# Wumpf/yasph2d

Hardware: AMD Instinct MI355X
Metric: particle-steps/sec (whole node), 2D DFSPH dam-break (higher is better)
Workload: dtype f32

## Files before the change

### include/sphx.h

```cpp
#ifndef SPHX_H
#define SPHX_H

#include <stddef.h>
#include <stdint.h>

#ifdef __cplusplus
extern "C" {
#endif

#define SPHX_ABI_VERSION 5

enum {
    SPHX_OK = 0,
    SPHX_ERR_INVALID_ARGUMENT = 1,
    SPHX_ERR_NO_DEVICE = 2,
    SPHX_ERR_HIP = 3,
    SPHX_ERR_NOT_READY = 4,
    SPHX_ERR_NONFINITE = 5,
    SPHX_ERR_NEIGHBOR_PANIC = 6,
    SPHX_ERR_CAPACITY = 7,
    SPHX_ERR_OUT_OF_DOMAIN = 8
};

enum {
// ... 93 lines not shown
    uint32_t* owner;
} sphx_render_out;
enum { SPHX_RENDER_NONE = 0xFFFFFFFFu, SPHX_RENDER_BOUNDARY = 0xFFFFFFFEu };
enum { SPHX_RENDER_DEVICE_POINTERS = 1u };
int sphx_render_fit(uint32_t width, uint32_t height, float x, float y, float w, float h, sphx_render_view* out);
int sphx_render(sphx_ctx* ctx, const sphx_render_view* view, uint32_t flags, const sphx_render_out* out);

typedef struct sphx_rect { float x0, y0, x1, y1; } sphx_rect;
#define SPHX_REMOVE_MAX_RECTS 8
enum { SPHX_REMOVE_OUTSIDE = 1u };
int sphx_append(sphx_ctx* ctx, const float* pos_xy, const float* vel_xy , uint32_t m, uint32_t* out_first_id );
int sphx_remove(sphx_ctx* ctx, const sphx_rect* rects, uint32_t n_rects, uint32_t flags, uint32_t* out_removed );

#define SPHX_STATE_SECTIONS 9
enum {
    SPHX_STATE_SEC_POSITIONS = 0, SPHX_STATE_SEC_VELOCITIES = 1, SPHX_STATE_SEC_PARTICLE_ID = 2, SPHX_STATE_SEC_DENSITY = 3, SPHX_STATE_SEC_ALPHA = 4,
    SPHX_STATE_SEC_KAPPA = 5, SPHX_STATE_SEC_STIFFNESS = 6, SPHX_STATE_SEC_ACCEL = 7, SPHX_STATE_SEC_BOUNDARY = 8
};
enum { SPHX_STATE_DEVICE_BUFFER = 1u };
int sphx_state_size(sphx_ctx* ctx, uint64_t* out_bytes);
int sphx_state_save(sphx_ctx* ctx, void* buf, uint64_t capacity, uint32_t flags, uint64_t* out_bytes );
int sphx_state_load(sphx_ctx* ctx, const void* buf, uint64_t bytes, uint32_t flags);
int sphx_state_digest(sphx_ctx* ctx, uint64_t* out );
int sphx_state_save_file(sphx_ctx* ctx, const char* path);
int sphx_state_load_file(sphx_ctx* ctx, const char* path);

#define SPHX_TRACK_MAX_IDS 16384
#define SPHX_TRACK_ABSENT  0xFFFFFFFFu
enum { SPHX_TRACK_DEVICE_POINTERS = 1u };
typedef struct sphx_track_out {
    uint32_t* slot;
    float* pos;
    float* vel;
    float* density;
} sphx_track_out;
typedef struct sphx_track_status { uint32_t m, recording, max_frames, every, frames, dropped, reserved[2]; } sphx_track_status;
int sphx_track_set(sphx_ctx* ctx, const uint32_t* ids , uint32_t m);
int sphx_track_fetch(sphx_ctx* ctx, uint32_t flags, const sphx_track_out* out);
int sphx_track_record(sphx_ctx* ctx, uint32_t max_frames, uint32_t every);
int sphx_track_get_status(const sphx_ctx* ctx, sphx_track_status* out);
int sphx_track_read(sphx_ctx* ctx, uint32_t first_frame, uint32_t n_frames, uint32_t flags, float* out );
int sphx_download_by_id(sphx_ctx* ctx, uint32_t first_id, uint32_t count, uint32_t flags, const sphx_track_out* out, uint32_t* out_present );

typedef struct sphx_fields_out {
    float* vel_grad;
    float* divergence;
    float* vorticity;
    float* color_grad;
} sphx_fields_out;
enum { SPHX_FIELDS_DEVICE_POINTERS = 1u };
int sphx_particle_fields(sphx_ctx* ctx, uint32_t flags, const sphx_fields_out* out);

#define SPHX_STATS_MAX_RECTS 8
enum { SPHX_STATS_DEVICE_POINTERS = 1u };
typedef struct sphx_stats_rec {
    uint64_t count;
    uint64_t nonfinite;
    uint64_t density_count;
    uint32_t density_valid;
    uint32_t reserved;
    double sum_pos[2];
    double sum_vel[2];
    double sum_speed_sq;
    double sum_angular;
    double sum_density;
    double sum_density_sq;
    double max_speed_sq;
    float min_pos[2], max_pos[2];
    float min_density, max_density;
} sphx_stats_rec;
typedef struct sphx_stats_frame { uint64_t step; float dt; uint32_t n; } sphx_stats_frame;
typedef struct sphx_stats_status { uint32_t n_rects, recording, max_frames, every, frames, dropped, reserved[2]; } sphx_stats_status;
int sphx_fluid_stats(sphx_ctx* ctx, const sphx_rect* rects , uint32_t n_rects, uint32_t flags, sphx_stats_rec* out );
int sphx_stats_record(sphx_ctx* ctx, const sphx_rect* rects , uint32_t n_rects, uint32_t max_frames, uint32_t every);
int sphx_stats_get_status(const sphx_ctx* ctx, sphx_stats_status* out);
int sphx_stats_read(sphx_ctx* ctx, uint32_t first_frame, uint32_t n_frames, sphx_stats_rec* out ,
                    sphx_stats_frame* info );

int sphx_debug_correction_counts(sphx_ctx* ctx, uint64_t out[3]);
int sphx_debug_quiet_counts(sphx_ctx* ctx, uint64_t out[2]);
int sphx_debug_takeover_counts(sphx_ctx* ctx, uint64_t out[3]);

int sphx_debug_rigid_counts(sphx_ctx* ctx, uint64_t out[3]);
int sphx_debug_download_accel(sphx_ctx* ctx, float* out_xy);

int sphx_clear_cached(sphx_ctx* ctx);
int sphx_step_begin(sphx_ctx* ctx, float dt_prev, float* out_vmax);
int sphx_step_finish(sphx_ctx* ctx, float dt, sphx_step_stats* out_stats);

typedef struct sphx_timer_law {
    uint32_t adaptive;
    float cfl_factor;
    float particle_diameter;
    uint32_t reserved;
    uint64_t timestep_min_ns;
    uint64_t timestep_max_ns;
    uint64_t simulation_step_ns;
} sphx_timer_law;
int sphx_step_begin_law(sphx_ctx* ctx, float dt_prev, const sphx_timer_law* law, float* out_vmax);

int sphx_wcsph_step_begin(sphx_ctx* ctx, float dt, float* out_vmax);
int sphx_wcsph_step_finish(sphx_ctx* ctx, float dt, sphx_step_stats* out_stats);

int sphx_update_neighborhood(sphx_ctx* ctx);
int sphx_update_densities(sphx_ctx* ctx, int kernel_kind);
int sphx_compute_alpha(sphx_ctx* ctx);

int sphx_download_solver_state(sphx_ctx* ctx, float* alpha, float* kappa, float* stiffness);
int sphx_download_neighbors(sphx_ctx* ctx, uint16_t* counts, uint32_t* lists, uint64_t* out_total_entries);
int sphx_download_cells(sphx_ctx* ctx, int which, uint32_t* first_particle, uint32_t* cidx, uint32_t* out_count);
uint32_t sphx_last_flags(const sphx_ctx* ctx);
int sphx_grid_info(const sphx_ctx* ctx, int which, uint32_t* out4);
int sphx_get_constants(const sphx_ctx* ctx, float* out6);
int sphx_get_viscosity(const sphx_ctx* ctx, uint32_t* model, float* fluid_viscosity, float* normalizer_laplacian);


int sphx_reserve(sphx_ctx* ctx, uint32_t capacity);
int sphx_tile_configure(sphx_ctx* ctx, int axis, uint32_t cell_lo, uint32_t cell_hi, uint32_t halo_cells, int has_left, int has_right);
#define SPHX_MAX_TILE_PEERS 8
typedef struct sphx_tile_rect { uint32_t x0, x1, y0, y1; } sphx_tile_rect;
int sphx_tile_configure_rect(sphx_ctx* ctx, const sphx_tile_rect* own, uint32_t halo_cells, const sphx_tile_rect* peers, uint32_t n_peers);
int sphx_tile_pack_n(sphx_ctx* ctx, void* const* d_send, uint32_t n_send, uint32_t cap_records);
int sphx_tile_apply_n(sphx_ctx* ctx, const void* const* d_recv, uint32_t n_recv, uint32_t cap_records);
int sphx_tile_advect_pack_n(sphx_ctx* ctx, float dt, void* const* d_send, uint32_t n_send, uint32_t cap_records);
int sphx_tile_upload(sphx_ctx* ctx, const float* pos_xy, const float* vel_xy, const uint32_t* ids, uint32_t n);
#define SPHX_HALO_RECORD_BYTES 32
int sphx_tile_pack(sphx_ctx* ctx, void* d_send_left, void* d_send_right, uint32_t cap_records);
int sphx_tile_apply(sphx_ctx* ctx, const void* d_from_left, const void* d_from_right, uint32_t cap_records);
int sphx_tile_count_kept(sphx_ctx* ctx);
int sphx_sub_regrid(sphx_ctx* ctx, uint32_t* out_n_local);
int sphx_sub_regrid_div(sphx_ctx* ctx, uint32_t* out_n_local);
int sphx_sub_regrid_warm(sphx_ctx* ctx, uint32_t* out_n_local);
int sphx_sub_run_ahead(sphx_ctx* ctx, float dt_prev_of_next_step);
int sphx_tile_carry_warmstart(sphx_ctx* ctx, int kappa, int stiffness);
int sphx_tile_defer_advect(sphx_ctx* ctx, int on);
int sphx_tile_band_packs(const sphx_ctx* ctx, uint32_t* out);
int sphx_tile_send_counts(sphx_ctx* ctx, void* const* d_send, uint32_t n_send, uint32_t cap_records, uint32_t* out_counts);
int sphx_sub_nonpressure(sphx_ctx* ctx, float dt_prev, float* out_vmax_sq);
int sphx_sub_predict(sphx_ctx* ctx, float dt);
int sphx_sub_warmstart(sphx_ctx* ctx, int divergence, float dt);
int sphx_sub_iteration(sphx_ctx* ctx, int divergence, float dt, int first, double* out_err_sum, uint64_t* out_n_owned);
int sphx_sub_advect(sphx_ctx* ctx, float dt);
int sphx_sub_predict_iteration(sphx_ctx* ctx, float dt, double* out_err_sum, uint64_t* out_n_owned);


typedef struct sphx_multi sphx_multi;
enum { SPHX_LAYOUT_AUTO = 0, SPHX_LAYOUT_STRIPS = 1, SPHX_LAYOUT_GRID = 2 };
typedef struct sphx_multi_options {
    uint32_t halo_cells;
    uint32_t fixed_halo;
    uint32_t rebalance_every;
    uint32_t layout;
    uint32_t cap_records;
    uint32_t overlap_exchange;
    uint32_t reserved[2];
} sphx_multi_options;
typedef struct sphx_comm_ops {
    void* user;
    int rank, world;
    int (*exchange)(void* user, const int* peers, int n_peers, void* const* d_send, void* const* d_recv, size_t bytes, void* hip_stream);
    int (*allreduce)(void* user, const double* in, int n, int op, double* out);
    void (*abort)(void* user);
} sphx_comm_ops;
typedef struct sphx_multi_info_t {
    uint32_t world, local_tiles, halo_now, halo_max, peers, n_local, cap_records, grid_layout;
    int32_t axis;
// ... 247 lines not shown
```

### yasph2d_amd/__init__.py

```python
import ctypes as C

import numpy as np

from . import _lib
from ._lib import (FLAG_DENSITY_ITER_CAP, FLAG_DIVERGENCE_ITER_CAP, FLAG_DENSE_CELL, FLAG_NEIGHBOR_CAP, FLAG_STRAY_PARTICLES, FLAG_WARMUP, KERNEL_POLY6,
                   KERNEL_SPIKY, KERNEL_WENDLAND_C2, VISCOSITY_PHYSICAL, VISCOSITY_XSPH, SphxError, SphxKernelTime, SphxParams, SphxStepStats)

__all__ = ["SphxContext", "FluidParticleWorld", "TimeManager", "DFSPHSolver", "DFSPHMultiSolver", "default_params", "duration_from_secs_f32",
           "duration_as_secs_f32", "SphxError", "WCSPHSolver", "VISCOSITY_XSPH", "VISCOSITY_PHYSICAL", "SAMPLE_FIELDS", "gauge_elevation",
           "sample_merge", "render_fit", "render_merge", "track_merge", "track_merge_frames", "write_png", "SCENE_RECT", "TRACK_FIELDS", "MULTI_TRACK_FIELDS", "FIELD_NAMES", "STATS_DTYPE", "STATS_FRAME_DTYPE"]


def _p(a):
    return a.ctypes.data_as(C.c_void_p) if a is not None else None


LISTS_32BIT = 0xFFFFFFFF


_VISCOSITY_MODELS = {"xsph": VISCOSITY_XSPH, "physical": VISCOSITY_PHYSICAL}


def default_params(smoothing_factor=2.0, particle_density=10000.0, fluid_density=100.0, device=0, fixed_iterations=(0, 0), viscosity="xsph",
                   fluid_viscosity=None):
# ... 538 lines not shown

    def track_record(self, max_frames, every=1):
        self._chk(self.L.sphx_track_record(self.h, max_frames, every))

    def track_frames(self, first=0, count=None):
        st = self.track_status()
        if count is None:
            count = max(st["frames"] - first, 0)
        out = np.zeros((count, st["m"], 4), np.float32)
        self._chk(self.L.sphx_track_read(self.h, first, count, 0, _p(out) if out.size else None))
        return out

    def ids_issued(self):
        first = C.c_uint32()
        rc = self.L.sphx_append(self.h, None, None, 0, C.byref(first))
        if rc == _lib.ERR_NOT_READY:
            return 0
        self._chk(rc)
        return first.value

    def download_by_id(self, first=0, count=None, fields=TRACK_FIELDS):
        if count is None:
            count = max(self.ids_issued() - first, 0)
        outs = _track_outputs(fields, count)
        present = C.c_uint32()
        self._chk(self.L.sphx_download_by_id(self.h, first, count, 0, C.byref(_track_struct(outs)), C.byref(present)))
        outs["present"] = present.value
        return outs

    def download_boundary(self):
        xy = np.zeros((self.nb, 2), np.float32)
        ids = np.zeros(self.nb, np.uint32)
        self._chk(self.L.sphx_download_boundary(self.h, _p(xy), _p(ids)))
        return xy, ids

    def download_solver_state(self):
        n = self.n
        a, k, s = (np.zeros(n, np.float32) for _ in range(3))
        self._chk(self.L.sphx_download_solver_state(self.h, _p(a), _p(k), _p(s)))
        return dict(alpha=a, kappa=k, stiffness=s)

    def download_neighbors(self):
        n = self.n
        counts = np.zeros((n, 2), np.uint16)
        total = C.c_uint64()
        self._chk(self.L.sphx_download_neighbors(self.h, _p(counts), None, C.byref(total)))
        lists = np.zeros(total.value, np.uint32)
        self._chk(self.L.sphx_download_neighbors(self.h, None, _p(lists), C.byref(total)))
        start = np.zeros(n + 1, np.uint64)
        np.cumsum(counts[:, 1].astype(np.uint64), out=start[1:])
        return counts, start, lists

    def download_cells(self, static=False):
        m = C.c_uint32()
        self._chk(self.L.sphx_download_cells(self.h, int(static), None, None, C.byref(m)))
        first = np.zeros(m.value, np.uint32)
        cidx = np.zeros(m.value, np.uint32)
        self._chk(self.L.sphx_download_cells(self.h, int(static), _p(first), _p(cidx), C.byref(m)))
        return first, cidx

    def last_flags(self):
        return self.L.sphx_last_flags(self.h)

    def correction_counts(self):
        out = (C.c_uint64 * 3)()
        self._chk(self.L.sphx_debug_correction_counts(self.h, out))
        return int(out[0]), int(out[1]), int(out[2])

    def quiet_counts(self):
        out = (C.c_uint64 * 2)()
        self._chk(self.L.sphx_debug_quiet_counts(self.h, out))
        return int(out[0]), int(out[1])

    def takeover_counts(self):
        out = (C.c_uint64 * 3)()
        self._chk(self.L.sphx_debug_takeover_counts(self.h, out))
        return int(out[0]), int(out[1]), int(out[2])

    def rigid_counts(self):
        out = (C.c_uint64 * 3)()
        self._chk(self.L.sphx_debug_rigid_counts(self.h, out))
        return int(out[0]), int(out[1]), int(out[2])

    def download_accel(self):
        out = np.zeros((self.n, 2), np.float32)
        self._chk(self.L.sphx_debug_download_accel(self.h, out.ctypes.data_as(C.c_void_p)))
        return out

    def grid_info(self, which=0):
        out = (C.c_uint32 * 4)()
        self._chk(self.L.sphx_grid_info(self.h, which, out))
        return dict(blocks=out[0], entries=out[1], nbx=out[2], nby=out[3])

    def constants(self):
        out = np.zeros(6, np.float32)
        self._chk(self.L.sphx_get_constants(self.h, _p(out)))
        return out

    def viscosity(self):
        m, mu, nlap = C.c_uint32(), C.c_float(), C.c_float()
        self._chk(self.L.sphx_get_viscosity(self.h, C.byref(m), C.byref(mu), C.byref(nlap)))
        return {VISCOSITY_XSPH: "xsph", VISCOSITY_PHYSICAL: "physical"}[m.value], np.float32(mu.value), np.float32(nlap.value)

    def sample(self, points, kernel=KERNEL_WENDLAND_C2, fields=SAMPLE_FIELDS):
        flags = _sample_fields(fields)
        if _is_torch(points):
            import torch

            if points.device.type != "cuda" or points.dtype != torch.float32 or points.dim() != 2 or points.shape[1] != 2:
                raise ValueError("points must be a float32 [m, 2] tensor on the context's device")
            if self.params is not None and points.device.index not in (None, self.params.device):
                raise ValueError("points are on %s, the context on device %d" % (points.device, self.params.device))
            pts = points.contiguous()
            m = pts.shape[0]
            outs = _torch_outputs(flags, (m,), pts.device)
            torch.cuda.current_stream(pts.device).synchronize()
            self._chk(self.L.sphx_sample_points(self.h, C.c_void_p(pts.data_ptr()), m, kernel, _lib.SAMPLE_DEVICE_POINTERS,
                                                C.byref(_out_struct(outs, lambda t: t.data_ptr()))))
            self.synchronize()
            return outs
        pts = np.ascontiguousarray(points, np.float32)
        if pts.ndim != 2 or pts.shape[1] != 2:
            raise ValueError("points must be a float32 [m, 2] array, not shape %s" % (pts.shape,))
        m = len(pts)
        outs = _numpy_outputs(flags, (m,))
        self._chk(self.L.sphx_sample_points(self.h, _p(pts), m, kernel, 0, C.byref(_out_struct(outs, lambda a: a.ctypes.data))))
        return outs

    def sample_grid(self, origin, spacing, shape, kernel=KERNEL_WENDLAND_C2, fields=SAMPLE_FIELDS):
        flags = _sample_fields(fields)
        dx, dy = (spacing, spacing) if np.ndim(spacing) == 0 else spacing
        ny, nx = (int(v) for v in shape)
        if nx < 0 or ny < 0:
            raise ValueError("shape must be (ny, nx) with non-negative sizes")
        outs = _numpy_outputs(flags, (ny, nx))
        self._chk(self.L.sphx_sample_grid(self.h, origin[0], origin[1], dx, dy, nx, ny, kernel, 0,
                                          C.byref(_out_struct(outs, lambda a: a.ctypes.data))))
        return outs

    def render(self, view=None, *, out=None, owner=False, rgba=True, **view_fields):
        if view is None:
            width, height = view_fields.pop("width", 1920), view_fields.pop("height", 1080)
            view = render_fit(width, height, view_fields.pop("world_rect", SCENE_RECT))
        else:
            view = _copy_view(view)
        _set_view_fields(view, view_fields)
        owner_tensor = owner if _is_torch(owner) else None
        owner = owner_tensor is not None or bool(owner)
        if not rgba and not owner:
            raise ValueError("nothing to render: rgba and owner are both off")
        h, w = view.height, view.width
        o = _lib.SphxRenderOut()
        if out is not None or owner_tensor is not None:
            import torch

            dev = out.device if out is not None else owner_tensor.device
            if out is not None and (not _is_torch(out) or out.device.type != "cuda" or out.dtype != torch.uint8 or tuple(out.shape) != (h, w, 4)
                                    or not out.is_contiguous()):
                raise ValueError("out must be a contiguous uint8 (%d, %d, 4) tensor on the context's device" % (h, w))
            if not rgba and out is not None:
                raise ValueError("out given with rgba=False")
            own = None
            if owner:
                own = owner_tensor if owner_tensor is not None else torch.empty((h, w), dtype=torch.int32, device=dev)
                if own.dtype != torch.int32 or tuple(own.shape) != (h, w) or not own.is_contiguous() or own.device != dev:
                    raise ValueError("owner must be a contiguous int32 (%d, %d) tensor on the device of out" % (h, w))
# ... 399 lines not shown
```

### yasph2d_amd/_lib.py

```python
import ctypes as C
import os
import subprocess

_HERE = os.path.dirname(os.path.abspath(__file__))
LIB_PATH = os.environ.get("SPHX_LIB") or os.path.join(_HERE, "libsphx.so")
CSRC = os.path.join(_HERE, "csrc")

OK, ERR_INVALID_ARGUMENT, ERR_NO_DEVICE, ERR_HIP, ERR_NOT_READY, ERR_NONFINITE, ERR_NEIGHBOR_PANIC, ERR_CAPACITY, ERR_OUT_OF_DOMAIN = range(9)
FLAG_NEIGHBOR_CAP, FLAG_DENSITY_ITER_CAP, FLAG_DIVERGENCE_ITER_CAP, FLAG_WARMUP, FLAG_STRAY_PARTICLES, FLAG_DENSE_CELL = 1, 2, 4, 8, 16, 32
KERNEL_WENDLAND_C2, KERNEL_POLY6, KERNEL_SPIKY = 0, 1, 2
VISCOSITY_XSPH, VISCOSITY_PHYSICAL = 0, 1


class SphxParams(C.Structure):
    _fields_ = [
        ("smoothing_length", C.c_float),
        ("particle_mass", C.c_float),
        ("fluid_density", C.c_float),
        ("particle_radius", C.c_float),
        ("gravity", C.c_float * 2),
        ("grid_min", C.c_float * 2),
        ("xsph_epsilon", C.c_float),
        ("max_avg_density_error", C.c_float),
        ("max_density_iterations", C.c_uint32),
# ... 183 lines not shown
                ("exchanges", C.c_uint64), ("rebalances", C.c_uint64), ("build_particles", C.c_uint64), ("neighbor_entries", C.c_uint64),
                ("remote_entries", C.c_uint64), ("owned_local", C.c_uint64), ("transport", C.c_char * 96),
                ("halo_bytes_packed", C.c_uint64), ("halo_bytes_sent", C.c_uint64), ("ownership_seconds", C.c_double)]


LAYOUT_AUTO, LAYOUT_STRIPS, LAYOUT_GRID = 0, 1, 2

_vp, _u16p = C.c_void_p, C.c_void_p
_f, _u32, _u64, _i = C.c_float, C.c_uint32, C.c_uint64, C.c_int
class SphxTileStateOut(C.Structure):
    _fields_ = [(k, C.c_void_p) for k in ("pos", "vel", "id", "density", "alpha", "kappa", "stiffness")]


SIGNATURES = {
    "sphx_abi_version": (_u32, []),
    "sphx_default_params": (_i, [_f, _f, _f, C.POINTER(SphxParams)]),
    "sphx_create": (_i, [C.POINTER(SphxParams), C.POINTER(_vp)]),
    "sphx_destroy": (None, [_vp]),
    "sphx_last_error": (C.c_char_p, [_vp]),
    "sphx_set_boundary": (_i, [_vp, _vp, _u32]),
    "sphx_upload": (_i, [_vp, _vp, _vp, _u32]),
    "sphx_append": (_i, [_vp, _vp, _vp, _u32, C.POINTER(_u32)]),
    "sphx_remove": (_i, [_vp, C.POINTER(SphxRect), _u32, _u32, C.POINTER(_u32)]),
    "sphx_state_size": (_i, [_vp, C.POINTER(_u64)]),
    "sphx_state_save": (_i, [_vp, _vp, _u64, _u32, C.POINTER(_u64)]),
    "sphx_state_load": (_i, [_vp, _vp, _u64, _u32]),
    "sphx_state_digest": (_i, [_vp, C.POINTER(_u64)]),
    "sphx_state_save_file": (_i, [_vp, C.c_char_p]),
    "sphx_state_load_file": (_i, [_vp, C.c_char_p]),
    "sphx_track_set": (_i, [_vp, _vp, _u32]),
    "sphx_track_fetch": (_i, [_vp, _u32, C.POINTER(SphxTrackOut)]),
    "sphx_track_record": (_i, [_vp, _u32, _u32]),
    "sphx_track_get_status": (_i, [_vp, C.POINTER(SphxTrackStatus)]),
    "sphx_track_read": (_i, [_vp, _u32, _u32, _u32, _vp]),
    "sphx_particle_fields": (_i, [_vp, _u32, C.POINTER(SphxFieldsOut)]),
    "sphx_multi_track_set": (_i, [_vp, _vp, _u32]),
    "sphx_multi_track_fetch": (_i, [_vp, _u32, C.POINTER(SphxMultiTrackOut)]),
    "sphx_multi_track_record": (_i, [_vp, _u32, _u32]),
    "sphx_multi_track_get_status": (_i, [_vp, C.POINTER(SphxTrackStatus)]),
    "sphx_multi_track_read": (_i, [_vp, _u32, _u32, _u32, _vp, _vp]),
    "sphx_multi_download_by_id": (_i, [_vp, _u32, _u32, _u32, C.POINTER(SphxMultiTrackOut), C.POINTER(_u32)]),
    "sphx_track_merge": (_i, [_u32, C.POINTER(SphxMultiTrackOut), _u32, C.POINTER(SphxMultiTrackOut), C.POINTER(_u32)]),
    "sphx_track_merge_frames": (_i, [_u64, C.POINTER(_vp), C.POINTER(_vp), _u32, _vp, _vp]),
    "sphx_tile_track_install": (_i, [_vp, _vp, _vp, _u32, _u32]),
    "sphx_tile_track_fetch_enqueue": (_i, [_vp]),
    "sphx_tile_track_fetch": (_i, [_vp, _vp, _vp, _vp]),
    "sphx_tile_track_window_enqueue": (_i, [_vp, _u32, _u32, _u32]),
    "sphx_tile_track_window_fetch": (_i, [_vp, _vp, C.POINTER(_u32)]),
    "sphx_tile_track_record": (_i, [_vp, _u32, _u32]),
    "sphx_tile_track_frame": (_i, [_vp]),
    "sphx_tile_track_read": (_i, [_vp, _u32, _u32, _vp, _vp]),
    "sphx_fluid_stats": (_i, [_vp, C.POINTER(SphxRect), _u32, _u32, _vp]),
    "sphx_stats_record": (_i, [_vp, C.POINTER(SphxRect), _u32, _u32, _u32]),
    "sphx_stats_get_status": (_i, [_vp, C.POINTER(SphxStatsStatus)]),
    "sphx_stats_read": (_i, [_vp, _u32, _u32, _vp, _vp]),
    "sphx_tile_fluid_stats": (_i, [_vp, C.POINTER(SphxRect), _u32, _u32, _vp]),
    "sphx_tile_stats_record": (_i, [_vp, C.POINTER(SphxRect), _u32, _u32, _u32]),
    "sphx_tile_stats_frame": (_i, [_vp, _f, _u32]),
    "sphx_tile_stats_read": (_i, [_vp, _u32, _u32, _vp, _vp]),
    "sphx_multi_fluid_stats": (_i, [_vp, C.POINTER(SphxRect), _u32, _u32, _vp, _vp]),
    "sphx_multi_stats_record": (_i, [_vp, C.POINTER(SphxRect), _u32, _u32, _u32]),
    "sphx_multi_stats_get_status": (_i, [_vp, C.POINTER(SphxStatsStatus)]),
    "sphx_multi_stats_read": (_i, [_vp, _u32, _u32, _vp, _vp]),
    "sphx_tile_state_pack": (_i, [_vp, _u32, C.POINTER(SphxTileStateOut), C.POINTER(_u64), C.POINTER(_u32)]),
    "sphx_tile_state_fetch": (_i, [_vp, C.POINTER(_u64), C.POINTER(_u32)]),
    "sphx_tile_upload_state": (_i, [_vp, _vp, _vp, _vp, _vp, _vp, _u32]),
    "sphx_get_tiling_invariant": (_i, [_vp]),
    "sphx_multi_state_size": (_i, [_vp, C.POINTER(_u64)]),
    "sphx_multi_state_save": (_i, [_vp, _vp, _u64, _u32, C.POINTER(_u64)]),
    "sphx_multi_state_load": (_i, [_vp, C.POINTER(_vp), C.POINTER(_u64), _u32, _u32]),
    "sphx_multi_state_digest": (_i, [_vp, C.POINTER(_u64)]),
    "sphx_multi_state_save_file": (_i, [_vp, C.c_char_p]),
    "sphx_multi_state_load_file": (_i, [_vp, C.c_char_p]),
    "sphx_multi_append": (_i, [_vp, _vp, _vp, _u32, C.POINTER(_u32)]),
    "sphx_multi_remove": (_i, [_vp, C.POINTER(SphxRect), _u32, _u32, C.POINTER(_u64)]),
    "sphx_tile_remove_mark": (_i, [_vp, C.POINTER(SphxRect), _u32, _u32]),
    "sphx_tile_remove_fetch": (_i, [_vp, C.POINTER(_u32)]),
    "sphx_tile_append": (_i, [_vp, _vp, _vp, _vp, _u32]),
    "sphx_tile_grow": (_i, [_vp, _u32]),
    "sphx_debug_correction_counts": (_i, [_vp, _vp]),
    "sphx_debug_quiet_counts": (_i, [_vp, _vp]),
    "sphx_debug_takeover_counts": (_i, [_vp, _vp]),
    "sphx_debug_rigid_counts": (_i, [_vp, _vp]),
    "sphx_debug_download_accel": (_i, [_vp, _vp]),
    "sphx_download_by_id": (_i, [_vp, _u32, _u32, _u32, C.POINTER(SphxTrackOut), C.POINTER(_u32)]),
    "sphx_download": (_i, [_vp, _vp, _vp, _vp, _vp]),
    "sphx_download_boundary": (_i, [_vp, _vp, _vp]),
    "sphx_num_particles": (_u32, [_vp]),
    "sphx_num_boundary": (_u32, [_vp]),
    "sphx_sample_points": (_i, [_vp, _vp, _u32, _i, _u32, C.POINTER(SphxSampleOut)]),
    "sphx_sample_grid": (_i, [_vp, _f, _f, _f, _f, _u32, _u32, _i, _u32, C.POINTER(SphxSampleOut)]),
    "sphx_multi_sample_points": (_i, [_vp, _vp, _u32, _i, _u32, C.POINTER(SphxMultiSampleOut)]),
    "sphx_multi_sample_grid": (_i, [_vp, _f, _f, _f, _f, _u32, _u32, _i, _u32, C.POINTER(SphxMultiSampleOut)]),
    "sphx_sample_merge": (_i, [_u32, C.POINTER(SphxMultiSampleOut), _u32, C.POINTER(SphxMultiSampleOut)]),
    "sphx_multi_tile_rects": (_i, [_vp, C.POINTER(SphxTileRect), C.POINTER(_u32)]),
    "sphx_multi_ghost_rings": (_i, [_vp, C.POINTER(C.c_double)]),
    "sphx_tile_sample_points": (_i, [_vp, _vp, _u32, _i, _u32]),
    "sphx_tile_sample_points_fetch": (_i, [_vp, _vp, _u32, C.POINTER(_u32)]),
    "sphx_tile_sample_window": (_i, [_vp, _f, _f, _f, _f, _u32, _u32, _i, _u32, C.POINTER(_u32)]),
    "sphx_tile_sample_window_fetch": (_i, [_vp, C.POINTER(SphxSampleOut)]),
    "sphx_multi_particle_fields": (_i, [_vp, _u32, C.POINTER(SphxMultiFieldsOut), C.POINTER(C.c_uint64)]),
    "sphx_tile_owned_count": (_i, [_vp, C.POINTER(_u32)]),
    "sphx_tile_particle_fields_enqueue": (_i, [_vp, _u32, _u32]),
    "sphx_tile_particle_fields_fetch": (_i, [_vp, C.POINTER(SphxFieldsOut), _vp, _u32, C.POINTER(_u32)]),
    "sphx_render_fit": (_i, [_u32, _u32, _f, _f, _f, _f, C.POINTER(SphxRenderView)]),
    "sphx_render": (_i, [_vp, C.POINTER(SphxRenderView), _u32, C.POINTER(SphxRenderOut)]),
    "sphx_multi_render": (_i, [_vp, C.POINTER(SphxRenderView), _u32, C.POINTER(SphxRenderOut)]),
    "sphx_multi_render_layer": (_i, [_vp, C.POINTER(SphxRenderView), _u32, C.POINTER(SphxRenderLayer)]),
    "sphx_render_merge": (_i, [_u32, _u32, C.POINTER(SphxRenderLayer), _u32, C.POINTER(SphxRenderLayer)]),
    "sphx_tile_render_layer": (_i, [_vp, C.POINTER(SphxRenderView), _u32, C.POINTER(SphxRenderLayer)]),
    "sphx_tile_render_window": (_i, [_vp, C.POINTER(SphxRenderView), _u32, C.POINTER(_u32), C.POINTER(SphxRenderLayer)]),
    "sphx_clear_cached": (_i, [_vp]),
    "sphx_step_begin": (_i, [_vp, _f, C.POINTER(_f)]),
    "sphx_step_begin_law": (_i, [_vp, _f, _vp, _vp]),
    "sphx_timer_law_of": (_i, [_vp, _f, _vp]),
    "sphx_timer_set_target_frame": (None, [_vp, _u64]),
    "sphx_timer_on_step_started": (None, [_vp]),
    "sphx_step_finish": (_i, [_vp, _f, C.POINTER(SphxStepStats)]),
    "sphx_update_neighborhood": (_i, [_vp]),
    "sphx_update_densities": (_i, [_vp, _i]),
    "sphx_compute_alpha": (_i, [_vp]),
    "sphx_download_solver_state": (_i, [_vp, _vp, _vp, _vp]),
    "sphx_download_neighbors": (_i, [_vp, _vp, _vp, C.POINTER(_u64)]),
    "sphx_download_cells": (_i, [_vp, _i, _vp, _vp, C.POINTER(_u32)]),
    "sphx_grid_info": (_i, [_vp, _i, C.POINTER(_u32)]),
    "sphx_last_flags": (_u32, [_vp]),
    "sphx_get_constants": (_i, [_vp, _vp]),
    "sphx_get_viscosity": (_i, [_vp, C.POINTER(_u32), C.POINTER(_f), C.POINTER(_f)]),
    "sphx_reserve": (_i, [_vp, _u32]),
    "sphx_tile_configure": (_i, [_vp, _i, _u32, _u32, _u32, _i, _i]),
    "sphx_tile_upload": (_i, [_vp, _vp, _vp, _vp, _u32]),
    "sphx_tile_pack": (_i, [_vp, _vp, _vp, _u32]),
    "sphx_tile_apply": (_i, [_vp, _vp, _vp, _u32]),
    "sphx_tile_count_kept": (_i, [_vp]),
    "sphx_sub_regrid": (_i, [_vp, C.POINTER(_u32)]),
    "sphx_sub_regrid_div": (_i, [_vp, C.POINTER(_u32)]),
    "sphx_sub_regrid_warm": (_i, [_vp, C.POINTER(_u32)]),
    "sphx_sub_nonpressure": (_i, [_vp, _f, C.POINTER(_f)]),
    "sphx_sub_predict": (_i, [_vp, _f]),
    "sphx_sub_warmstart": (_i, [_vp, _i, _f]),
    "sphx_sub_iteration": (_i, [_vp, _i, _f, _i, C.POINTER(C.c_double), C.POINTER(_u64)]),
    "sphx_sub_predict_iteration": (_i, [_vp, _f, C.POINTER(C.c_double), C.POINTER(_u64)]),
    "sphx_tile_band_packs": (_i, [_vp, C.POINTER(_u32)]),
    "sphx_tile_send_counts": (_i, [_vp, _vp, _u32, _u32, C.POINTER(_u32)]),
    "sphx_sub_advect": (_i, [_vp, _f]),
    "sphx_shm_open": (_vp, [C.c_char_p, _i, _i]),
    "sphx_shm_allreduce": (_i, [_vp, _vp, _i, _i, _vp]),
    "sphx_shm_allgather": (_i, [_vp, _vp, _i, _vp]),
    "sphx_shm_abort": (None, [_vp]),
    "sphx_sub_run_ahead": (_i, [_vp, C.c_float]),
    "sphx_tile_carry_warmstart": (_i, [_vp, _i, _i]),
    "sphx_set_tiling_invariant": (_i, [_vp, _i]),
    "sphx_tile_defer_advect": (_i, [_vp, _i]),
    "sphx_build_stats": (_i, [_vp, _vp, _vp, _vp]),
    "sphx_shm_close": (None, [_vp]),
    "sphx_tile_configure_rect": (_i, [_vp, _vp, _u32, _vp, _u32]),
    "sphx_tile_pack_n": (_i, [_vp, _vp, _u32, _u32]),
    "sphx_tile_apply_n": (_i, [_vp, _vp, _u32, _u32]),
    "sphx_tile_advect_pack_n": (_i, [_vp, _f, _vp, _u32, _u32]),
    "sphx_view_request": (_i, [_vp, _u32, C.POINTER(_u32)]),
    "sphx_view_fetch": (_i, [_vp, _i, C.POINTER(C.POINTER(_f)), C.POINTER(_u32)]),
    "sphx_synchronize": (_i, [_vp]),
    "sphx_set_stream": (_i, [_vp, _vp]),
    "sphx_profile_enable": (_i, [_vp, _i]),
    "sphx_profile_reset": (_i, [_vp]),
    "sphx_profile_filter": (_i, [_vp, C.c_char_p, _u32]),
# ... 101 lines not shown
```

### yasph2d_amd/csrc/sphx_handoff.hpp

```cpp
#pragma once
#include <cstdint>
#include <cstring>

namespace sphx {

struct BuildHandoff {
    enum Kind : uint8_t { None, WarmApplied, FirstErrors };
    Kind kind = None;
    bool has_flags = false, warm_taken = false;
    uint32_t mark_tag = 0;
    struct Taken {
        bool fused, flags_usable, warm_taken;
    };
    static BuildHandoff warm_applied() { return BuildHandoff{WarmApplied, false, false, 0u}; }
    static BuildHandoff first_errors(bool flags, uint32_t tag, bool taken) { return BuildHandoff{FirstErrors, flags, flags && taken, tag}; }
    void clear() { *this = BuildHandoff{}; }
    bool first_errors_pending() const { return kind == FirstErrors; }
    bool take_warm() {
        const bool applied = kind == WarmApplied;
        if (applied) clear();
        return applied;
    }
    Taken take_first_errors(bool first_divergence, uint32_t rseq) {
        if (kind != FirstErrors || !first_divergence) return Taken{false, false, false};
        const bool usable = has_flags && mark_tag == rseq;
        const Taken t{true, usable, usable && warm_taken};
        clear();
        return t;
    }
};

class PendingCount {
  public:
    enum class Maker : uint8_t { Nobody, Correction, Pack, Classifier };
    PendingCount() = default;
    void made_by_correction(uint32_t n) { *this = PendingCount(Maker::Correction, n); }
    void made_by_pack(uint32_t n) { *this = PendingCount(Maker::Pack, n); }
    void made_by_classifier(uint32_t n, float dt) { *this = PendingCount(Maker::Classifier, n, true, bits(dt)); }
    bool live() const { return maker_ != Maker::Nobody; }
    bool from_classifier() const { return maker_ == Maker::Classifier; }
    bool is_for(uint32_t n) const { return live() && n_ == n; }
    bool is_for_first_of(uint32_t n) const { return live() && n_ <= n; }
    uint32_t n() const { return n_; }
    bool take_over_class(uint32_t n, float dt) {
        const bool mine = from_classifier() && takeable_ && n_ == n && dt_bits_ == bits(dt);
        if (mine) made_by_pack(n);
        return mine;
    }
    void bar_take_over() { takeable_ = false; }
    bool drop() {
        const bool wipe = live();
        forget();
        return wipe;
    }
    bool drop_if_from_classifier() { return from_classifier() && drop(); }
    void forget() { *this = PendingCount(); }

  private:
    PendingCount(Maker m, uint32_t n, bool takeable = false, uint32_t dt_bits = 0) : maker_(m), takeable_(takeable), n_(n), dt_bits_(dt_bits) {}
    static uint32_t bits(float f) {
        uint32_t u;
        std::memcpy(&u, &f, 4);
        return u;
    }
    Maker maker_ = Maker::Nobody;
    bool takeable_ = false;
    uint32_t n_ = 0, dt_bits_ = 0;
};

struct VelMarks {
    bool valid = false, thin_seen = false;
    uint32_t tag = 0, knz_tag = 0;
    struct Taken {
        bool usable, check_knz;
        uint32_t tag, knz_tag;
    };
    void made(uint32_t gather_tag) { *this = VelMarks{true, false, gather_tag, 0u}; }
    void thin(uint32_t rseq) {
        if (!valid) return;
        if (thin_seen) return wrote();
        thin_seen = true;
        knz_tag = rseq;
    }
    void wrote() { *this = VelMarks{}; }
    Taken take() {
        const Taken t{valid, valid && thin_seen, tag, knz_tag};
        wrote();
        return t;
    }
};

}
```

### yasph2d_amd/csrc/sphx_internal.hpp

```cpp
#pragma once
#include <hip/hip_runtime.h>

#include <dlfcn.h>

#include <algorithm>
#include <cstdint>
#include <cstdlib>
#include <cstdio>
#include <cstring>
#include <functional>
#include <map>
#include <string>
#include <vector>

#include "../../include/sphx.h"
#include "sphx_handoff.hpp"

namespace sphx {

constexpr uint32_t EMPTY = 0xFFFFFFFFu;
constexpr uint32_t MAX_NEIGHBORS = 64;
constexpr uint32_t BLOCK_SHIFT = 6;
constexpr uint32_t BLOCK_CELLS = 4096;
constexpr uint32_t SCAN_TILE = 4096;
// ... 18 lines not shown
constexpr uint32_t REMOTE_CAP = 512;
constexpr uint32_t ENTRY_BITS = 10, ENTRY_MASK = (1u << ENTRY_BITS) - 1u;
constexpr uint32_t WAVE_REMOTE = REMOTE_CAP / 4;
constexpr uint32_t STRIPES = 32;

constexpr uint32_t DIR_FRINGE = 0x80000000u;
constexpr uint32_t DIR_STATIC = 1u;
constexpr uint32_t DIR_FLAGS = DIR_FRINGE | DIR_STATIC;
enum : uint32_t { DF_OUT_OF_DOMAIN = 1u, DF_HALO_CAP = 2u, DF_NB_CAP = 4u, DF_NB_PANIC = 8u, DF_NEAR_EDGE = 16u, DF_STRAY = 32u, DF_SCAN_STALL = 64u, DF_NONFINITE = 128u, DF_DENSE_CELL = 256u };
constexpr uint32_t RANK_LOOP_MAX = 4096;
constexpr uint32_t LOOP_HIST = 512;

constexpr uint32_t MAX_TILE_PEERS = 8;
struct TileRect {
    uint32_t x0, x1, y0, y1;
};

struct Consts {
    float h;
    float radius_sq;
    float cell_inv;
    float gmin_x, gmin_y;
    float w_hinv, w_norm, w_ngrad;
    float p6_hsq, p6_norm, p6_ngrad;
    float sp_h, sp_norm, sp_ngrad;
    float mass, rho0, xsph_eps;
    float ax, ay;
    float gx, gy;
    float wc_stiffness, wc_boundary_force;
    TileRect tile;
    uint32_t remote_cap;
    uint32_t q_noclamp;
    uint32_t nt_cold;
    uint32_t xcd_shift;
    uint32_t rev;
};

struct ViscConsts {
    uint32_t visc_model;
    float mu;
    float vis_nlap;
};
template <int VM>
struct ViscArg {};
template <>
struct ViscArg<SPHX_VISCOSITY_PHYSICAL> : ViscConsts {};

struct NbView {
    const uint32_t* list;
    const uint16_t* counts;
    const uint32_t* wave;
    const uint32_t* remote;
    uint32_t lazy_hi;
    uint32_t stream;
};
constexpr uint32_t COUNT_MANY_LINES = 1u << 14;
struct PVr {
    const float2* pos;
    const float2* vel;
};

struct GridView {
    const uint32_t* dir;
    const uint2* fine;
    uint32_t bx0, by0, nbx, nby;
    uint32_t cbits;
};
struct NbGrid {
    const uint32_t* dirn;
    const uint2* fine;
    uint32_t bx0, by0, nbx, nbx1, nby1;
};
constexpr uint32_t DIRN_FLAG = 1u;

struct alignas(128) Stripe {
    unsigned long long nb_entries;
    unsigned long long owned;
    unsigned long long rem_entries;
    unsigned long long res_hi, res_lo;
    uint32_t ticket;
    uint32_t pad0;
    unsigned long long zs_skipped, zs_window, zs_remote;
    unsigned long long zs_quiet;
    uint32_t pad[12];
};
static_assert(sizeof(Stripe) == 128, "one stripe, one cache line");
struct alignas(128) VmaxStripe {
    uint32_t vmax[4];
    uint32_t pad[28];
};
struct alignas(128) MarkStripe {
    uint32_t knz_mark;
    uint32_t vmix_mark;
    uint32_t pad[30];
};
static_assert(sizeof(MarkStripe) == 128, "one stripe, one cache line");
struct alignas(128) SpecLine {
    uint32_t flags;
    uint32_t pad0;
    unsigned long long moved;
    uint32_t pad[28];
};
struct DevScalars {
    uint32_t flags;
    uint32_t ticket;
    uint32_t sort_total;
    float dt;
    uint32_t loop_done;
    uint32_t pad0;
    unsigned long long snap_hi[2], snap_lo[2];
    uint32_t rigid_exits, rigid_marked;
    uint32_t pad[16];
    Stripe stripe[STRIPES];
    VmaxStripe vstripe[STRIPES];
    MarkStripe mstripe[STRIPES];
    SpecLine spec;
};

struct Mailbox {
    volatile uint32_t seq;
    uint32_t flags;
    uint32_t vmax_sq_bits;
    uint32_t quiet_seq;
    double err_sum;
    unsigned long long nb_entries;
    unsigned long long owned_cum;
    unsigned long long rem_entries;
    uint32_t sort_total;
    uint32_t dt_bits;
    unsigned long long dt_ns;
    volatile uint32_t loop_gen_done;
    uint32_t loop_iters;
    double loop_hist[LOOP_HIST];
    uint32_t send_counts[MAX_TILE_PEERS];
    uint32_t rigid_tag;
};

struct ResArgs {
    uint32_t enabled;
    uint32_t rseq;
    Mailbox* mb;
    uint32_t seq;
};
struct VmaxArgs {
    uint32_t enabled;
    uint32_t vslot;
    Mailbox* mb;
    uint32_t seq;
};
struct LoopArgs {
    uint32_t enabled;
    uint32_t iter;
    uint32_t fixed;
    uint32_t max_iters;
    uint32_t gen;
    uint32_t n_total;
    float tol;
    float rho0;
    float dt;
};

struct TimerLaw {
    uint32_t enabled, adaptive;
    float cfl_factor, particle_diameter;
    unsigned long long min_ns, max_ns, step_ns;
};

struct Grid {
    uint32_t* dir = nullptr;
    uint32_t* dirn = nullptr;
    uint32_t dir_cap = 0;
    uint2* fine = nullptr;
    uint32_t* hist = nullptr;
    uint32_t* tile_empty = nullptr;
    uint32_t tile_cap = 0;
    uint32_t fine_cap = 0;
    uint32_t bx0 = 0, by0 = 0, nbx = 0, nby = 0, nblk = 0;
    std::vector<uint8_t> cover;
    std::vector<uint32_t> h_dir;
    bool fine_valid = false;
    uint32_t len() const { return nblk * BLOCK_CELLS; }
    uint32_t cbits_floor = 1;
    uint32_t cbits() const {
        uint32_t b = cbits_floor < 1u ? 1u : cbits_floor > 31u ? 31u : cbits_floor;
        while (b < 31u && ((1u << b) - 1u) < len()) ++b;
        return b;
    }
    GridView view() const { return GridView{dir, fine, bx0, by0, nbx, nby, cbits()}; }
    NbGrid nview() const { return nbx && nby ? NbGrid{dirn, fine, bx0, by0, nbx, nbx - 1u, nby - 1u} : NbGrid{dirn, fine, 0u, 0u, 1u, 0u, 0u}; }
};

struct ProfTotals {
    uint64_t launches = 0;
    double ms = 0, bytes = 0;
};
struct ProfPending {
    const char* name;
    double bytes;
    hipEvent_t a, b;
// ... 13 lines not shown
    uint32_t B = 0, capB = 0;
    uint32_t cached_n = 0;
    bool set_changed = false;
    uint64_t ids_issued = 0;
    uint32_t* edit_buf = nullptr;
    uint32_t edit_cap = 0;
    static constexpr uint32_t MARK_NONE = 0xFFFFFFFFu, MARK_EMPTY = 0xFFFFFFFEu;
    uint32_t edit_mark = MARK_NONE;
    struct Track {
        uint32_t m = 0, unique = 0, log2_bits = 0;
        uint32_t* set_buf = nullptr;
        uint32_t *table = nullptr, *map = nullptr, *filter = nullptr, *found = nullptr;
        float* rec = nullptr;
        uint32_t recording = 0, max_frames = 0, every = 0, frames = 0, dropped = 0, steps = 0;
        uint32_t* scratch = nullptr;
        size_t scratch_cap = 0;
        uint32_t window_cap = 0;
    } track;
    struct Stats {
        sphx_stats_rec* scratch = nullptr;
        sphx_stats_rec* rec = nullptr;
        sphx_rect rects[SPHX_STATS_MAX_RECTS] = {};
        uint32_t n_rects = 0, recording = 0, max_frames = 0, every = 0, frames = 0, dropped = 0, steps = 0;
        std::vector<sphx_stats_frame> info;
    } stats;
    bool uploaded = false, boundary_changed = true, tails_dirty = true, in_step = false;
    bool lists_current = false;
    unsigned long long* state_dig = nullptr;
    uint32_t* mstate_buf = nullptr;
    size_t mstate_cap = 0;
    uint32_t mstate_n = 0;
    uint32_t fast_walk_ok = 0;
    uint32_t sample_ready = 0;
    bool tile_density_ready = false;
    const char* sample_missing = "no neighbour build yet: run a step, or sphx_update_neighborhood + sphx_update_densities";
    float* sample_buf = nullptr;
    size_t sample_cap = 0;
    struct TileSample {
        uint32_t m = 0;
        uint32_t fields = 0;
        uint32_t win[4] = {0, 0, 0, 0};
        size_t rec_at = 0;
        uint32_t* null_grid = nullptr;
    } tsample;
    uint32_t* render_buf = nullptr;
    size_t render_cap = 0;
    float* fields_buf = nullptr;
    size_t fields_cap = 0;
    struct TileFields {
        bool queued = false;
        uint32_t n = 0;
        uint32_t mask = 0;
        bool ids = false;
    } tfields;
    uint32_t num_density_iters = 1, num_divergence_iters = 0;
    float step_dt_prev = 0, step_vmax = 0;
    uint32_t step_flags = 0;

    float2 *posA = nullptr, *posA2 = nullptr;
    float2 *vel = nullptr, *vel2 = nullptr;
    sphx::PVr pv() const { return sphx::PVr{posA, vel}; }
    float* kbuf = nullptr;
    uint32_t* knz = nullptr;
    int zero_skip = -1;
    bool zero_skip_on() const { return zero_skip < 0 ? N >= 4000000u : zero_skip != 0; }
    int zero_skip_count = 0;
    bool quiet_hint[2] = {false, false};
    unsigned long long qf_launches = 0;
    int quiet_takeover = 1;
    uint32_t thin_grid = 0;
    int quiet_takeover_density = 1;
    bool take_over(bool divergence) const {
        return !tile_mode && (divergence || quiet_takeover_density) && (quiet_takeover == 2 || (quiet_takeover == 1 && quiet_hint[divergence ? 1 : 0]));
    }
    unsigned long long thin_launches = 0, takeover_producers = 0;
    int rigid_skip = -1;
    bool rigid_on() const { return !tile_mode && (rigid_skip < 0 ? N >= 4000000u : rigid_skip != 0); }
    sphx::VelMarks velmarks;
    uint32_t gather_seq = 0;
    bool rigid_hint = false;
    uint32_t rigid_judged = 0;
    void rigid_forget() {
        velmarks.wrote();
        rigid_hint = false;
        rigid_judged = 0;
    }
    unsigned long long rigid_launches = 0;
    float2* accel = nullptr;
    float *density = nullptr, *alpha = nullptr, *alpha2 = nullptr, *kappa = nullptr, *stiff = nullptr;
    float *kappa2 = nullptr, *stiff2 = nullptr;
    uint32_t *pid = nullptr, *pid2 = nullptr;
    uint32_t *key = nullptr, *slot = nullptr, *order = nullptr;
    uint32_t idx_cap = 0;
    uint32_t soff() const { return capN; }
    float2 *bpos = nullptr, *bpos2 = nullptr;
    uint32_t *bid = nullptr, *bid2 = nullptr;
    sphx::Grid gdyn, gstat;
    bool have_fluid_bbox = false;
    uint32_t fb[4] = {0, 0, 0, 0};
    uint32_t builds_since_cover = 0;
    bool need_expand = false;
    bool need_recover = false;
    uint32_t recover_streak = 0;
    uint32_t recover_cooldown = 0;
    float wcsph_vmax_prev = 0.0f;
    std::vector<float> h_boundary;
    uint32_t* nb_list = nullptr;
    uint16_t* nb_counts = nullptr;
    uint32_t* nb_wave = nullptr;
    uint32_t* nb_remote = nullptr;
    uint32_t pre_seq = 0, pre_warm = 0, law_dt_bits = 0;
    bool law_active = false;
    uint32_t pre_gen = 0;
    uint32_t pre_queued = 0;
    uint32_t loop_gen = 0;
    uint32_t res_seq = 0;
    uint32_t vmax_seq = 0;
    struct RunAhead {
        bool queued = false;
        bool valid = false;
        uint32_t n = 0, dt_bits = 0, vslot = 0;
        uint32_t seq = 0;
    } ahead;
    float tile_pending_dt = 0.0f;
    uint32_t tile_pending_n = 0;
    bool tile_defer_advect = false;
    float sub_ahead_dt = 0.0f;
    bool tile_carry_kappa = true, tile_carry_stiff = true;
    bool tiling_invariant = false;
    int run_ahead = 1;
#ifndef SPHX_DEFAULT_FUSE_PREDICT
#define SPHX_DEFAULT_FUSE_PREDICT 1
#endif
    int fuse_predict = SPHX_DEFAULT_FUSE_PREDICT;
    int tile_fuse_class = 1;
    uint32_t tile_band_packs = 0;
    bool tile_fix_owner = false;
    int fuse_div = 1;
    int xcd_chunk = -1;
    int alternate_sweep = 1;
    int fuse_warm = 1;
    sphx::BuildHandoff handoff;
    int host_loop = 0;
    std::string prof_filter;
    uint32_t prof_every = 1, prof_counter = 0;
    bool external_stream = false;
    hipStream_t view_stream = nullptr;
    hipEvent_t view_packed = nullptr, view_done = nullptr;
    float *view_dev = nullptr, *view_host = nullptr;
    uint32_t view_cap = 0, view_count = 0;
    bool view_pending = false;
    uint32_t wcsph_n = 0;
    bool in_wcsph = false;
    int lazy_table = 1;
    int stream_lists = -1;
    int nt_cold_stores = -1;
    sphx::NbView nbv() const {
        return sphx::NbView{nb_list, nb_counts, nb_wave, nb_remote, (uint32_t)lazy_table, stream_lists < 0 ? (N >= 4000000u ? 1u : 0u) : (uint32_t)stream_lists};
    }
    uint32_t* scan_partials = nullptr;
    uint32_t scan_partials_cap = 0;
    unsigned long long* scan_state = nullptr;
    uint32_t scan_state_cap = 0, scan_epoch = 0;
    sphx::PendingCount pending;
    int no_fused_count = 0;
    int scan_two_pass = 0;
    sphx::DevScalars* d_scal = nullptr;
    sphx::Mailbox* mbox = nullptr;
    sphx::Mailbox* mbox_dev = nullptr;
    uint32_t seq = 0;
// ... 29 lines not shown
```

### yasph2d_amd/csrc/sphx_kernels.hip

```cpp
#include "sphx_internal.hpp"
#include "sphx_sqrt.hpp"
#include "sphx_xcd.hpp"

namespace sphx {

__device__ __forceinline__ uint32_t part1by1(uint32_t x) {
    x &= 0xffffu;
    x = (x ^ (x << 8)) & 0x00ff00ffu;
    x = (x ^ (x << 4)) & 0x0f0f0f0fu;
    x = (x ^ (x << 2)) & 0x33333333u;
    x = (x ^ (x << 1)) & 0x55555555u;
    return x;
}
__device__ __forceinline__ uint32_t morton2(uint32_t x, uint32_t y) { return (part1by1(y) << 1) | part1by1(x); }

__device__ __forceinline__ uint32_t spread6(uint32_t v) {
    v &= 63u;
    v = (v | (v << 4)) & 0x30Fu;
    v = (v | (v << 2)) & 0x333u;
    v = (v | (v << 1)) & 0x555u;
    return v;
}
__device__ __forceinline__ uint32_t sat_u16(float v) {
    v = fminf(fmaxf(v, 0.0f), 65535.0f);
// ... 1989 lines not shown
        va.mb->vmax_sq_bits = bits;
        if (law.enabled) {
            __hip_atomic_store((uint32_t*)&scal->dt, __float_as_uint(dt_new), __ATOMIC_RELAXED, __HIP_MEMORY_SCOPE_AGENT);
            va.mb->dt_ns = ns;
            va.mb->dt_bits = __float_as_uint(dt_new);
        }
    }
    publish_common(scal, va.mb, va.seq);
}

__device__ __forceinline__ unsigned long long residual_fixed(float e, bool& bad) {
    bad = !(e < 1073741824.0f);
    const float t = __builtin_rintf((bad ? 0.0f : e) * 16777216.0f);
    const uint32_t bits = __float_as_uint(t);
    const uint32_t m = (bits & 0x7fffffu) | 0x800000u;
    const int sh = (int)((bits >> 23) & 0xffu) - 150;
    unsigned long long f = sh >= 0 ? (unsigned long long)m << (sh & 63) : (unsigned long long)(m >> min(-sh, 31));
    return (bits & 0x7f800000u) ? f : 0ull;
}
__device__ __forceinline__ void block_residual_add(float e, DevScalars* __restrict__ scal) {
    bool bad;
    const unsigned long long f = wave_sum_u63(residual_fixed(e, bad));
    __shared__ unsigned long long ws[4];
    if ((threadIdx.x & 63) == 0) ws[threadIdx.x >> 6] = f;
    if (__any(bad) && (threadIdx.x & 63) == 0) atomicOr(&scal->flags, DF_NONFINITE);
    __syncthreads();
    if (threadIdx.x == 0) {
        const unsigned long long t = ws[0] + ws[1] + ws[2] + ws[3];
        Stripe* st = &scal->stripe[blockIdx.x % STRIPES];
        if (t >> 32) atomicAdd(&st->res_hi, t >> 32);
        if (t & 0xffffffffull) atomicAdd(&st->res_lo, t & 0xffffffffull);
    }
}
__device__ __forceinline__ void residual_stripe_load(const DevScalars* __restrict__ scal, unsigned long long& hi, unsigned long long& lo) {
    const uint32_t lane = threadIdx.x & 63u;
    hi = lane < STRIPES ? scal->stripe[lane].res_hi : 0ull;
    lo = lane < STRIPES ? scal->stripe[lane].res_lo : 0ull;
}
__device__ __forceinline__ void residual_wave_reduce(unsigned long long& hi, unsigned long long& lo) {
    hi = wave_sum_u63(hi);
    lo = wave_sum_u63(lo);
}
__device__ __forceinline__ double residual_sum_f64(unsigned long long hi, unsigned long long lo, unsigned long long hi0, unsigned long long lo0) {
    return ((double)(hi - hi0) * 4294967296.0 + (double)(lo - lo0)) * (1.0 / 16777216.0);
}

__global__ __launch_bounds__(256) void k_block_occupancy(const uint2* __restrict__ fine, uint32_t nblk, uint8_t* __restrict__ occ) {
    const uint32_t b = blockIdx.x * 256 + threadIdx.x;
    if (b >= nblk) return;
    occ[b] = fine[(size_t)b * BLOCK_CELLS].x != fine[(size_t)b * BLOCK_CELLS + BLOCK_CELLS - 1].y ? 1 : 0;
}

__global__ __launch_bounds__(64) void k_clear_vmax_slot(DevScalars* scal, uint32_t vslot) {
    if (threadIdx.x < STRIPES) __hip_atomic_store(&scal->vstripe[threadIdx.x].vmax[vslot & 3u], 0u, __ATOMIC_RELAXED, __HIP_MEMORY_SCOPE_AGENT);
}

__global__ __launch_bounds__(64) void k_publish_vmax(DevScalars* scal, VmaxArgs va) {
    const uint32_t b = wave_vmax_get(scal, va.vslot);
    vmax_publish(scal, va, b, TimerLaw{}, 0ull, 0.0f);
}

#ifndef NONP_BOUNDS
#define NONP_BOUNDS __launch_bounds__(256) __attribute__((amdgpu_waves_per_eu(8, 8)))
#endif
__device__ __forceinline__ float physical_visc(const Consts& K, const ViscConsts& V, float mu_m, float r, float rho_j) {
    return mu_m * (V.vis_nlap * (K.h - r)) / rho_j;
}
template <int VM>
__global__ NONP_BOUNDS void k_nonpressure(PVr PV, const float* __restrict__ density, uint32_t n, uint32_t soff, Consts K,
                                                      float dt, NbView nb, float2* __restrict__ accel, DevScalars* __restrict__ scal, uint32_t vslot,
                                                      ViscArg<VM> V) {
    __shared__ Stage<2, 1> rec;
    const uint32_t blk = xcd_bid(K.rev, K.xcd_shift);
#include "sphx_nonpressure_body.inc"
    block_vmax_add(vsq, scal, vslot, (uint32_t*)&rec.raw[0]);
}

struct RigidArgs {
    uint32_t vmix_tag;
    uint32_t knz_tag;
    uint32_t check_knz;
    uint32_t vgrid;
    Mailbox* mb;
};
__device__ __forceinline__ bool rigid_marked(const DevScalars* __restrict__ scal, float rho0, float dt, const RigidArgs& ra) {
    uint32_t vm = ~ra.vmix_tag, km = ~ra.knz_tag;
    if ((threadIdx.x & 63u) < STRIPES) {
        vm = scal->mstripe[threadIdx.x & 63u].vmix_mark;
        km = scal->mstripe[threadIdx.x & 63u].knz_mark;
    }
    const float rd = rho0 * dt;
    const bool dt_ok = dt > 0.0f && dt <= 3.402823466e38f && rd >= 1.175494351e-38f && rd <= 3.402823466e38f;
    return __any(vm == ra.vmix_tag || (ra.check_knz != 0u && km == ra.knz_tag)) != 0 || !dt_ok;
}
template <int VM>
__global__ NONP_BOUNDS void k_nonpressure_rigid(PVr PV, const float* __restrict__ density, uint32_t n, uint32_t soff, Consts K,
                                                            float dt, NbView nb, float2* __restrict__ accel, DevScalars* __restrict__ scal, uint32_t vslot,
                                                            ViscArg<VM> V, RigidArgs ra) {
    __shared__ Stage<2, 1> rec;
    uint32_t* const wm = (uint32_t*)&rec.raw[0];
    if (threadIdx.x < 64) {
        const bool m = rigid_marked(scal, K.rho0, dt, ra);
        if (threadIdx.x == 0) wm[0] = m ? 1u : 0u;
    }
    __syncthreads();
    const bool marked = wm[0] != 0u;
    if (blockIdx.x == 0 && threadIdx.x == 0) {
        __hip_atomic_store(&ra.mb->rigid_tag, marked ? 0u : ra.vmix_tag, __ATOMIC_RELAXED, __HIP_MEMORY_SCOPE_SYSTEM);
        atomicAdd(marked ? &scal->rigid_marked : &scal->rigid_exits, 1u);
    }
    if (!marked) {
        const float2 a = make_float2(K.ax, K.ay);
        for (uint32_t vblk = blockIdx.x; vblk < ra.vgrid; vblk += gridDim.x) {
            const uint32_t i = xcd_map(vblk, ra.vgrid, K.rev, K.xcd_shift) * 256u + threadIdx.x;
            if (i < n) accel[i] = a;
        }
        if (blockIdx.x == 0 && threadIdx.x == 0) {
            const float2 v = PV.vel[0];
            const float px = v.x + a.x * dt, py = v.y + a.y * dt;
            const uint32_t m = __float_as_uint(px * px + py * py);
            if (m) atomicMax(&scal->vstripe[0].vmax[vslot & 3u], m);
        }
        return;
    }
    uint32_t vbits = 0u;
    for (uint32_t vblk = blockIdx.x; vblk < ra.vgrid; vblk += gridDim.x) {
        __syncthreads();
        const uint32_t blk = xcd_map(vblk, ra.vgrid, K.rev, K.xcd_shift);
#include "sphx_nonpressure_body.inc"
        vbits = max(vbits, __float_as_uint(vsq));
    }
    block_vmax_add(__uint_as_float(vbits), scal, vslot, wm);
}
__global__ __launch_bounds__(64) void k_rigid_judge(const DevScalars* __restrict__ scal, float rho0, float dt, RigidArgs ra) {
    const bool marked = rigid_marked(scal, rho0, dt, ra);
    if (threadIdx.x == 0) __hip_atomic_store(&ra.mb->rigid_tag, marked ? 0u : ra.vmix_tag, __ATOMIC_RELAXED, __HIP_MEMORY_SCOPE_SYSTEM);
}

__global__ __launch_bounds__(256) void k_predict(float2* __restrict__ vel, const float2* __restrict__ accel, uint32_t n, float dt,
                                                  DevScalars* __restrict__ scal, VmaxArgs va, TimerLaw law) {
    const uint32_t i = xcd_bid() * 256 + threadIdx.x;
    const uint32_t il = min(i, n - 1u);
    float2 v = vel[il];
    const float2 a = accel[il];
    if (va.enabled) {
        __shared__ float dt_s;
        if (threadIdx.x < 64) {
            const uint32_t b = wave_vmax_get(scal, va.vslot);
            unsigned long long ns = 0;
            float d = dt;
            if (law.enabled) {
                ns = timer_law_step_ns(law, sqrtf(__uint_as_float(b)));
                d = duration_as_secs_f32(ns);
            }
            if (threadIdx.x == 0) dt_s = d;
            if (blockIdx.x == 0) vmax_publish(scal, va, b, law, ns, d);
        }
        __syncthreads();
        dt = dt_s;
    }
    if (i >= n) return;
    v.x = v.x + a.x * dt;
    v.y = v.y + a.y * dt;
    vel[i] = v;
}

__global__ __launch_bounds__(256) void k_wcsph_leapfrog1(float2* __restrict__ vel, float2* __restrict__ posA, const float2* __restrict__ accel,
                                                          uint32_t n, float dt) {
    const uint32_t i = xcd_bid() * 256 + threadIdx.x;
    if (i >= n) return;
    const float2 p0 = posA[i], v0 = vel[i];
    float4 pv = make_float4(p0.x, p0.y, v0.x, v0.y);
    const float2 a = accel[i];
    const float hdt = 0.5f * dt;
    pv.z = pv.z + hdt * a.x;
    pv.w = pv.w + hdt * a.y;
    pv.x = pv.x + pv.z * dt;
    pv.y = pv.y + pv.w * dt;
    vel[i] = make_float2(pv.z, pv.w);
    posA[i] = make_float2(pv.x, pv.y);
}
__device__ __forceinline__ float powi7(float a) {
    float r = a;
    a = a * a;
    r = r * a;
    a = a * a;
    return r * a;
}
__device__ __forceinline__ float wcsph_pressure(const Consts& K, float local_density) {
    return K.wc_stiffness * (powi7(fmaxf(local_density / K.rho0, 1.0f)) - 1.0f);
}
template <int VM>
__global__ TRAV_BOUNDS void k_wcsph_accel(PVr PV, const float* __restrict__ density, uint32_t n, uint32_t soff, Consts K,
                                          float dt, NbView nb, float2* __restrict__ accel, DevScalars* __restrict__ scal, uint32_t vslot,
                                          ViscArg<VM> V) {
    __shared__ Stage<2, 1> rec;
    const uint32_t blk = xcd_bid(K.rev, K.xcd_shift);
    const uint32_t i = blk * 256 + threadIdx.x;
// ... 1 lines not shown
    struct StageRec {
        float4 pv;
        float rho;
    };
    nb_stage(
        h, nb, blk, i, n, [&](uint32_t g) { return StageRec{ldpv(PV, g), gat(density, g < soff ? g : 0u)}; },
        [&](uint32_t g) {
            const Pair<float4> pv = ldpv2(PV, g);
            const Pair<float> rho = gat2(density, g < soff ? g : 0u);
            return Pair<StageRec>{StageRec{pv.a, rho.a}, StageRec{pv.b, rho.b}};
        },
        [&](uint32_t slot, const StageRec& r) {
            rec.put_vec01(slot, r.pv);
            rec.put_scal<0>(slot, r.rho);
        });
    __syncthreads();
    float vsq = 0.0f;
    if (i < n) {
        const uint32_t oi = (i - h.lw0) * 4u;
        const float4 pvi = h.wide ? ldpv(PV, i) : rec.vec01(oi);
        const float rhoi = density[i];
        const uint32_t cd = h.cd, ct = h.ct;
        float ax = K.gx, ay = K.gy;
        const float pi = wcsph_pressure(K, rhoi);
        struct Rec {
            float4 pv;
            float rho;
        };
        auto walk = [&](auto fast) {
            auto consume = [&](const Rec& q, uint32_t k) {
                const float dx = q.pv.x - pvi.x, dy = q.pv.y - pvi.y;
                const float r_sq = dx * dx + dy * dy;
                const float r = sqrt_dist<decltype(fast)::value>(r_sq);
                if (k < cd) {
                    const float pj = wcsph_pressure(K, q.rho);
                    const float pu = -K.mass * (pi + pj) / (2.0f * rhoi * q.rho);
                    const float dd = fmaxf(K.sp_h - r, 0.0f);
                    const float sg = K.sp_ngrad * dd * dd / (r + 1.0e-10f);
                    float tx = ax + pu * (sg * dx);
                    float ty = ay + pu * (sg * dy);
                    float f;
                    if constexpr (VM == SPHX_VISCOSITY_PHYSICAL)
                        f = physical_visc(K, V, V.mu * K.mass, r, q.rho);
                    else
                        f = K.xsph_eps * K.mass * poly6_eval(K, r_sq) / (q.rho * dt);
                    ax = tx + f * (q.pv.z - pvi.z);
                    ay = ty + f * (q.pv.w - pvi.w);
                } else {
                    const float s = K.wc_boundary_force * spiky_eval(K, r) / r_sq;
                    ax = ax - s * dx;
                    ay = ay - s * dy;
                }
            };
            nb_traverse(
                h, ct, [&](uint32_t o) { return Rec{rec.vec01(o), rec.scal<0>(o)}; },
                [&](uint32_t g) { return Rec{ldpv(PV, g), gat(density, g < soff ? g : i)}; }, consume);
        };
        if (K.q_noclamp)
            walk(std::true_type{});
        else
            walk(std::false_type{});
        accel[i] = make_float2(ax, ay);
        const float px = pvi.z + ax * dt, py = pvi.w + ay * dt;
        vsq = tile_owns(K, pvi.x, pvi.y) ? px * px + py * py : 0.0f;
    }
    block_vmax_add(vsq, scal, vslot);
}

struct PredArgs {
    const float2* accel;
    float2* vel_out;
    VmaxArgs va;
    TimerLaw law;
};
struct NoTake {};
template <bool DIVERGENCE, bool PREDICT = false, bool KNZ = false, bool TAKE = false>
__global__ TRAV_BOUNDS void k_compute_error(PVr PV, const float* __restrict__ density,
                                                        const float* __restrict__ alpha, uint32_t n, uint32_t soff, Consts K, float dt,
                                                        NbView nb, float* __restrict__ kbuf, float* __restrict__ warm_zero,
                                                        DevScalars* __restrict__ scal, const float* __restrict__ dt_dev, LoopArgs la,
                                                        uint32_t* __restrict__ clear_hist, uint32_t clear_len, PredArgs pa,
                                                        uint32_t* __restrict__ knz, uint32_t knz_tag,
                                                        std::conditional_t<TAKE && !DIVERGENCE, CountArgs, NoTake> ta) {
    static_assert(!TAKE || KNZ, "the take-over producers are the ones that leave flags");
    constexpr bool SPEC = TAKE && !DIVERGENCE;
    if (la.enabled && la.iter > 1u && scal->loop_done != 0u) return;
    if (dt_dev) dt = *dt_dev;
    if (clear_hist) {
        const uint32_t per = (clear_len + gridDim.x - 1u) / gridDim.x;
        const uint32_t c0 = blockIdx.x * per, c1 = min(c0 + per, clear_len);
        for (uint32_t k = c0 + threadIdx.x; k < c1; k += 256u) clear_hist[k] = 0u;
    }
    __shared__ Stage<2, 0> rec;
    auto put = [&](uint32_t slot, const float4& r) { rec.put_vec01(slot, r); };
    auto take = [&](uint32_t o) { return rec.vec01(o); };
    const uint32_t blk = xcd_bid(K.rev, K.xcd_shift);
    const uint32_t i = blk * 256 + threadIdx.x;
    NbHead h = nb_head(nb, blk, i, n);
    const float rho_i = (!DIVERGENCE && i < n) ? density[i] : 0.0f;
    const float alpha_i = i < n ? alpha[i] : 0.0f;
    struct PredRec {
        float4 pv;
        float2 a;
    };
    auto load_pred = [&](uint32_t g) { return PredRec{ldpv(PV, g), gat(pa.accel, g < soff ? g : 0u)}; };
    auto predicted = [&](const PredRec& r, uint32_t g) {
        return g < soff ? make_float4(r.pv.x, r.pv.y, r.pv.z + r.a.x * dt, r.pv.w + r.a.y * dt) : r.pv;
    };
    if (PREDICT) {
        uint32_t vb = 0;
        if (pa.va.enabled && threadIdx.x < STRIPES) vb = scal->vstripe[threadIdx.x].vmax[pa.va.vslot & 3u];
        auto load_pred2 = [&](uint32_t g) {
            const Pair<float4> pv = ldpv2(PV, g);
            const Pair<float2> a = gat2(pa.accel, g < soff ? g : 0u);
            return Pair<PredRec>{PredRec{pv.a, a.a}, PredRec{pv.b, a.b}};
        };
        const NbStaged<PredRec> st = nb_stage_load(h, nb, blk, i, n, load_pred, load_pred2);
        __shared__ float dt_s;
        if (pa.va.enabled && threadIdx.x < 64) {
            const uint32_t b = wave_max_u32(vb);
            const unsigned long long ns = timer_law_step_ns(pa.law, sqrtf(__uint_as_float(b)));
            const float d = duration_as_secs_f32(ns);
            if (threadIdx.x == 0) dt_s = d;
            if (blockIdx.x == 0) vmax_publish(scal, pa.va, b, pa.law, ns, d);
        }
        if (pa.va.enabled) {
            __syncthreads();
            dt = dt_s;
        }
        nb_stage_store(h, st, [&](uint32_t slot, const PredRec& r, uint32_t g) { put(slot, predicted(r, g)); });
    } else {
        nb_stage(h, nb, blk, i, n, [&](uint32_t g) { return ldpv(PV, g); }, [&](uint32_t g) { return ldpv2(PV, g); }, put);
    }
    __syncthreads();
    float e = 0.0f, e_owned = 0.0f;
    uint32_t k_bits = 0u;
    [[maybe_unused]] float2 pnew = make_float2(0.0f, 0.0f);
    [[maybe_unused]] DirAhead ahead{0xFFFFFFFFu, EMPTY};
    if (i < n) {
        const uint32_t ct = h.ct;
        float4 pvi = h.wide ? ldpv(PV, i) : take((i - h.lw0) * 4u);
        if (PREDICT && h.wide) pvi = predicted(load_pred(i), i);
        if constexpr (SPEC) {
            if (ta.hist) {
                uint32_t cx0, cy0;
                cell_of(K, make_float2(pvi.x, pvi.y), cx0, cy0);
                ahead = dir_ahead(ta.g, cx0, cy0);
            }
        }
        if (!(DIVERGENCE && ct < 9)) {
            const float2 ri = make_float2(pvi.x, pvi.y);
            float delta = 0.0f;
            auto walk = [&](auto fast) {
                auto consume = [&](const float4& r, uint32_t) {
                    const float2 g = wendland_grad<decltype(fast)::value>(K, ri, make_float2(r.x, r.y));
                    const float dvx = pvi.z - r.z, dvy = pvi.w - r.w;
                    delta = delta + (dvx * g.x + dvy * g.y);
                };
                nb_traverse(h, ct, take, [&](uint32_t g) { return PREDICT ? predicted(load_pred(g), g) : ldpv(PV, g); }, consume);
            };
            if (K.q_noclamp)
                walk(std::true_type{});
            else
                walk(std::false_type{});
            if (DIVERGENCE) {
                e = fmaxf(delta * K.mass, 0.0f);
            } else {
                e = rho_i + delta * K.mass * dt;
                e = fmaxf(K.rho0, e) - K.rho0;
            }
        }
        const float kv = e * alpha_i;
        kbuf[i] = kv;
        k_bits = __float_as_uint(kv);
        if (PREDICT) pa.vel_out[i] = make_float2(pvi.z, pvi.w);
        if constexpr (TAKE)
            store_cold(&warm_zero[i], 0.0f + kv, K.nt_cold);
        else if (warm_zero)
            warm_zero[i] = 0.0f;
        e_owned = tile_owns(K, pvi.x, pvi.y) ? e : 0.0f;
        if constexpr (SPEC) pnew = make_float2(pvi.x + pvi.z * dt, pvi.y + pvi.w * dt);
    }
    if constexpr (SPEC)
        if (ta.hist) count_cell(K, ta.g, i < n, i, pnew, ta.hist, ta.cidx, ta.slot, 1u, scal, ahead, &scal->spec.flags);
    if constexpr (KNZ) knz_store(knz, i, k_bits, scal, knz_tag);
    block_residual_add(e_owned, scal);
}

struct ZeroSkipArgs {
    const uint32_t* knz;
    uint32_t count;
};
template <bool WARM, bool INV_DT, bool TILE = false, bool ZS = false, bool QF = false>
__global__ TRAV_BOUNDS void k_correct(float2* __restrict__ vel, const float2* __restrict__ posA, const float* __restrict__ kbuf,
                                                  float* __restrict__ warm, uint32_t n,
                                                  uint32_t soff, Consts K, float inv_dt, float lim, NbView nb,
                                                  const float* __restrict__ dt_dev, CountArgs ca, DevScalars* __restrict__ scal, LoopArgs la, ResArgs ra,
                                                  uint32_t first, TileClassArgs tc, ZeroSkipArgs zs) {
    constexpr bool THIN = false;
    constexpr uint32_t vblk = 0u, vgrid = 0u;
    constexpr bool look = true;
#define SPHX_CORRECT_LEAVE(quiet) return
#include "sphx_correct_body.inc"
#undef SPHX_CORRECT_LEAVE
}

template <bool INV_DT>
__global__ TRAV_BOUNDS void k_correct_thin(float2* __restrict__ vel, const float2* __restrict__ posA, const float* __restrict__ kbuf,
                                                       float* __restrict__ warm, uint32_t n, uint32_t soff, Consts K, float inv_dt, float lim, NbView nb,
                                                       const float* __restrict__ dt_dev, CountArgs ca, DevScalars* __restrict__ scal, LoopArgs la,
                                                       ResArgs ra, ZeroSkipArgs zs, uint32_t vgrid) {
    constexpr bool WARM = false, TILE = false, ZS = true, QF = true, THIN = true;
    constexpr uint32_t first = 1u;
    const TileClassArgs tc{};
    for (uint32_t vblk = blockIdx.x; vblk < vgrid; vblk += gridDim.x) {
        const bool look = vblk == blockIdx.x;
        if (!look) __syncthreads();
#define SPHX_CORRECT_LEAVE(quiet) \
    {                             \
        if (quiet) return;        \
        continue;                 \
    }
#include "sphx_correct_body.inc"
#undef SPHX_CORRECT_LEAVE
    }
}

__global__ __launch_bounds__(256) void k_export_counts(const uint16_t* __restrict__ counts, uint32_t n, uint16_t* __restrict__ out,
                                                        uint32_t* __restrict__ totals) {
    const uint32_t i = blockIdx.x * 256 + threadIdx.x;
    if (i >= n) return;
    const uint32_t c = counts[i];
    out[2 * i] = (uint16_t)(c & 0x7fu);
    out[2 * i + 1] = (uint16_t)((c >> 7) & 0x7fu);
    totals[i] = (c >> 7) & 0x7fu;
}
__global__ __launch_bounds__(256) void k_export_lists(NbView nb, uint32_t soff, const uint32_t* __restrict__ start, uint32_t n,
                                                       uint32_t* __restrict__ out) {
    const uint32_t i = blockIdx.x * 256 + threadIdx.x;
    if (i >= n) return;
    const NbHead h = nb_head(nb, i >> 8, i, n);
    const uint32_t s = start[i];
    for (uint32_t k = 0; k < h.ct; ++k) {
        uint32_t g;
        if (h.wide) {
            g = *(const uint32_t*)(h.rows + (uint32_t)((k * 64u + h.lane) * 4u));
        } else {
            const uint32_t word = *(const uint32_t*)(h.rows + (k / 3u) * SUBROW_B + h.lane * 4u);
            const uint32_t slot = entry_off(word, k % 3u) >> 2;
            g = slot < LIST_WIN ? h.lw0 + slot : nb.remote[(size_t)(i >> 8) * REMOTE_CAP + (slot - LIST_WIN)];
        }
        out[s + k] = g < soff ? g : g - soff;
    }
}
__global__ __launch_bounds__(256) void k_keys_of(const float2* __restrict__ pos, uint32_t n, Consts K, uint32_t* __restrict__ key) {
    const uint32_t i = blockIdx.x * 256 + threadIdx.x;
    if (i >= n) return;
    uint32_t cx, cy;
    cell_of(K, pos[i], cx, cy);
    key[i] = morton2(cx, cy);
}
__global__ void k_clear_flags(DevScalars* scal, uint32_t mask) { atomicAnd(&scal->flags, ~mask); }
__global__ __launch_bounds__(256) void k_view_pack(PVr PV, uint32_t n, uint32_t stride, float* __restrict__ out) {
    const uint32_t k = blockIdx.x * 256 + threadIdx.x;
    const uint64_t i = (uint64_t)k * stride;
    if (i >= n) return;
    const float4 pv = ldpv(PV, (uint32_t)i);
    out[3 * (size_t)k + 0] = pv.x;
    out[3 * (size_t)k + 1] = pv.y;
// ... 40 lines not shown
```

### yasph2d_amd/csrc/sphx_launch.inc

```
#include <algorithm>
#include <cmath>

using namespace sphx;

static std::string g_create_error;

#define SPHX_HIP(ctx, expr)                                                        \
    do {                                                                           \
        hipError_t e__ = (expr);                                                   \
        if (e__ != hipSuccess) return (ctx)->fail(SPHX_ERR_HIP, #expr, hipGetErrorString(e__)); \
    } while (0)

namespace {

inline uint32_t nblocks(uint32_t n, uint32_t per = 256) {
    const uint32_t b = (n + per - 1) / per;
    return per == 256 ? (b + 7u) & ~7u : b;
}
inline double kbar_of(const sphx_ctx* c) { return (c->N && c->nb_last) ? (double)c->nb_last / (double)c->N : 12.0; }
inline double list_bytes(const sphx_ctx* c) {
    if (!c->K.remote_cap) return 2.0 + 4.0 * kbar_of(c);
    const double rbar = c->N ? (double)c->rem_last / (double)c->N : 0.5;
    return 2.0 + 4.0 / 64.0 + (4.0 / 3.0) * kbar_of(c) + 4.0 * rbar + 4.0 / 256.0;
}
// ... 423 lines not shown
    const unsigned long long rm = c->mbox->rem_entries;
    if (rm != c->rem_cum) {
        c->rem_last = rm - c->rem_cum;
        c->rem_cum = rm;
    }
    const unsigned long long ow = c->mbox->owned_cum;
    if (ow != c->owned_cum) {
        c->owned_last = ow - c->owned_cum;
        c->owned_cum = ow;
    }
    const uint32_t f = c->mbox->flags;
    if (f) hipLaunchKernelGGL(k_clear_flags, dim3(1), dim3(1), 0, c->stream, c->d_scal, f);
    if (f & DF_NB_CAP) c->step_flags |= SPHX_FLAG_NEIGHBOR_CAP;
    if (f & DF_HALO_CAP) return c->fail(SPHX_ERR_CAPACITY, "halo exchange buffer too small for the particles near a tile cut");
    if (f & DF_NEAR_EDGE) c->need_expand = true;
    if (f & DF_STRAY) {
        c->step_flags |= SPHX_FLAG_STRAY_PARTICLES;
        c->need_recover = true;
    }
    if (f & DF_DENSE_CELL) c->step_flags |= SPHX_FLAG_DENSE_CELL;
    if (f & DF_SCAN_STALL) return c->fail(SPHX_ERR_HIP, "the cell-table scan stalled waiting for a predecessor workgroup");
    if (f & DF_NONFINITE) return c->fail(SPHX_ERR_NONFINITE, "a solver residual is not finite (dfsph.rs:223 / :378 assert)");
    if (f & DF_OUT_OF_DOMAIN) return c->fail(SPHX_ERR_OUT_OF_DOMAIN, "a particle left the Morton domain the grid tables were sized for, or has no cell at all (a NaN position)");
    if (f & DF_NB_PANIC) return c->fail(SPHX_ERR_NEIGHBOR_PANIC, "64 dynamic neighbours and a static hit (neighborhood_search.rs:373 panics here)");
    return SPHX_OK;
}

int publish_and_wait(sphx_ctx* c) {
    const uint32_t seq = ++c->seq;
    hipLaunchKernelGGL(k_publish, dim3(1), dim3(64), 0, c->stream, c->d_scal, c->mbox_dev, seq);
    return wait_mailbox(c, seq);
}

void wipe_histogram(sphx_ctx* c, Grid& g) {
    if (g.hist && g.len()) hipMemsetAsync(g.hist, 0, (size_t)g.len() * 4, c->stream);
}
void drop_fused_count(sphx_ctx* c) {
    if (c->pending.drop()) wipe_histogram(c, c->gdyn);
}
void clear_histograms(sphx_ctx* c) {
    c->pending.forget();
    for (Grid* g : {&c->gdyn, &c->gstat}) wipe_histogram(c, *g);
}

void drop_class_count(sphx_ctx* c) {
    if (c->pending.drop_if_from_classifier()) wipe_histogram(c, c->gdyn);
}
void flush_pending_advect(sphx_ctx* c) {
    if (c->pending.from_classifier() || c->tile_pending_dt > 0.0f) (void)hipSetDevice(c->device);
    drop_class_count(c);
    if (!(c->tile_pending_dt > 0.0f)) return;
    const uint32_t n = c->tile_pending_n;
    const float dt = c->tile_pending_dt;
    c->tile_pending_dt = 0.0f;
    c->tile_pending_n = 0;
    const bool fix = c->tile_fix_owner;
    c->tile_fix_owner = false;
    if (!n) return;
    if (fix) {
        TilePeers none{};
        hipLaunchKernelGGL(k_tile_pack, dim3(nblocks(n)), dim3(256), 0, c->stream, (const float2*)c->vel, c->posA, c->pid, (const float*)c->kappa,
                           (const float*)c->stiff, n, c->K, c->tile_halo, none, (const uint32_t*)c->tile_blk, 0u, dt, CountArgs{}, c->d_scal, 1u,
                           (const uint32_t*)nullptr);
        return;
    }
    hipLaunchKernelGGL(k_advect, dim3(nblocks(n)), dim3(256), 0, c->stream, c->posA, (const float2*)c->vel, n, dt);
}

void sub_step_enter(sphx_ctx* c) {
    c->ahead.valid = false;
    flush_pending_advect(c);
}

int build_grid(sphx_ctx* c, Grid& g, const float2* pos, uint32_t n, const GatherArgs& ga, float advect_dt, bool ring, uint32_t* tile_n = nullptr,
               bool mark_velocities = false) {
    hipStream_t st = c->stream;
    DevScalars* ds = c->d_scal;
    const uint32_t len = g.len();
    const uint32_t nt = nblocks(len, c->scan_two_pass ? SCAN_TILE : SCAN1_TILE);
    const bool counted = &g == &c->gdyn && advect_dt > 0 && !tile_n && c->pending.is_for(n);
    const bool partial = &g == &c->gdyn && tile_n && advect_dt == 0.0f && !counted && c->pending.is_for_first_of(n);
    const uint32_t first = partial ? c->pending.n() : 0u;
    if (&g == &c->gdyn) c->velmarks.wrote();
    if (counted || partial)
        c->pending.forget();
    else
        drop_fused_count(c);
    if (n > first && !counted) {
        const uint32_t gbc = std::max(1u, nblocks(n - first));
        if (advect_dt > 0)
            launch(c, "advect+cell_count", (16.0 + 4 + 4) * n, [&] {
                hipLaunchKernelGGL(k_key_count<true>, dim3(gbc), dim3(256), 0, st, c->pv(), (const float2*)nullptr, n, advect_dt, c->K,
                                   g.view(), g.hist, c->key, c->slot, ring ? 1u : 0u, ds, first);
            });
        else
            launch(c, "cell_count", (8.0 + 4 + 4) * (n - first), [&] {
                hipLaunchKernelGGL(k_key_count<false>, dim3(gbc), dim3(256), 0, st, PVr{nullptr, nullptr}, pos, n, 0.0f, c->K, g.view(),
                                   g.hist, c->key, c->slot, ring ? 1u : 0u, ds, first);
            });
    }
    if (!len) hipMemsetAsync(&ds->sort_total, 0, 4, st);
    uint32_t scan_seq = 0;
    if (len)
        launch(c, "cell_scan", (c->scan_two_pass ? 20.0 : 16.0) * len, [&] {
            if (c->scan_two_pass) {
                hipLaunchKernelGGL(k_scan_reduce, dim3(nt), dim3(256), 0, st, (const uint32_t*)g.hist, len, c->scan_partials, ds, &ds->sort_total);
                hipLaunchKernelGGL(k_scan_apply, dim3(nt), dim3(256), 0, st, g.hist, g.fine, len, (const uint32_t*)c->scan_partials);
                hipMemsetAsync(g.tile_empty, 0, (size_t)g.tile_cap * 4, st);
            } else {
                if (++c->scan_epoch == 0) c->scan_epoch = 1;
                if (tile_n) scan_seq = ++c->seq;
                hipLaunchKernelGGL(k_scan_onepass, dim3(nt), dim3(256), 0, st, g.hist, g.fine, len, c->scan_state, c->scan_epoch, ds, &ds->sort_total,
                                   tile_n ? c->mbox_dev : (Mailbox*)nullptr, scan_seq, g.tile_empty, tile_n ? 0xFFFFFFFFu : n);
            }
        });
    g.fine_valid = len != 0;
    if (n) {
        launch(c, "cell_scatter", 12.0 * n, [&] {
            hipLaunchKernelGGL(k_scatter, dim3((nblocks(n, 256 * SCATTER_PER_LANE) + 7u) & ~7u), dim3(256), 0, st, (const uint32_t*)c->key, (const uint32_t*)c->slot, n, (const uint2*)g.fine,
                               c->order, g.cbits(), g.hist, xcd_scatter_pack(c->K.rev, xcd_shift_of(c)));
        });
        const uint32_t ng = n;
        if (tile_n) {
            if (scan_seq) {
                *tile_n = scan_seq;
            } else {
                const uint32_t seq = ++c->seq;
                hipLaunchKernelGGL(k_publish, dim3(1), dim3(64), 0, st, ds, c->mbox_dev, seq);
                *tile_n = seq;
            }
        }
        const uint32_t gb2 = std::max(8u, (nblocks(ng, 256 * GATHER_PER_LANE) + 7u) & ~7u);
        double gbytes = 4;
        gbytes += ga.vel_in ? (16 + 16) : 16;
        if (ga.r_in) gbytes += 8;
        if (ga.r2_in) gbytes += 8;
        if (ga.r3_in) gbytes += 8;
        if (ga.u_in) gbytes += 8;
        GatherArgs gm = ga;
        if (mark_velocities && &g == &c->gdyn && !tile_n && ga.vel_in) {
            if (++c->gather_seq == 0) c->gather_seq = 1;
            gm.vmix_tag = c->gather_seq;
        }
        if (ng)
            launch(c, "gather_attributes", gbytes * ng, [&] {
                hipLaunchKernelGGL(k_rank_gather, dim3(gb2), dim3(256), 0, st, (const uint32_t*)c->order, (const uint32_t*)c->key, ng, n,
                                   (const uint2*)g.fine, gm, tile_n ? (const uint32_t*)&ds->sort_total : (const uint32_t*)nullptr, g.cbits(), xcd_pack(c->K.rev, xcd_shift_of(c)));
            });
        if (ng && gm.vmix_tag) c->velmarks.made(gm.vmix_tag);
    }
    return SPHX_OK;
}

int ensure_index_scratch(sphx_ctx* c) {
    const uint32_t need = std::max(std::max(std::max(c->N, c->capN), c->B), 1u);
    if (need <= c->idx_cap) return SPHX_OK;
    int rc;
    if ((rc = dev_alloc(c, &c->key, need))) return rc;
#ifdef SPHX_SLOT_AT_COUNT
    if ((rc = dev_alloc(c, &c->slot, need))) return rc;
#endif
    if ((rc = dev_alloc(c, &c->order, need))) return rc;
    SPHX_HIP(c, hipMemsetAsync(c->order, 0, (size_t)need * 4, c->stream));
    c->idx_cap = need;
    return SPHX_OK;
}
// ... 148 lines not shown
        c->need_recover = false;
        c->recover_streak = 8;
    }
    if (c->recover_streak) {
        c->recover_streak -= 1;
        if (c->recover_cooldown) {
            c->recover_cooldown -= 1;
        } else if ((rc = recover_directory(c, cover_dt, cover_below))) {
            return rc;
        }
    }
    GatherArgs ga{};
    ga.flags = c->d_scal;
    ga.pos_in = c->posA;
    ga.pos_out = c->posA2;
    ga.vel_in = c->vel;
    ga.vel_out = c->vel2;
    ga.advect_dt = advect_dt;
    ga.advect_below = 0xFFFFFFFFu;
    if (extra_alpha) {
        ga.r_in = c->alpha;
        ga.r_out = c->alpha2;
    }
    ga.u_in = c->pid;
    ga.u_out = c->pid2;
    uint32_t tile_n = c->N;
    const bool carry_kappa = c->tile_mode ? c->tile_carry_kappa : c->tiling_invariant, carry_stiff = c->tile_mode ? c->tile_carry_stiff : c->tiling_invariant;
    ga.rank_by_id = c->tiling_invariant ? 1u : 0u;
    ga.nt_cold = c->nt_cold_stores < 0 ? (c->N >= NT_COLD_FROM ? 1u : 0u) : (uint32_t)c->nt_cold_stores;
    if (carry_kappa) {
        ga.r2_in = c->kappa;
        ga.r2_out = c->kappa2;
    }
    if (carry_stiff) {
        ga.r3_in = c->stiff;
        ga.r3_out = c->stiff2;
    }
    if (c->tile_mode) ga.count_owned = c->d_scal;
    if (c->tile_pending_dt > 0.0f) {
        if (c->tile_mode && advect_dt == 0.0f && c->pending.is_for(c->tile_pending_n) && c->tile_pending_n <= c->N) {
            ga.advect_dt = c->tile_pending_dt;
            ga.advect_below = c->tile_pending_n;
            c->tile_pending_dt = 0.0f;
            c->tile_pending_n = 0;
            if (c->tile_fix_owner) {
                c->tile_fix_owner = false;
                ga.fix_owner = 1u;
                ga.cell_inv = c->K.cell_inv;
                ga.gmin_x = c->K.gmin_x;
                ga.gmin_y = c->K.gmin_y;
                ga.own = c->K.tile;
            }
        } else {
            flush_pending_advect(c);
        }
    }
    const bool take_div = fuse && fuse_div && !fuse_warm && zero_skip_flags(c) && c->take_over(true);
    if ((rc = build_grid(c, c->gdyn, c->posA, c->N, ga, advect_dt, true, c->tile_mode ? &tile_n : nullptr, take_div && advect_dt > 0.0f && c->rigid_on())))
        return rc;
    if (carry_kappa) std::swap(c->kappa, c->kappa2);
    if (carry_stiff) std::swap(c->stiff, c->stiff2);
    std::swap(c->vel, c->vel2);
    std::swap(c->posA, c->posA2);
    if (extra_alpha) std::swap(c->alpha, c->alpha2);
    std::swap(c->pid, c->pid2);
    c->K.q_noclamp = c->fast_walk_ok;
    hipStream_t st = c->stream;
    const uint32_t* n_dev = c->tile_mode ? (const uint32_t*)&c->d_scal->sort_total : (const uint32_t*)nullptr;
    if (c->N) {
        const uint32_t n = c->N;
        auto go = [&](auto kernel, const DivArgs& dv) {
            hipLaunchKernelGGL(kernel, dim3(nblocks(n)), dim3(256), 0, st, (const float2*)c->posA, n, c->soff(), c->K, c->gdyn.nview(), c->gstat.nview(),
                               c->nb_list, c->nb_counts, c->nb_wave, c->nb_remote, c->density, c->alpha, c->d_scal, n_dev, dv);
        };
        c->handoff.clear();
        if (fuse && fuse_warm) {
            DivArgs dv{};
            dv.velw = c->vel;
            dv.warm = c->stiff;
            dv.lim = -0.5f * c->K.rho0 * c->K.rho0;
            launch(c, "neighbor_build+density_alpha+divergence_warmstart", (8.0 + list_bytes(c) + 8.0 + 8.0 + 8.0 + 4.0) * n, [&] { go(k_neighbor_build<3>, dv); });
            c->handoff = BuildHandoff::warm_applied();
            c->velmarks.wrote();
        } else if (fuse && fuse_div) {
            DivArgs dv{};
            dv.vel = (const float2*)c->vel;
            dv.kbuf = c->kbuf;
            dv.knz = zero_skip_flags(c);
            dv.knz_tag = c->res_seq + 1u;
            const bool take = take_div;
            if (take) {
                dv.warm = c->stiff;
                c->takeover_producers += 1;
            }
            launch(c, "neighbor_build+density_alpha+density_change", (8.0 + list_bytes(c) + 8.0 + 8.0 + 4.0) * n,
                   [&] { take ? go(k_neighbor_build<2, true>, dv) : go(k_neighbor_build<2>, dv); });
            c->handoff = BuildHandoff::first_errors(dv.knz != nullptr, dv.knz_tag, take);
        } else if (fuse)
            launch(c, "neighbor_build+density_alpha", (8.0 + list_bytes(c) + 8.0) * n, [&] { go(k_neighbor_build<1>, DivArgs{}); });
        else
            launch(c, "neighbor_build", (8.0 + list_bytes(c)) * n, [&] { go(k_neighbor_build<0>, DivArgs{}); });
    }
    if (c->tile_mode && c->N) {
        if ((rc = wait_mailbox(c, tile_n))) return rc;
        c->N = std::min(c->mbox->sort_total, c->N);
    }
    c->lists_current = true;
    c->sample_ready = 1u;
    c->sample_missing = "the densities of the last neighbour build are missing: call sphx_update_densities";
    return SPHX_OK;
}

template <int KIND>
void launch_density(sphx_ctx* c, bool density, bool alpha) {
    const uint32_t n = c->N;
    if (!n) return;
    const double bytes = (8.0 + list_bytes(c) + (density ? 4 : 0) + (alpha ? 4 : 0)) * n;
    auto go = [&](auto kernel) {
        hipLaunchKernelGGL(kernel, dim3(nblocks(n)), dim3(256), 0, c->stream, (const float2*)c->posA, n, c->soff(), c->K, c->nbv(), c->density, c->alpha);
    };
    if (density && alpha) return launch(c, "density_alpha", bytes, [&] { go(k_density_alpha<KIND, true, true>); });
    if (density) return launch(c, "update_densities", bytes, [&] { go(k_density_alpha<KIND, true, false>); });
    launch(c, "compute_alpha_factors", bytes, [&] { go(k_density_alpha<0, false, true>); });
}

int alloc_particles(sphx_ctx* c, uint32_t n, uint32_t cap = 0, bool keep_set = false) {
    if (n <= c->capN) return SPHX_OK;
    cap = std::max(cap, n);
    int rc = 0;
    if ((rc = ensure_nb_arrays(c, cap, c->capB, keep_set))) return rc;
    float *old_kappa = c->kappa, *old_stiff = c->stiff, *old_alpha = c->alpha;
    float2* old_accel = c->accel;
    uint32_t* old_pid = keep_set ? c->pid : nullptr;
    if (keep_set) c->pid = nullptr;
    const uint32_t keep = std::min(c->cached_n, c->capN);
    const uint32_t keep_accel = std::min(c->wcsph_n, c->capN);
    c->kappa = c->stiff = c->alpha = nullptr;
    c->accel = nullptr;
    auto give_up = [&](int code) {
        dev_free(&old_kappa);
        dev_free(&old_stiff);
        dev_free(&old_alpha);
        dev_free(&old_accel);
        dev_free(&old_pid);
        c->cached_n = 0;
        c->wcsph_n = 0;
        c->uploaded = false;
        return code;
    };
#define A(p) \
    if ((rc = dev_alloc(c, &c->p, cap))) return give_up(rc);
    A(accel) A(density) A(alpha) A(alpha2) A(kappa) A(stiff) A(kappa2) A(stiff2) A(pid) A(pid2) A(nb_counts) A(kbuf)
#undef A
    if ((rc = dev_alloc(c, &c->knz, (size_t)(nblocks(cap) + 8) * 4))) return give_up(rc);
    if ((rc = dev_alloc(c, &c->nb_remote, (size_t)(nblocks(cap) + 8) * REMOTE_CAP))) return give_up(rc);
    if ((rc = dev_alloc(c, &c->nb_wave, (size_t)(nblocks(cap) + 8) * 4))) return give_up(rc);
    const size_t slices = ((size_t)cap + 63) / 64;
    if ((rc = dev_alloc(c, &c->nb_list, slices * 64 * 64))) return give_up(rc);
    SPHX_HIP(c, hipMemsetAsync(c->kappa, 0, (size_t)cap * 4, c->stream));
    SPHX_HIP(c, hipMemsetAsync(c->stiff, 0, (size_t)cap * 4, c->stream));
    SPHX_HIP(c, hipMemsetAsync(c->alpha, 0, (size_t)cap * 4, c->stream));
    SPHX_HIP(c, hipMemsetAsync(c->density, 0, (size_t)cap * 4, c->stream));
    if (keep) {
        SPHX_HIP(c, hipMemcpyAsync(c->kappa, old_kappa, (size_t)keep * 4, hipMemcpyDeviceToDevice, c->stream));
        SPHX_HIP(c, hipMemcpyAsync(c->stiff, old_stiff, (size_t)keep * 4, hipMemcpyDeviceToDevice, c->stream));
        SPHX_HIP(c, hipMemcpyAsync(c->alpha, old_alpha, (size_t)keep * 4, hipMemcpyDeviceToDevice, c->stream));
    }
    if (keep_accel) SPHX_HIP(c, hipMemcpyAsync(c->accel, old_accel, (size_t)keep_accel * 8, hipMemcpyDeviceToDevice, c->stream));
    if (old_pid && c->N) SPHX_HIP(c, hipMemcpyAsync(c->pid, old_pid, (size_t)c->N * 4, hipMemcpyDeviceToDevice, c->stream));
    SPHX_HIP(c, hipStreamSynchronize(c->stream));
    dev_free(&old_kappa);
    dev_free(&old_stiff);
    dev_free(&old_alpha);
    dev_free(&old_accel);
    dev_free(&old_pid);
    c->capN = cap;
    return SPHX_OK;
}

inline bool device_loop(const sphx_ctx* c) { return !c->tile_mode && !c->host_loop; }


void launch_predict(sphx_ctx* c, const char* label, float dt, const VmaxArgs& va = VmaxArgs{}, const TimerLaw& tl = TimerLaw{}) {
    const uint32_t n = c->N;
    c->velmarks.wrote();
    launch(c, label, 24.0 * n, [&] { hipLaunchKernelGGL(k_predict, dim3(nblocks(n)), dim3(256), 0, c->stream, c->vel, (const float2*)c->accel, n, dt, c->d_scal, va, tl); });
}

void launch_compute_error(sphx_ctx* c, bool divergence, float dt, const float* dt_dev, const LoopArgs& la, uint32_t* clear_hist, uint32_t clear_len,
                          const PredArgs* pred, uint32_t* knz, uint32_t knz_tag, bool take_warm = false,
                          const CountArgs& take_count = CountArgs{}) {
    const uint32_t n = c->N;
    const double lb = list_bytes(c);
    if (pred) c->velmarks.wrote();
    auto go = [&](auto kernel, float* warm, const PredArgs& pa, auto take) {
        hipLaunchKernelGGL(kernel, dim3(nblocks(n)), dim3(256), 0, c->stream, c->pv(), (const float*)c->density, (const float*)c->alpha, n, c->soff(), c->K, dt,
                           c->nbv(), c->kbuf, warm, c->d_scal, dt_dev, la, clear_hist, clear_len, pa, knz, knz_tag, take);
    };
    if (divergence) {
        launch(c, "compute_density_change", (16 + 4 + 4 + lb) * n, [&] {
            if (knz && take_warm) return go(k_compute_error<true, false, true, true>, c->stiff, PredArgs{}, NoTake{});
            if (knz) return go(k_compute_error<true, false, true>, nullptr, PredArgs{}, NoTake{});
            go(k_compute_error<true>, nullptr, PredArgs{}, NoTake{});
        });
    } else if (pred) {
        PredArgs pa = *pred;
        pa.accel = c->accel;
        pa.vel_out = c->vel2;
        launch(c, "velocity_prediction+compute_density_error", (16 + 8 + 8 + 4 + 4 + 4 + lb) * n, [&] {
            if (knz && take_warm) return go(k_compute_error<false, true, true, true>, c->kappa, pa, take_count);
            if (knz) return go(k_compute_error<false, true, true>, nullptr, pa, NoTake{});
            go(k_compute_error<false, true>, nullptr, pa, NoTake{});
        });
    } else {
        launch(c, "compute_density_error", (16 + 4 + 4 + 4 + lb) * n + (clear_hist ? 4.0 * clear_len : 0.0), [&] {
            if (knz && take_warm) return go(k_compute_error<false, false, true, true>, c->kappa, PredArgs{}, take_count);
            if (knz) return go(k_compute_error<false, false, true>, nullptr, PredArgs{}, NoTake{});
            go(k_compute_error<false>, nullptr, PredArgs{}, NoTake{});
        });
    }
}

inline bool correct_skip_ok(const sphx_ctx* c, bool divergence, float dt, const float* dt_dev, const TileClassArgs& tc, const uint32_t* knz) {
    const float inv_dt = 1.0f / dt;
    return knz && c->K.q_noclamp && !tc.pid && std::isfinite(c->K.mass) && c->K.mass > 0.0f && (dt_dev || divergence || (inv_dt > 0.0f && std::isfinite(inv_dt)));
}
void launch_correct(sphx_ctx* c, bool divergence, float dt, const float* dt_dev, const CountArgs& ca, const LoopArgs& la, const ResArgs& ra, bool first,
                    const TileClassArgs& tc, const uint32_t* knz, bool warm_taken = false) {
    const uint32_t n = c->N, f = first ? 1u : 0u;
    const float inv_dt = 1.0f / dt, lim = -0.5f * c->K.rho0 * c->K.rho0;
    const char* const label = divergence ? "correct_velocity_with_divergence_error" : "correct_velocity_with_density_error";
    float* warm = divergence ? c->stiff : c->kappa;
    const bool skip_ok = correct_skip_ok(c, divergence, dt, dt_dev, tc, knz);
    const ZeroSkipArgs zs{skip_ok ? knz : nullptr, c->zero_skip_count ? 1u : 0u};
    const bool quiet_first = zs.knz && c->quiet_hint[divergence ? 1 : 0];
    const bool thin = first && warm_taken && zs.knz && (divergence || ca.hist);
    if ((quiet_first || thin) && c->zero_skip_count) c->qf_launches += 1;
    thin ? c->velmarks.thin(ra.rseq) : c->velmarks.wrote();
    if (thin) {
        c->thin_launches += 1;
        const uint32_t vblocks = nblocks(n);
        auto go_thin = [&](auto kernel) {
            hipLaunchKernelGGL(kernel, dim3(std::min(vblocks, c->thin_grid ? c->thin_grid : 2048u)), dim3(256), 0, c->stream, c->vel, (const float2*)c->posA,
                               (const float*)c->kbuf, warm, n, c->soff(), c->K, inv_dt, lim, c->nbv(), dt_dev, ca, c->d_scal, la, ra, zs, vblocks);
        };
        const double bytes = (16 + 8 + 12 + 8 + list_bytes(c) + (ca.hist ? 8 : 0)) * n;
        return launch(c, label, bytes, [&] { divergence ? go_thin(k_correct_thin<false>) : go_thin(k_correct_thin<true>); }, false);
    }
    auto go = [&](auto kernel, const ZeroSkipArgs& zsa) {
        hipLaunchKernelGGL(kernel, dim3(nblocks(n)), dim3(256), 0, c->stream, c->vel, (const float2*)c->posA, (const float*)c->kbuf, warm, n, c->soff(), c->K, inv_dt,
                           lim, c->nbv(), dt_dev, ca, c->d_scal, la, ra, f, tc, zsa);
    };
    launch(c, label, (16 + 8 + 12 + 8 + list_bytes(c) + (ca.hist ? (tc.pid ? 8 + 4 : 8) : 0)) * n, [&] {
        if (divergence && quiet_first) return go(k_correct<false, false, false, true, true>, zs);
        if (quiet_first) return go(k_correct<false, true, false, true, true>, zs);
        if (divergence && zs.knz) return go(k_correct<false, false, false, true>, zs);
        if (divergence) return go(k_correct<false, false>, zs);
        if (tc.pid) return go(k_correct<false, true, true>, ZeroSkipArgs{});
        if (zs.knz) return go(k_correct<false, true, false, true>, zs);
        go(k_correct<false, true>, zs);
    });
}

void launch_warmstart(sphx_ctx* c, bool divergence, float dt, const float* dt_dev, bool labelled) {
    const uint32_t n = c->N;
    c->velmarks.wrote();
    const float inv_dt = 1.0f / dt, lim = -0.5f * c->K.rho0 * c->K.rho0;
    auto one = [&](auto kernel, float* warm) {
        hipLaunchKernelGGL(kernel, dim3(nblocks(n)), dim3(256), 0, c->stream, c->vel, (const float2*)c->posA, (const float*)c->kbuf, warm, n, c->soff(), c->K, inv_dt,
                           lim, c->nbv(), dt_dev, CountArgs{}, c->d_scal, LoopArgs{}, ResArgs{}, 0u, TileClassArgs{}, ZeroSkipArgs{});
    };
    auto go = [&] { divergence ? one(k_correct<true, false>, c->stiff) : one(k_correct<true, true>, c->kappa); };
    if (!labelled) return go();
    launch(c, divergence ? "correct_divergence_error_warmstart" : "correct_density_error_warmstart", (16 + 8 + 8 + 4 + list_bytes(c)) * n, go);
}

struct IterSpec {
    bool divergence, first;
    float dt;
    const float* dt_dev = nullptr;
    uint32_t* out_warm = nullptr;
    const PredArgs* pred = nullptr;
    LoopArgs la{};
    uint32_t* clear_hist = nullptr;
    uint32_t clear_len = 0;
    CountArgs ca{};
    bool drop_count = false;
    TileClassArgs tc{};
};
inline CountArgs count_args(const sphx_ctx* c, float dt) { return CountArgs{c->gdyn.view(), c->gdyn.hist, c->key, c->slot, dt}; }

uint32_t enqueue_iteration(sphx_ctx* c, const IterSpec& s) {
    if (s.out_warm && s.first) {
        const bool warm = (s.divergence ? c->num_divergence_iters : c->num_density_iters) > 1;
        *s.out_warm = warm ? 1u : 0u;
        if (warm && !(s.divergence && c->handoff.take_warm()))
            launch_warmstart(c, s.divergence, s.dt, s.dt_dev, true);
    }
    const uint32_t seq = ++c->seq;
    const ResArgs ra{1u, ++c->res_seq, c->mbox_dev, seq};
    uint32_t* knz = s.tc.pid ? nullptr : zero_skip_flags(c);
    bool warm_taken = false;
    const BuildHandoff::Taken built = c->handoff.take_first_errors(s.divergence && s.first, ra.rseq);
    if (built.fused) {
        if (!built.flags_usable) knz = nullptr;
        warm_taken = knz && built.warm_taken;
    } else {
        if (s.drop_count) drop_fused_count(c);
        warm_taken = s.first && knz && c->take_over(s.divergence) && (s.divergence || (s.ca.hist && correct_skip_ok(c, false, s.dt, s.dt_dev, s.tc, knz)));
        if (warm_taken) c->takeover_producers += 1;
        launch_compute_error(c, s.divergence, s.dt, s.dt_dev, s.la, s.clear_hist, s.clear_len, s.pred, knz, ra.rseq, warm_taken, s.ca);
    }
    if (s.pred) std::swap(c->vel, c->vel2);
    if (s.drop_count) drop_fused_count(c);
    if (s.ca.hist) s.tc.pid ? c->pending.made_by_classifier(c->N, s.dt) : c->pending.made_by_correction(c->N);
    launch_correct(c, s.divergence, s.dt, s.dt_dev, s.ca, s.la, ra, s.first, s.tc, knz, warm_taken);
    return seq;
}

uint32_t enqueue_context_iteration(sphx_ctx* c, bool divergence, float dt, const float* dt_dev, uint32_t iter, uint32_t gen, uint32_t* out_warm, bool count_ok,
                                   const PredArgs* pred = nullptr) {
    IterSpec s{divergence, iter == 1, dt, dt_dev, out_warm, pred};
    if (gen) {
        s.la.enabled = 1;
        s.la.iter = iter;
        s.la.fixed = divergence ? c->P.fixed_divergence_iterations : c->P.fixed_density_iterations;
        s.la.max_iters = divergence ? c->P.max_divergence_iterations : c->P.max_density_iterations;
        s.la.gen = gen;
        s.la.n_total = c->N;
        s.la.tol = divergence ? c->P.max_divergence_error : c->P.max_avg_density_error;
        s.la.rho0 = c->K.rho0;
        s.la.dt = dt;
    }
    if (!divergence) s.clear_len = c->gdyn.len();
    if (!divergence && count_ok && !c->no_fused_count && !c->tile_mode && c->gdyn.len()) {
        s.ca = count_args(c, dt);
        s.drop_count = !gen || s.first;
        if (!s.drop_count && c->pending.live()) s.clear_hist = c->gdyn.hist;
    }
    return enqueue_iteration(c, s);
}

int judge_residual(sphx_ctx* c, bool divergence, double err_sum, uint32_t iters, float dt, float* out_avg, bool* out_more, uint32_t* io_flags) {
    const uint32_t n = c->N;
    const float rho0 = c->K.rho0;
    const uint32_t fixed = divergence ? c->P.fixed_divergence_iterations : c->P.fixed_density_iterations;
    const uint32_t max_iters = divergence ? c->P.max_divergence_iterations : c->P.max_density_iterations;
    const float tol = divergence ? c->P.max_divergence_error : c->P.max_avg_density_error;
    const float sum = (float)err_sum;
    float avg;
    if (divergence) {
        avg = sum / (float)n / rho0;
        if (!std::isfinite(avg)) return c->fail(SPHX_ERR_NONFINITE, "avg_divergence is not finite (dfsph.rs:378)");
    } else {
        avg = sum / (float)n;
        if (!std::isfinite(avg)) return c->fail(SPHX_ERR_NONFINITE, "avg_density_error is not finite (dfsph.rs:223)");
    }
    bool more;
    if (fixed) {
        more = iters < fixed;
    } else {
        const float rel = divergence ? avg : avg / rho0;
        more = !(rel * dt < tol);
        if (more && iters > max_iters) {
            *io_flags |= divergence ? SPHX_FLAG_DIVERGENCE_ITER_CAP : SPHX_FLAG_DENSITY_ITER_CAP;
            more = false;
        }
    }
    *out_avg = avg;
    *out_more = more;
    return SPHX_OK;
}

int wait_loop(sphx_ctx* c, uint32_t seq, uint32_t gen, bool* out_done) {
    volatile uint32_t* ps = &c->mbox->seq;
    volatile uint32_t* pg = &c->mbox->loop_gen_done;
    bool done = false, reached = false;
    for (int spin = 0; spin < 400000; ++spin) {
        if (*pg == gen) {
            done = true;
            break;
        }
        if ((int32_t)(*ps - seq) >= 0) {
            reached = true;
            break;
        }
        __builtin_ia32_pause();
    }
    if (!done && !reached) {
        SPHX_HIP(c, hipStreamSynchronize(c->stream));
        done = *pg == gen;
        if (!done && (int32_t)(*ps - seq) < 0) return c->fail(SPHX_ERR_HIP, "device did not publish the solver residual (kernel fault?)");
    }
    __atomic_thread_fence(__ATOMIC_ACQUIRE);
    if (!done) done = *pg == gen;
    *out_done = done;
    return SPHX_OK;
}

uint32_t take_vmax_slot(sphx_ctx* c) {
    if (c->ahead.queued) {
        c->ahead.queued = c->ahead.valid = false;
        hipLaunchKernelGGL(k_clear_vmax_slot, dim3(1), dim3(64), 0, c->stream, c->d_scal, c->ahead.vslot);
        return c->ahead.vslot;
    }
    return c->vmax_seq++ & 3u;
}

inline bool finite_not_neg_zero(float f) {
    uint32_t u;
    std::memcpy(&u, &f, 4);
    return std::isfinite(f) && u != 0x80000000u;
}
inline bool rigid_conditions(const sphx_ctx* c, float dt) {
    const float rd = c->K.rho0 * dt;
    const float fc = c->VK.visc_model == SPHX_VISCOSITY_PHYSICAL ? c->VK.mu * c->K.mass * c->VK.vis_nlap * c->K.h : c->K.xsph_eps * c->K.mass * c->K.p6_norm;
    return c->rigid_on() && c->K.q_noclamp && c->lists_current && finite_not_neg_zero(c->K.ax) && finite_not_neg_zero(c->K.ay) && dt > 0.0f &&
           std::isfinite(dt) && std::isfinite(rd) && rd >= 1.175494351e-38f && std::isfinite(fc);
}
void enqueue_nonpressure(sphx_ctx* c, float dt_prev, uint32_t vslot, const VelMarks::Taken& marks = VelMarks::Taken{}) {
    const uint32_t n = c->N;
    const bool judged = marks.usable && rigid_conditions(c, dt_prev);
    const RigidArgs ra{marks.tag, marks.knz_tag, marks.check_knz ? 1u : 0u, nblocks(n), c->mbox_dev};
    c->rigid_judged = judged ? marks.tag : 0u;
    if (!judged) c->rigid_hint = false;
    if (judged && (c->rigid_skip == 2 || c->rigid_hint)) {
        c->rigid_launches += 1;
        auto go_rigid = [&](auto kernel, auto visc) {
            hipLaunchKernelGGL(kernel, dim3(std::min(ra.vgrid, c->thin_grid ? c->thin_grid : 2048u)), dim3(256), 0, c->stream, c->pv(), (const float*)c->density, n,
                               c->soff(), c->K, dt_prev, c->nbv(), c->accel, c->d_scal, vslot, visc, ra);
        };
        return launch(c, "nonpressure_accel_vmax", 8.0 * n, [&] {
            if (c->VK.visc_model == SPHX_VISCOSITY_PHYSICAL) return go_rigid(k_nonpressure_rigid<SPHX_VISCOSITY_PHYSICAL>, ViscArg<SPHX_VISCOSITY_PHYSICAL>{c->VK});
            go_rigid(k_nonpressure_rigid<SPHX_VISCOSITY_XSPH>, ViscArg<SPHX_VISCOSITY_XSPH>{});
        }, false);
    }
    auto go = [&](auto kernel, auto visc) {
        hipLaunchKernelGGL(kernel, dim3(nblocks(n)), dim3(256), 0, c->stream, c->pv(), (const float*)c->density, n, c->soff(), c->K, dt_prev, c->nbv(), c->accel,
                           c->d_scal, vslot, visc);
        if (judged) hipLaunchKernelGGL(k_rigid_judge, dim3(1), dim3(64), 0, c->stream, (const DevScalars*)c->d_scal, c->K.rho0, dt_prev, ra);
    };
    launch(c, "nonpressure_accel_vmax", (16.0 + 8 + 4 + list_bytes(c)) * n, [&] {
        if (c->VK.visc_model == SPHX_VISCOSITY_PHYSICAL) return go(k_nonpressure<SPHX_VISCOSITY_PHYSICAL>, ViscArg<SPHX_VISCOSITY_PHYSICAL>{c->VK});
        go(k_nonpressure<SPHX_VISCOSITY_XSPH>, ViscArg<SPHX_VISCOSITY_XSPH>{});
    });
}

void enqueue_run_ahead(sphx_ctx* c, float dt, bool publish) {
    const uint32_t vslot = take_vmax_slot(c);
    c->ahead.queued = c->ahead.valid = true;
    c->ahead.vslot = vslot;
    c->ahead.seq = 0;
    c->ahead.n = c->N;
    std::memcpy(&c->ahead.dt_bits, &dt, 4);
    enqueue_nonpressure(c, dt, vslot, publish ? VelMarks::Taken{} : c->velmarks.take());
    if (publish) {
        c->ahead.seq = ++c->seq;
        hipLaunchKernelGGL(k_publish_vmax, dim3(1), dim3(64), 0, c->stream, c->d_scal, VmaxArgs{1u, vslot, c->mbox_dev, c->ahead.seq});
    }
}

int solver_loop(sphx_ctx* c, bool divergence, float dt, uint32_t* out_iters, float* out_avg, uint32_t* out_warm, uint32_t* io_flags, bool count_ok,
                uint32_t pre_seq = 0, uint32_t pre_q = 0, uint32_t pre_gen = 0, bool run_ahead = false) {
    uint32_t iters = 0;
    float avg = 0;
    int rc;
    if (device_loop(c)) {
        const uint32_t prev = std::max(1u, divergence ? c->num_divergence_iters : c->num_density_iters);
        const uint32_t cap = (divergence ? c->P.max_divergence_iterations : c->P.max_density_iterations) + 1;
        uint32_t gen = pre_gen, q = pre_q, seq1 = pre_seq;
        if (!pre_seq) {
            if (++c->loop_gen == 0) c->loop_gen = 1;
            gen = c->loop_gen;
            seq1 = enqueue_context_iteration(c, divergence, dt, nullptr, 1, gen, out_warm, count_ok);
            q = 1;
        }
        while (q < std::min(prev, cap)) enqueue_context_iteration(c, divergence, dt, nullptr, ++q, gen, out_warm, count_ok);
        if (run_ahead && c->run_ahead) enqueue_run_ahead(c, dt, false);
        uint32_t w = q;
        for (;;) {
            bool done = false;
            if ((rc = wait_loop(c, seq1 + w - 1, gen, &done))) return rc;
            if (done) break;
            c->ahead.valid = false;
            while (q < w + 2) enqueue_context_iteration(c, divergence, dt, nullptr, ++q, gen, out_warm, count_ok);
            w += 1;
        }
        iters = c->mbox->loop_iters;
        if ((rc = wait_mailbox(c, seq1 + iters - 1))) return rc;
        c->quiet_hint[divergence ? 1 : 0] = c->mbox->quiet_seq == seq1 + iters - 1;
        const uint32_t first = iters > LOOP_HIST - 1 ? iters - (LOOP_HIST - 1) : 1;
        for (uint32_t k = first; k <= iters; ++k) {
            bool more;
            uint32_t fl = 0;
            if ((rc = judge_residual(c, divergence, c->mbox->loop_hist[k % LOOP_HIST], k, dt, &avg, &more, &fl))) return rc;
            if (more != (k < iters)) {
                c->uploaded = false;
                return c->fail(SPHX_ERR_HIP, "the device's residual test disagrees with the host's (solver loop); upload the state again");
            }
            if (k == iters) *io_flags |= fl;
        }
    } else {
        uint32_t seq = pre_seq ? pre_seq : enqueue_context_iteration(c, divergence, dt, nullptr, 1, 0, out_warm, count_ok);
        for (;;) {
            iters += 1;
            if ((rc = wait_mailbox(c, seq))) return rc;
            bool more;
            if ((rc = judge_residual(c, divergence, c->mbox->err_sum, iters, dt, &avg, &more, io_flags))) return rc;
            if (!more) {
                c->quiet_hint[divergence ? 1 : 0] = c->mbox->quiet_seq == seq;
                break;
            }
            seq = enqueue_context_iteration(c, divergence, dt, nullptr, iters + 1, 0, out_warm, count_ok);
        }
    }
    *out_iters = iters;
    *out_avg = avg;
    if (divergence)
        c->num_divergence_iters = iters;
    else
        c->num_density_iters = iters;
    return SPHX_OK;
}

}

extern "C" {

uint32_t sphx_abi_version(void) { return SPHX_ABI_VERSION; }

int sphx_default_params(float smoothing_factor, float particle_density, float fluid_density, sphx_params* p) {
    if (!p || !(particle_density > 0)) return SPHX_ERR_INVALID_ARGUMENT;
    std::memset(p, 0, sizeof(*p));
    const float radius = 0.5f / std::sqrt(particle_density);
    p->smoothing_length = 2.0f * radius * smoothing_factor;
    p->particle_mass = fluid_density / particle_density;
    p->fluid_density = fluid_density;
    p->particle_radius = radius;
    p->gravity[0] = 0.0f;
    p->gravity[1] = -9.81f;
    p->grid_min[0] = -100.0f;
    p->grid_min[1] = -100.0f;
    p->xsph_epsilon = 0.05f;
    p->viscosity_model = SPHX_VISCOSITY_XSPH;
    p->fluid_viscosity = 1.0016f / 1000.0f;
    p->max_avg_density_error = 0.01f / 100.0f;
    p->max_density_iterations = 200;
    p->max_divergence_error = 0.1f / 100.0f;
    p->max_divergence_iterations = 400;
    p->device = 0;
    return SPHX_OK;
}

const char* sphx_last_error(const sphx_ctx* ctx) { return ctx ? ctx->err.c_str() : g_create_error.c_str(); }

int sphx_debug_correction_counts(sphx_ctx* c, uint64_t out[3]) {
    if (!c || !out) return SPHX_ERR_INVALID_ARGUMENT;
    SPHX_HIP(c, hipSetDevice(c->device));
    SPHX_HIP(c, hipStreamSynchronize(c->stream));
    std::vector<Stripe> st(STRIPES);
    SPHX_HIP(c, hipMemcpy(st.data(), c->d_scal->stripe, sizeof(Stripe) * STRIPES, hipMemcpyDeviceToHost));
    out[0] = out[1] = out[2] = 0;
    for (const Stripe& s : st) {
        out[0] += s.zs_skipped;
        out[1] += s.zs_window;
        out[2] += s.zs_remote;
    }
    return SPHX_OK;
}

int sphx_debug_takeover_counts(sphx_ctx* c, uint64_t out[3]) {
    if (!c || !out) return SPHX_ERR_INVALID_ARGUMENT;
    out[0] = c->thin_launches;
    out[1] = c->takeover_producers;
    SPHX_HIP(c, hipSetDevice(c->device));
    SPHX_HIP(c, hipStreamSynchronize(c->stream));
    unsigned long long moved = 0;
    SPHX_HIP(c, hipMemcpy(&moved, &c->d_scal->spec.moved, sizeof(moved), hipMemcpyDeviceToHost));
    out[2] = moved;
    return SPHX_OK;
}

int sphx_debug_rigid_counts(sphx_ctx* c, uint64_t out[3]) {
    if (!c || !out) return SPHX_ERR_INVALID_ARGUMENT;
    out[0] = c->rigid_launches;
    SPHX_HIP(c, hipSetDevice(c->device));
    SPHX_HIP(c, hipStreamSynchronize(c->stream));
    uint32_t dev[2] = {0u, 0u};
    SPHX_HIP(c, hipMemcpy(dev, &c->d_scal->rigid_exits, sizeof(dev), hipMemcpyDeviceToHost));
    out[1] = dev[0];
    out[2] = dev[1];
    return SPHX_OK;
}

int sphx_debug_download_accel(sphx_ctx* c, float* out_xy) {
    if (!c || (c->N && !out_xy)) return SPHX_ERR_INVALID_ARGUMENT;
    SPHX_HIP(c, hipSetDevice(c->device));
    SPHX_HIP(c, hipStreamSynchronize(c->stream));
    if (c->N) SPHX_HIP(c, hipMemcpy(out_xy, c->accel, (size_t)c->N * 8, hipMemcpyDeviceToHost));
    return SPHX_OK;
}

int sphx_debug_quiet_counts(sphx_ctx* c, uint64_t out[2]) {
    if (!c || !out) return SPHX_ERR_INVALID_ARGUMENT;
    SPHX_HIP(c, hipSetDevice(c->device));
    SPHX_HIP(c, hipStreamSynchronize(c->stream));
    std::vector<Stripe> st(STRIPES);
    SPHX_HIP(c, hipMemcpy(st.data(), c->d_scal->stripe, sizeof(Stripe) * STRIPES, hipMemcpyDeviceToHost));
    out[0] = 0;
    for (const Stripe& s : st) out[0] += s.zs_quiet;
    out[1] = c->qf_launches;
    return SPHX_OK;
}

int sphx_create(const sphx_params* params, sphx_ctx** out) {
    if (!params || !out) return SPHX_ERR_INVALID_ARGUMENT;
    *out = nullptr;
    if (!(params->smoothing_length > 0) || !(params->particle_mass > 0) || !(params->fluid_density > 0)) {
        g_create_error = "smoothing_length, particle_mass and fluid_density must be positive";
        return SPHX_ERR_INVALID_ARGUMENT;
    }
    if (params->viscosity_model != SPHX_VISCOSITY_XSPH && params->viscosity_model != SPHX_VISCOSITY_PHYSICAL) {
        g_create_error = "viscosity_model must be SPHX_VISCOSITY_XSPH (0) or SPHX_VISCOSITY_PHYSICAL (1)";
        return SPHX_ERR_INVALID_ARGUMENT;
    }
    if (!std::isfinite(params->fluid_viscosity)) {
        g_create_error = "fluid_viscosity must be finite";
        return SPHX_ERR_INVALID_ARGUMENT;
    }
    int ndev = 0;
    if (hipGetDeviceCount(&ndev) != hipSuccess || ndev <= 0 || params->device < 0 || params->device >= ndev) {
        g_create_error = "no usable HIP device (libsphx has no CPU fallback)";
        return SPHX_ERR_NO_DEVICE;
    }
    sphx_ctx* c = new sphx_ctx();
    if (const char* e = std::getenv("SPHX_SCAN_TWO_PASS")) c->scan_two_pass = e[0] == '1';
    if (const char* e = std::getenv("SPHX_CBITS_MIN")) c->gdyn.cbits_floor = c->gstat.cbits_floor = (uint32_t)std::max(1, std::atoi(e));
    if (const char* e = std::getenv("SPHX_NO_FUSED_COUNT")) c->no_fused_count = e[0] == '1';
    if (const char* e = std::getenv("SPHX_HOST_LOOP")) c->host_loop = e[0] == '1';
    if (const char* e = std::getenv("SPHX_RUN_AHEAD")) c->run_ahead = e[0] != '0';
    if (const char* e = std::getenv("SPHX_FUSE_PREDICT")) c->fuse_predict = e[0] != '0';
    if (const char* e = std::getenv("SPHX_LAZY_TABLE")) c->lazy_table = e[0] != '0' ? 1 : 0;
    if (const char* e = std::getenv("SPHX_STREAM_LISTS")) c->stream_lists = e[0] != '0' ? 1 : 0;
    if (const char* e = std::getenv("SPHX_NT_COLD_STORES")) c->nt_cold_stores = e[0] != '0' ? 1 : 0;
    if (const char* e = std::getenv("SPHX_TILE_FUSE_CLASS")) c->tile_fuse_class = e[0] != '0';
    if (const char* e = std::getenv("SPHX_FUSE_DIV")) c->fuse_div = e[0] != '0';
    if (const char* e = std::getenv("SPHX_XCD_CHUNK")) c->xcd_chunk = (int)xcd_shift_clamp(std::atoi(e));
    if (const char* e = std::getenv("SPHX_ALTERNATE_SWEEP")) c->alternate_sweep = e[0] == '2' ? 2 : (e[0] != '0');
    if (const char* e = std::getenv("SPHX_ZERO_SKIP")) c->zero_skip = e[0] != '0';
    if (const char* e = std::getenv("SPHX_ZERO_SKIP_COUNT")) c->zero_skip_count = e[0] == '1';
    if (const char* e = std::getenv("SPHX_QUIET_TAKEOVER")) c->quiet_takeover = std::strcmp(e, "force") == 0 ? 2 : (e[0] != '0' ? 1 : 0);
    if (const char* e = std::getenv("SPHX_QUIET_TAKEOVER_DENSITY")) c->quiet_takeover_density = e[0] != '0';
    if (const char* e = std::getenv("SPHX_RIGID_SKIP")) c->rigid_skip = std::strcmp(e, "force") == 0 ? 2 : (e[0] != '0' ? 1 : 0);
    if (const char* e = std::getenv("SPHX_THIN_GRID")) c->thin_grid = (uint32_t)std::max(0, std::atoi(e));
    if (const char* e = std::getenv("SPHX_FUSE_WARM")) c->fuse_warm = e[0] != '0';
    c->P = *params;
    c->device = params->device;
    const float h = params->smoothing_length;
    const float PI_F = (float)3.14159265358979323846;
    Consts& K = c->K;
    K.h = h;
    K.radius_sq = h * h;
    K.cell_inv = 1.0f / h;
    K.gmin_x = params->grid_min[0];
    K.gmin_y = params->grid_min[1];
    K.w_hinv = 1.0f / h;
    K.w_norm = 4.0f * 7.0f / (PI_F * rs_powi(h, 2));
    K.w_ngrad = 140.0f / (PI_F * rs_powi(h, 4));
    K.p6_hsq = h * h;
    K.p6_norm = 4.0f / (PI_F * rs_powi(h, 8));
    K.p6_ngrad = 24.0f / (PI_F * rs_powi(h, 8));
    K.sp_h = h;
    K.sp_norm = 10.0f / (PI_F * rs_powi(h, 5));
    K.sp_ngrad = 30.0f / (PI_F * rs_powi(h, 5));
    K.mass = params->particle_mass;
    K.rho0 = params->fluid_density;
    K.xsph_eps = params->xsph_epsilon;
    c->VK.visc_model = params->viscosity_model;
    c->VK.mu = params->fluid_viscosity;
    c->VK.vis_nlap = 360.0f / (29.0f * PI_F * rs_powi(h, 5));
    K.tile = TileRect{0u, 65536u, 0u, 65536u};
    K.remote_cap = params->list_span_limit == SPHX_LISTS_32BIT ? 0u : params->list_span_limit == 0 ? REMOTE_CAP : std::min(params->list_span_limit, REMOTE_CAP);
    {
        volatile float hh = h * h, root = std::sqrt(hh), qmax = h * K.w_hinv;
        c->fast_walk_ok = (root == h && qmax <= 1.0f) ? 1u : 0u;
        if (const char* e = std::getenv("SPHX_QCLAMP")) if (e[0] == '1') c->fast_walk_ok = 0u;
        K.q_noclamp = 0u;
        K.rev = 0u;
        K.nt_cold = 0u;
        K.xcd_shift = 0u;
    }
    K.gx = params->gravity[0];
    K.gy = params->gravity[1];
    {
        const float speed_of_sound = 1.0f / std::sqrt(0.01f);
        K.wc_stiffness = params->fluid_density * speed_of_sound * speed_of_sound / 7.0f;
        K.wc_boundary_force = 1.0f;
    }
    K.ax = params->gravity[0] * K.mass / K.mass;
    K.ay = params->gravity[1] * K.mass / K.mass;
    auto bail = [&](const char* what, hipError_t e) {
        g_create_error = std::string(what) + ": " + hipGetErrorString(e);
        sphx_destroy(c);
        return SPHX_ERR_HIP;
    };
    hipError_t e;
    if ((e = hipSetDevice(c->device)) != hipSuccess) return bail("hipSetDevice", e);
    if ((e = hipStreamCreateWithFlags(&c->stream, hipStreamNonBlocking)) != hipSuccess) return bail("hipStreamCreate", e);
    if ((e = hipMalloc((void**)&c->d_scal, sizeof(DevScalars))) != hipSuccess) return bail("hipMalloc", e);
    if ((e = hipHostMalloc((void**)&c->mbox, sizeof(Mailbox), hipHostMallocMapped | hipHostMallocCoherent)) != hipSuccess)
        return bail("hipHostMalloc", e);
    std::memset((void*)c->mbox, 0, sizeof(Mailbox));
    if ((e = hipHostGetDevicePointer((void**)&c->mbox_dev, (void*)c->mbox, 0)) != hipSuccess) return bail("hipHostGetDevicePointer", e);
    if ((e = hipMemsetAsync(c->d_scal, 0, sizeof(DevScalars), c->stream)) != hipSuccess) return bail("hipMemset", e);
    int rc = set_directory(c, c->gdyn, 0, 0, 0, 0, nullptr, true);
    if (!rc) rc = set_directory(c, c->gstat, 0, 0, 0, 0, nullptr, true);
    if (!rc) rc = dev_alloc(c, &c->bpos, 1);
    if (!rc) rc = dev_alloc(c, &c->bpos2, 1);
    if (!rc) rc = dev_alloc(c, &c->bid, 1);
    if (!rc) rc = dev_alloc(c, &c->bid2, 1);
    if (!rc) rc = ensure_nb_arrays(c, 0, 1, false);
    if (rc) {
        g_create_error = c->err;
        sphx_destroy(c);
        return rc;
    }
    c->capB = 1;
    *out = c;
    return SPHX_OK;
}

void sphx_destroy(sphx_ctx* c) {
    if (!c) return;
    hipSetDevice(c->device);
    if (c->stream) hipStreamSynchronize(c->stream);
#ifdef SPHX_STAMPS
// ... 294 lines not shown
        drop_fused_count(c);
        return c->fail(SPHX_ERR_INVALID_ARGUMENT, c->uploaded ? "dt must be positive and finite"
                                                               : "dt must be positive and finite (phase B had started: upload the state again)");
    }
    SPHX_HIP(c, hipSetDevice(c->device));
    const uint32_t n = c->N;
    sphx_step_stats s;
    std::memset(&s, 0, sizeof(s));
    s.dt_prev = c->step_dt_prev;
    s.dt = dt;
    s.vmax = c->step_vmax;
    int rc;
    auto broken = [&](int code) {
        if (code == SPHX_ERR_HIP || code == SPHX_ERR_NONFINITE) {
            c->uploaded = false;
            clear_histograms(c);
        }
        drop_fused_count(c);
        c->ahead.valid = false;
        c->handoff.clear();
        c->rigid_forget();
        c->law_active = false;
        return code;
    };
    if (n) {
        uint32_t pre = 0, pre_q = 0, pre_gen = 0;
        if (c->law_active) {
            uint32_t bits;
            std::memcpy(&bits, &dt, 4);
            if (bits != c->law_dt_bits) {
                c->uploaded = false;
                c->law_active = false;
                drop_fused_count(c);
                return c->fail(SPHX_ERR_INVALID_ARGUMENT, "dt differs from the sphx_timer_law handed to sphx_step_begin_law; upload the state again");
            }
            pre = c->pre_seq;
            pre_q = c->pre_queued;
            pre_gen = c->pre_gen;
            s.warmstart_density = c->pre_warm;
        } else {
            launch_predict(c, "velocity_prediction", dt);
        }
        c->law_active = false;
        if ((rc = solver_loop(c, false, dt, &s.density_iterations, &s.avg_density_error, &s.warmstart_density, &c->step_flags, true, pre, pre_q, pre_gen)))
            return broken(rc);
        const bool fuse_div = c->fuse_div && !c->tile_mode && c->num_divergence_iters <= 1;
        const bool fuse_warm = c->fuse_div && c->fuse_warm && !c->tile_mode && c->num_divergence_iters > 1;
        if ((rc = update_neighborhood(c, false, dt, true, fuse_div, fuse_warm))) return broken(rc);
        if ((rc = solver_loop(c, true, dt, &s.divergence_iterations, &s.avg_divergence, &s.warmstart_divergence, &c->step_flags, false, 0, 0, 0, true)))
            return broken(rc);
        s.neighbor_entries = c->nb_last;
        s.remote_entries = (uint32_t)std::min<unsigned long long>(c->rem_last, 0xFFFFFFFFull);
    }
    c->law_active = false;
    s.flags = c->step_flags;
    if (out) *out = s;
    sample_after_step(c);
    track_after_step(c);
    stats_after_step(c, dt);
    return SPHX_OK;
}

int sphx_wcsph_step_begin(sphx_ctx* c, float dt, float* out_vmax) {
    if (!c || !out_vmax) return SPHX_ERR_INVALID_ARGUMENT;
    c->ahead.valid = false;
    if (!c->uploaded) return c->fail(SPHX_ERR_NOT_READY, "sphx_wcsph_step_begin before sphx_upload");
    if (c->in_step) return c->fail(SPHX_ERR_NOT_READY, "a step is already open");
    if (c->tile_mode) return c->fail(SPHX_ERR_INVALID_ARGUMENT, "WCSPH is not available on tiles");
    if (!(dt > 0) || !std::isfinite(dt)) return c->fail(SPHX_ERR_INVALID_ARGUMENT, "dt must be positive and finite");
    SPHX_HIP(c, hipSetDevice(c->device));
    sample_went_stale(c, "the last WCSPH step did not finish: run a step, or sphx_update_neighborhood + sphx_update_densities");
    c->step_flags = 0;
    c->step_dt_prev = dt;
    const uint32_t n = c->N;
    *out_vmax = 0.0f;
    c->step_vmax = 0.0f;
    if (n == 0) {
        c->in_step = true;
        c->in_wcsph = true;
        return SPHX_OK;
    }
    hipStream_t st = c->stream;
    const dim3 g(nblocks(n)), b(256);
    if (c->wcsph_n < n)
        SPHX_HIP(c, hipMemsetAsync(c->accel + c->wcsph_n, 0, (size_t)(n - c->wcsph_n) * 8, st));
    c->wcsph_n = n;
    launch(c, "wcsph_leapfrog1", 40.0 * n, [&] { hipLaunchKernelGGL(k_wcsph_leapfrog1, g, b, 0, st, c->vel, c->posA, (const float2*)c->accel, n, dt); });
    if (2.0f * c->wcsph_vmax_prev * dt * c->K.cell_inv > 16.0f) c->recover_streak = std::max(c->recover_streak, 1u);
    int rc;
    if ((rc = update_neighborhood(c, false, 0.0f, false))) return rc;
    launch_density<1>(c, true, false);
    const uint32_t seq = ++c->seq;
    const VmaxArgs va{1u, take_vmax_slot(c), c->mbox_dev, seq};
    launch(c, "wcsph_accelerations_vmax", (16.0 + 4 + 8 + 4 + list_bytes(c)) * n, [&] {
        if (c->VK.visc_model == SPHX_VISCOSITY_PHYSICAL)
            hipLaunchKernelGGL(k_wcsph_accel<SPHX_VISCOSITY_PHYSICAL>, g, b, 0, st, c->pv(), (const float*)c->density, n, c->soff(), c->K, dt, c->nbv(),
                               c->accel, c->d_scal, va.vslot, ViscArg<SPHX_VISCOSITY_PHYSICAL>{c->VK});
        else
            hipLaunchKernelGGL(k_wcsph_accel<SPHX_VISCOSITY_XSPH>, g, b, 0, st, c->pv(), (const float*)c->density, n, c->soff(), c->K, dt, c->nbv(),
                               c->accel, c->d_scal, va.vslot, ViscArg<SPHX_VISCOSITY_XSPH>{});
    });
    hipLaunchKernelGGL(k_publish_vmax, dim3(1), dim3(64), 0, st, c->d_scal, va);
    if ((rc = wait_mailbox(c, seq))) return rc;
    const uint32_t vbits = c->mbox->vmax_sq_bits;
    float vsq;
    std::memcpy(&vsq, &vbits, 4);
    if (!std::isfinite(vsq)) return c->fail(SPHX_ERR_NONFINITE, "max velocity is not finite (Duration::from_secs_f32 would panic, timemanager.rs:264)");
    c->step_vmax = std::sqrt(vsq);
    c->wcsph_vmax_prev = c->step_vmax;
    *out_vmax = c->step_vmax;
    c->in_step = true;
    c->in_wcsph = true;
    return SPHX_OK;
}

int sphx_wcsph_step_finish(sphx_ctx* c, float dt, sphx_step_stats* out) {
    if (!c) return SPHX_ERR_INVALID_ARGUMENT;
    if (!c->in_step || !c->in_wcsph) return c->fail(SPHX_ERR_NOT_READY, "sphx_wcsph_step_finish without sphx_wcsph_step_begin");
    if (!(dt > 0) || !std::isfinite(dt)) return c->fail(SPHX_ERR_INVALID_ARGUMENT, "dt must be positive and finite");
    SPHX_HIP(c, hipSetDevice(c->device));
    c->in_step = false;
    c->in_wcsph = false;
    const uint32_t n = c->N;
    sphx_step_stats s;
    std::memset(&s, 0, sizeof(s));
    s.dt_prev = c->step_dt_prev;
    s.dt = dt;
    s.vmax = c->step_vmax;
    if (n) {
        launch_predict(c, "wcsph_leapfrog2", 0.5f * dt);
        int rc = publish_and_wait(c);
        if (rc) return rc;
        s.neighbor_entries = c->nb_last;
    }
    s.flags = c->step_flags;
    if (out) *out = s;
    sample_after_step(c);
    track_after_step(c);
    stats_after_step(c, dt);
    return SPHX_OK;
}

int sphx_view_request(sphx_ctx* c, uint32_t stride, uint32_t* out_count) {
    if (!c || stride == 0) return SPHX_ERR_INVALID_ARGUMENT;
    if (c->in_step) return c->fail(SPHX_ERR_NOT_READY, "sphx_view_request between step_begin and step_finish");
    SPHX_HIP(c, hipSetDevice(c->device));
    const uint32_t n = c->N;
    const uint32_t m = (uint32_t)(((uint64_t)n + stride - 1) / stride);
    if (!c->view_stream) {
        SPHX_HIP(c, hipStreamCreateWithFlags(&c->view_stream, hipStreamNonBlocking));
        SPHX_HIP(c, hipEventCreateWithFlags(&c->view_packed, hipEventDisableTiming));
        SPHX_HIP(c, hipEventCreateWithFlags(&c->view_done, hipEventDisableTiming));
    } else {
        SPHX_HIP(c, hipEventSynchronize(c->view_done));
    }
    if (m > c->view_cap) {
        if (c->view_dev) hipFree(c->view_dev);
        if (c->view_host) hipHostFree(c->view_host);
        c->view_dev = nullptr;
        c->view_host = nullptr;
        c->view_cap = 0;
        SPHX_HIP(c, hipMalloc((void**)&c->view_dev, (size_t)m * 12));
        SPHX_HIP(c, hipHostMalloc((void**)&c->view_host, (size_t)m * 12, hipHostMallocDefault));
        c->view_cap = m;
    }
    if (m) {
// ... 611 lines not shown
```

### yasph2d_amd/csrc/sphx_state.inc

```
#include <cerrno>

#include "sphx_state_format.hpp"

namespace sphx {

__global__ __launch_bounds__(256) void k_state_digest(const uint32_t* __restrict__ w, unsigned long long W, unsigned long long* __restrict__ out) {
    constexpr unsigned long long M = sphx_state::DIGEST_MUL;
    __shared__ unsigned long long wave_sum[4];
    const uint4* __restrict__ v = (const uint4*)w;
    const unsigned long long n4 = W >> 2, stride = (unsigned long long)gridDim.x * 256ull;
    unsigned long long acc = 0;
#pragma unroll 4
    for (unsigned long long q = (unsigned long long)blockIdx.x * 256ull + threadIdx.x; q < n4; q += stride) {
        const uint4 x = v[q];
        const unsigned long long k = (8ull * q + 1ull) * M;
        acc += (unsigned long long)x.x * k + (unsigned long long)x.y * (k + 2ull * M) + (unsigned long long)x.z * (k + 4ull * M) +
               (unsigned long long)x.w * (k + 6ull * M);
    }
    if (blockIdx.x == 0u && threadIdx.x < (uint32_t)(W & 3ull)) {
        const unsigned long long i = 4ull * n4 + threadIdx.x;
        acc += (unsigned long long)w[i] * ((2ull * i + 1ull) * M);
    }
#pragma unroll
    for (int off = 32; off; off >>= 1) acc += __shfl_down(acc, off);
    if ((threadIdx.x & 63u) == 0u) wave_sum[threadIdx.x >> 6] = acc;
    __syncthreads();
    if (threadIdx.x == 0u) {
        unsigned long long s = wave_sum[0] + wave_sum[1] + wave_sum[2] + wave_sum[3];
        if (blockIdx.x == 0u) s += W * sphx_state::DIGEST_LEN;
        atomicAdd(out, s);
    }
}

}

namespace {

using sphx_state::Header;
constexpr uint32_t STATE_NSEC = sphx_state::NSEC;

int state_check(sphx_ctx* c, const char* fn, bool need_state) {
    const std::string f = fn;
    if (c->tile_mode)
        return c->fail(SPHX_ERR_INVALID_ARGUMENT, (f + ": not available on a tile context (its arrays hold ghosts and miss the particles other tiles own)").c_str());
    if (c->in_step) return c->fail(SPHX_ERR_NOT_READY, (f + ": between step_begin and step_finish (finish the step first)").c_str());
    if (need_state && !c->uploaded) return c->fail(SPHX_ERR_NOT_READY, (f + ": the context holds no state (upload or load one first)").c_str());
    return SPHX_OK;
}

void state_header_of(const sphx_ctx* c, Header& h) {
    std::memset(&h, 0, sizeof(h));
    h.params = c->P;
    h.params.device = 0;
    h.s.n = c->N;
    h.s.b = c->B;
    h.s.cached_n = c->cached_n;
    h.s.wcsph_n = c->wcsph_n;
    h.s.ids_issued = c->ids_issued;
    h.s.num_density_iters = c->num_density_iters;
    h.s.num_divergence_iters = c->num_divergence_iters;
    h.s.set_changed = c->set_changed ? 1u : 0u;
    h.s.tiling_invariant = c->tiling_invariant ? 1u : 0u;
    h.s.lists_current = c->lists_current && !c->boundary_changed ? 1u : 0u;
    h.s.sampling_allowed = c->sample_ready == 2u && h.s.lists_current ? 1u : 0u;
    sphx_state::layout(h);
}

const void* state_section_ptr(const sphx_ctx* c, uint32_t k) {
    switch (k) {
        case SPHX_STATE_SEC_POSITIONS: return c->posA;
        case SPHX_STATE_SEC_VELOCITIES: return c->vel;
        case SPHX_STATE_SEC_PARTICLE_ID: return c->pid;
        case SPHX_STATE_SEC_DENSITY: return c->density;
        case SPHX_STATE_SEC_ALPHA: return c->alpha;
        case SPHX_STATE_SEC_KAPPA: return c->kappa;
        case SPHX_STATE_SEC_STIFFNESS: return c->stiff;
        case SPHX_STATE_SEC_ACCEL: return c->accel;
        default: return nullptr;
    }
}

int state_digests(sphx_ctx* c, const Header& h, uint64_t* dig) {
    if (!c->state_dig) SPHX_HIP(c, hipMalloc((void**)&c->state_dig, STATE_NSEC * sizeof(unsigned long long)));
    hipStream_t st = c->stream;
    SPHX_HIP(c, hipMemsetAsync(c->state_dig, 0, STATE_NSEC * sizeof(unsigned long long), st));
    for (uint32_t k = 0; k < STATE_NSEC; ++k) {
        const void* p = state_section_ptr(c, k);
        const unsigned long long W = h.sec[k].bytes / 4u;
        if (!p || !W) continue;
        const unsigned long long want = ((W >> 2) + 255ull) / 256ull;
        const uint32_t grid = (uint32_t)std::min<unsigned long long>(std::max<unsigned long long>(want, 1ull), 2048ull);
        hipLaunchKernelGGL(k_state_digest, dim3(grid), dim3(256), 0, st, (const uint32_t*)p, W, c->state_dig + k);
    }
    unsigned long long host[STATE_NSEC];
    SPHX_HIP(c, hipMemcpyAsync(host, c->state_dig, sizeof(host), hipMemcpyDeviceToHost, st));
    SPHX_HIP(c, hipStreamSynchronize(st));
    for (uint32_t k = 0; k < STATE_NSEC; ++k) dig[k] = host[k];
    dig[SPHX_STATE_SEC_BOUNDARY] = sphx_state::digest_words(c->h_boundary.data(), h.sec[SPHX_STATE_SEC_BOUNDARY].bytes / 4u);
    return SPHX_OK;
}

}

extern "C" {

int sphx_state_size(sphx_ctx* c, uint64_t* out_bytes) {
    if (!c) return SPHX_ERR_INVALID_ARGUMENT;
    if (!out_bytes) return c->fail(SPHX_ERR_INVALID_ARGUMENT, "sphx_state_size: out_bytes is NULL");
    *out_bytes = 0;
    if (int rc = state_check(c, "sphx_state_size", true)) return rc;
    Header h;
    state_header_of(c, h);
    *out_bytes = h.total_bytes;
    return SPHX_OK;
}

int sphx_state_digest(sphx_ctx* c, uint64_t* out) {
    if (!c) return SPHX_ERR_INVALID_ARGUMENT;
    if (!out) return c->fail(SPHX_ERR_INVALID_ARGUMENT, "sphx_state_digest: out is NULL");
    if (int rc = state_check(c, "sphx_state_digest", true)) return rc;
    SPHX_HIP(c, hipSetDevice(c->device));
    Header h;
    state_header_of(c, h);
    return state_digests(c, h, out);
}

int sphx_state_save(sphx_ctx* c, void* buf, uint64_t capacity, uint32_t flags, uint64_t* out_bytes) {
    if (!c) return SPHX_ERR_INVALID_ARGUMENT;
    if (out_bytes) *out_bytes = 0;
    if (flags & ~(uint32_t)SPHX_STATE_DEVICE_BUFFER) return c->fail(SPHX_ERR_INVALID_ARGUMENT, "sphx_state_save: unknown flags bits");
    if (int rc = state_check(c, "sphx_state_save", true)) return rc;
    Header h;
    state_header_of(c, h);
    if (out_bytes) *out_bytes = h.total_bytes;
    if (!buf) return c->fail(SPHX_ERR_INVALID_ARGUMENT, "sphx_state_save: buf is NULL");
    if (capacity < h.total_bytes) return c->fail(SPHX_ERR_CAPACITY, "sphx_state_save: the buffer is smaller than sphx_state_size");
    SPHX_HIP(c, hipSetDevice(c->device));
    uint64_t dig[STATE_NSEC];
    if (int rc = state_digests(c, h, dig)) return rc;
    for (uint32_t k = 0; k < STATE_NSEC; ++k) h.sec[k].digest = dig[k];
    sphx_state::seal(h);
    const bool dev = (flags & SPHX_STATE_DEVICE_BUFFER) != 0;
    unsigned char* const b = (unsigned char*)buf;
    hipStream_t st = c->stream;
    if (dev)
        SPHX_HIP(c, hipMemcpyAsync(b, &h, sizeof(h), hipMemcpyHostToDevice, st));
    else
        std::memcpy(b, &h, sizeof(h));
    for (uint32_t k = 0; k < STATE_NSEC; ++k) {
        const uint64_t off = h.sec[k].offset, bytes = h.sec[k].bytes, next = k + 1 < STATE_NSEC ? h.sec[k + 1].offset : h.total_bytes;
        const void* p = state_section_ptr(c, k);
        if (bytes) {
            if (p)
                SPHX_HIP(c, hipMemcpyAsync(b + off, p, bytes, dev ? hipMemcpyDeviceToDevice : hipMemcpyDeviceToHost, st));
            else if (dev)
                SPHX_HIP(c, hipMemcpyAsync(b + off, c->h_boundary.data(), bytes, hipMemcpyHostToDevice, st));
            else
                std::memcpy(b + off, c->h_boundary.data(), bytes);
        }
        if (const uint64_t pad = next - (off + bytes)) {
            if (dev)
                SPHX_HIP(c, hipMemsetAsync(b + off + bytes, 0, pad, st));
            else
                std::memset(b + off + bytes, 0, pad);
        }
    }
    SPHX_HIP(c, hipStreamSynchronize(st));
    return SPHX_OK;
}

int sphx_state_load(sphx_ctx* c, const void* buf, uint64_t bytes, uint32_t flags) {
    if (!c) return SPHX_ERR_INVALID_ARGUMENT;
    if (flags & ~(uint32_t)SPHX_STATE_DEVICE_BUFFER) return c->fail(SPHX_ERR_INVALID_ARGUMENT, "sphx_state_load: unknown flags bits");
    if (!buf) return c->fail(SPHX_ERR_INVALID_ARGUMENT, "sphx_state_load: buf is NULL");
    if (int rc = state_check(c, "sphx_state_load", false)) return rc;
    const bool dev = (flags & SPHX_STATE_DEVICE_BUFFER) != 0;
    const unsigned char* const b = (const unsigned char*)buf;
    hipStream_t st = c->stream;
    if (bytes < sphx_state::HEADER_BYTES) return c->fail(SPHX_ERR_INVALID_ARGUMENT, "sphx_state_load", "truncated: shorter than the header");
    unsigned char head[sphx_state::HEADER_BYTES];
    if (dev) {
        SPHX_HIP(c, hipSetDevice(c->device));
        SPHX_HIP(c, hipMemcpyAsync(head, b, sizeof(head), hipMemcpyDeviceToHost, st));
        SPHX_HIP(c, hipStreamSynchronize(st));
    } else {
        std::memcpy(head, b, sizeof(head));
    }
    Header h;
    std::string why;
    if (!sphx_state::validate(head, bytes, &h, &why)) return c->fail(SPHX_ERR_INVALID_ARGUMENT, "sphx_state_load", why.c_str());
    if (const char* field = sphx_state::params_mismatch(h.params, c->P))
        return c->fail(SPHX_ERR_INVALID_ARGUMENT, "sphx_state_load: the blob was saved under other params than this context's; first field that differs", field);
    if ((h.s.tiling_invariant != 0) != c->tiling_invariant)
        return c->fail(SPHX_ERR_INVALID_ARGUMENT, h.s.tiling_invariant ? "sphx_state_load: the blob was saved in tiling-invariant mode, this context is not in it"
                                                                       : "sphx_state_load: this context is in tiling-invariant mode, the blob was not saved in it");
    const uint32_t n = h.s.n, nb = h.s.b;
    std::vector<float> hpos((size_t)n * 2), hbnd((size_t)nb * 2);
    const sphx_state::Section &sp = h.sec[SPHX_STATE_SEC_POSITIONS], &sb = h.sec[SPHX_STATE_SEC_BOUNDARY];
    if (dev) {
        if (sp.bytes) SPHX_HIP(c, hipMemcpyAsync(hpos.data(), b + sp.offset, sp.bytes, hipMemcpyDeviceToHost, st));
        if (sb.bytes) SPHX_HIP(c, hipMemcpyAsync(hbnd.data(), b + sb.offset, sb.bytes, hipMemcpyDeviceToHost, st));
        SPHX_HIP(c, hipStreamSynchronize(st));
    } else {
        if (sp.bytes) std::memcpy(hpos.data(), b + sp.offset, sp.bytes);
        if (sb.bytes) std::memcpy(hbnd.data(), b + sb.offset, sb.bytes);
    }
    if (sphx_state::digest_words(hbnd.data(), sb.bytes / 4u) != sb.digest)
        return c->fail(SPHX_ERR_INVALID_ARGUMENT, "sphx_state_load: digest mismatch in section", sphx_state::section_name(SPHX_STATE_SEC_BOUNDARY));
    SPHX_HIP(c, hipSetDevice(c->device));
    c->ahead.valid = false;
    auto broken = [&](int code) {
        c->uploaded = false;
        return code;
    };
    int rc;
    if (hbnd.size() != c->h_boundary.size() || (nb && std::memcmp(hbnd.data(), c->h_boundary.data(), hbnd.size() * 4) != 0)) {
        if ((rc = sphx_set_boundary(c, nb ? hbnd.data() : nullptr, nb))) return broken(rc);
    }
    sample_went_stale(c, "sphx_state_load did not complete: upload or load the state again");
    SPHX_HIP(c, hipStreamSynchronize(st));
    clear_histograms(c);
    if ((rc = alloc_particles(c, std::max(n, h.s.wcsph_n)))) return broken(rc);
    c->N = n;
    lists_went_stale(c);
    if (c->capN) {
        SPHX_HIP(c, hipMemsetAsync(c->alpha, 0, (size_t)c->capN * 4, st));
        SPHX_HIP(c, hipMemsetAsync(c->kappa, 0, (size_t)c->capN * 4, st));
        SPHX_HIP(c, hipMemsetAsync(c->stiff, 0, (size_t)c->capN * 4, st));
    }
    for (uint32_t k = 0; k < STATE_NSEC; ++k) {
        void* p = const_cast<void*>(state_section_ptr(c, k));
        if (p && h.sec[k].bytes)
            SPHX_HIP(c, hipMemcpyAsync(p, b + h.sec[k].offset, h.sec[k].bytes, dev ? hipMemcpyDeviceToDevice : hipMemcpyHostToDevice, st));
    }
    uint64_t dig[STATE_NSEC];
    if ((rc = state_digests(c, h, dig))) return broken(rc);
    for (uint32_t k = 0; k < STATE_NSEC; ++k)
        if (dig[k] != h.sec[k].digest)
            return broken(c->fail(SPHX_ERR_INVALID_ARGUMENT, "sphx_state_load: digest mismatch in section (upload or load the state again)", sphx_state::section_name(k)));
    c->cached_n = h.s.cached_n;
    c->wcsph_n = h.s.wcsph_n;
    c->ids_issued = h.s.ids_issued;
    c->num_density_iters = h.s.num_density_iters;
    c->num_divergence_iters = h.s.num_divergence_iters;
    c->set_changed = h.s.set_changed != 0;
    c->in_wcsph = false;
    c->handoff.clear();
    c->need_expand = c->need_recover = false;
    c->recover_streak = c->recover_cooldown = 0;
    c->uploaded = true;
    c->have_fluid_bbox = cell_bbox(c, hpos.data(), n, c->fb);
    c->gdyn.cover.clear();
    c->gdyn.nbx = c->gdyn.nby = 0;
    if (c->have_fluid_bbox && (rc = cover_dynamic(c, hpos.data(), n, false))) return broken(rc);
    if ((rc = ensure_index_scratch(c))) return broken(rc);
    if (h.s.lists_current) {
        const uint32_t flags_before = c->step_flags;
        if ((rc = update_neighborhood(c, false, 0.0f, false)) || (rc = publish_and_wait(c))) return broken(rc);
        c->step_flags = flags_before;
        if (h.s.sampling_allowed) c->sample_ready = 2u;
    } else {
        if (c->cached_n == n && n) c->set_changed = true;
        sample_went_stale(c, "the loaded state held no current neighbour lists: run a step, or sphx_update_neighborhood + sphx_update_densities");
    }
    return SPHX_OK;
}

int sphx_state_save_file(sphx_ctx* c, const char* path) {
    if (!c) return SPHX_ERR_INVALID_ARGUMENT;
    if (!path) return c->fail(SPHX_ERR_INVALID_ARGUMENT, "sphx_state_save_file: path is NULL");
    uint64_t bytes = 0;
    int rc;
    if ((rc = sphx_state_size(c, &bytes))) return rc;
    std::vector<unsigned char> blob(bytes);
    if ((rc = sphx_state_save(c, blob.data(), bytes, 0u, nullptr))) return rc;
    const std::string tmp = std::string(path) + ".tmp";
    FILE* f = std::fopen(tmp.c_str(), "wb");
    bool ok = f != nullptr;
    if (ok) {
        ok = std::fwrite(blob.data(), 1, blob.size(), f) == blob.size();
        ok = std::fclose(f) == 0 && ok;
    }
    if (ok) ok = std::rename(tmp.c_str(), path) == 0;
    if (!ok) {
        const std::string e = std::strerror(errno);
        std::remove(tmp.c_str());
        return c->fail(SPHX_ERR_INVALID_ARGUMENT, "sphx_state_save_file: cannot write the file", e.c_str());
    }
    return SPHX_OK;
}

int sphx_state_load_file(sphx_ctx* c, const char* path) {
    if (!c) return SPHX_ERR_INVALID_ARGUMENT;
    if (!path) return c->fail(SPHX_ERR_INVALID_ARGUMENT, "sphx_state_load_file: path is NULL");
    FILE* f = std::fopen(path, "rb");
    if (!f) return c->fail(SPHX_ERR_INVALID_ARGUMENT, "sphx_state_load_file: cannot open the file", std::strerror(errno));
    std::vector<unsigned char> blob;
    unsigned char chunk[1 << 16];
    size_t got;
    while ((got = std::fread(chunk, 1, sizeof(chunk), f)) > 0) blob.insert(blob.end(), chunk, chunk + got);
    const bool bad = std::ferror(f) != 0;
    std::fclose(f);
    if (bad) return c->fail(SPHX_ERR_INVALID_ARGUMENT, "sphx_state_load_file: cannot read the file");
    return sphx_state_load(c, blob.empty() ? (const void*)"" : (const void*)blob.data(), blob.size(), 0u);
}

}
// ... 1 lines not shown
```

Baseline: 13.37 billion.

## Defer uniform acceleration fill and add rigid-motion density-error fast path

```diff
diff --git a/include/sphx.h b/include/sphx.h
--- a/include/sphx.h
+++ b/include/sphx.h
@@ -199,6 +199,7 @@
 int sphx_debug_takeover_counts(sphx_ctx* ctx, uint64_t out[3]);
 
 int sphx_debug_rigid_counts(sphx_ctx* ctx, uint64_t out[3]);
+int sphx_debug_rigid_predict_counts(sphx_ctx* ctx, uint64_t out[4]);
 int sphx_debug_download_accel(sphx_ctx* ctx, float* out_xy);
 
 int sphx_clear_cached(sphx_ctx* ctx);
diff --git a/yasph2d_amd/__init__.py b/yasph2d_amd/__init__.py
--- a/yasph2d_amd/__init__.py
+++ b/yasph2d_amd/__init__.py
@@ -644,6 +644,11 @@
         self._chk(self.L.sphx_debug_rigid_counts(self.h, out))
         return int(out[0]), int(out[1]), int(out[2])
 
+    def rigid_predict_counts(self):
+        out = (C.c_uint64 * 4)()
+        self._chk(self.L.sphx_debug_rigid_predict_counts(self.h, out))
+        return int(out[0]), int(out[1]), int(out[2]), int(out[3])
+
     def download_accel(self):
         out = np.zeros((self.n, 2), np.float32)
         self._chk(self.L.sphx_debug_download_accel(self.h, out.ctypes.data_as(C.c_void_p)))
diff --git a/yasph2d_amd/_lib.py b/yasph2d_amd/_lib.py
--- a/yasph2d_amd/_lib.py
+++ b/yasph2d_amd/_lib.py
@@ -289,6 +289,7 @@
     "sphx_debug_quiet_counts": (_i, [_vp, _vp]),
     "sphx_debug_takeover_counts": (_i, [_vp, _vp]),
     "sphx_debug_rigid_counts": (_i, [_vp, _vp]),
+    "sphx_debug_rigid_predict_counts": (_i, [_vp, _vp]),
     "sphx_debug_download_accel": (_i, [_vp, _vp]),
     "sphx_download_by_id": (_i, [_vp, _u32, _u32, _u32, C.POINTER(SphxTrackOut), C.POINTER(_u32)]),
     "sphx_download": (_i, [_vp, _vp, _vp, _vp, _vp]),
diff --git a/yasph2d_amd/csrc/sphx_compute_error_body.inc b/yasph2d_amd/csrc/sphx_compute_error_body.inc
--- /dev/null
+++ b/yasph2d_amd/csrc/sphx_compute_error_body.inc
@@ -0,0 +1,177 @@
+    static_assert(!TAKE || KNZ, "the take-over producers are the ones that leave flags");
+    constexpr bool SPEC = TAKE && !DIVERGENCE;
+    if (la.enabled && la.iter > 1u && scal->loop_done != 0u) return;
+    if (dt_dev) dt = *dt_dev;
+    if (clear_hist) {
+        const uint32_t per = (clear_len + gridDim.x - 1u) / gridDim.x;
+        const uint32_t c0 = blockIdx.x * per, c1 = min(c0 + per, clear_len);
+        for (uint32_t k = c0 + threadIdx.x; k < c1; k += 256u) clear_hist[k] = 0u;
+    }
+    __shared__ Stage<2, 0> rec;
+    auto put = [&](uint32_t slot, const float4& r) { rec.put_vec01(slot, r); };
+    auto take = [&](uint32_t o) { return rec.vec01(o); };
+    const uint32_t blk = xcd_bid(K.rev, K.xcd_shift);
+    const uint32_t i = blk * 256 + threadIdx.x;
+    [[maybe_unused]] bool k_a = false;
+    if constexpr (RIGID != 0) {
+        static_assert(!DIVERGENCE && PREDICT && KNZ && TAKE, "the rigid form is the density loop's take-over producer with the prediction");
+        uint32_t vb = 0;
+        if (pa.va.enabled && threadIdx.x < STRIPES) vb = scal->vstripe[threadIdx.x].vmax[pa.va.vslot & 3u];
+        const uint32_t verdict = scal->verdict.accel_uniform;
+        const float2 v0 = PV.vel[0];
+        const uint32_t last = n ? n - 1u : 0u, ic = min(i, last);
+        const uint32_t craw = nb.counts[ic];
+        const uint32_t wi = (uint32_t)__builtin_amdgcn_readfirstlane(i >> 6);
+        const uint32_t ww = wi * 64u < n ? nb.wave[wi] : 0u;
+        const float2 p_i = PV.pos[ic];
+        const float rho_r = density[ic], alpha_r = alpha[ic];
+        __shared__ float dt_r;
+        if (pa.va.enabled && threadIdx.x < 64) {
+            const uint32_t b = wave_max_u32(vb);
+            const unsigned long long ns = timer_law_step_ns(pa.law, sqrtf(__uint_as_float(b)));
+            const float d = duration_as_secs_f32(ns);
+            if (threadIdx.x == 0) dt_r = d;
+            if (blockIdx.x == 0) vmax_publish(scal, pa.va, b, pa.law, ns, d);
+        }
+        if (pa.va.enabled) {
+            __syncthreads();
+            dt = dt_r;
+        }
+        k_a = verdict == ta.accel_tag;
+        const float4 pvi = make_float4(p_i.x, p_i.y, v0.x + K.ax * dt, v0.y + K.ay * dt);
+        const bool finite = ((__float_as_uint(pvi.z) & 0x7f800000u) != 0x7f800000u) && ((__float_as_uint(pvi.w) & 0x7f800000u) != 0x7f800000u);
+        DirAhead ahead_r{0xFFFFFFFFu, EMPTY};
+        if constexpr (RIGID == 2) {
+            if (ta.hist && i < n) {
+                uint32_t cx0, cy0;
+                cell_of(K, p_i, cx0, cy0);
+                ahead_r = dir_ahead(ta.g, cx0, cy0);
+            }
+        }
+        const uint32_t c = i < n ? craw : 0u;
+        const bool reaches_static = (c & 0x7fu) != ((c >> 7) & 0x7fu) || (ww >> 31) != 0u;
+        const bool walks = __syncthreads_or(reaches_static ? 1 : 0) != 0 || !k_a || !finite || RIGID != 2;
+        if (ta.count && threadIdx.x == 0) {
+            Stripe& s = scal->stripe[blockIdx.x % STRIPES];
+            if (k_a && blk * 256u < n) atomicAdd(walks ? &s.rp_walk : &s.rp_exit, 1u);
+            if (!k_a && blockIdx.x == 0) atomicAdd(&s.rp_noverdict, 1u);
+        }
+        if (!walks) {
+            float e = 0.0f, e_owned = 0.0f;
+            uint32_t k_bits = 0u;
+            float2 pnew = make_float2(0.0f, 0.0f);
+            if (i < n) {
+                const float delta = 0.0f;
+                e = rho_r + delta * K.mass * dt;
+                e = fmaxf(K.rho0, e) - K.rho0;
+                const float kv = e * alpha_r;
+                kbuf[i] = kv;
+                k_bits = __float_as_uint(kv);
+                pa.vel_out[i] = make_float2(pvi.z, pvi.w);
+                store_cold(&warm_zero[i], 0.0f + kv, K.nt_cold);
+                e_owned = tile_owns(K, pvi.x, pvi.y) ? e : 0.0f;
+                pnew = make_float2(pvi.x + pvi.z * dt, pvi.y + pvi.w * dt);
+            }
+            if (ta.hist) count_cell(K, ta.g, i < n, i, pnew, ta.hist, ta.cidx, ta.slot, 1u, scal, ahead_r, &scal->spec.flags);
+            knz_store(knz, i, k_bits, scal, knz_tag);
+            block_residual_add(e_owned, scal);
+            return;
+        }
+    }
+    NbHead h = nb_head(nb, blk, i, n);
+    const float rho_i = (!DIVERGENCE && i < n) ? density[i] : 0.0f;
+    const float alpha_i = i < n ? alpha[i] : 0.0f;
+    struct PredRec {
+        float4 pv;
+        float2 a;
+    };
+    auto load_pred = [&](uint32_t g) {
+        if constexpr (RIGID != 0) {
+            if (k_a) return PredRec{ldpv(PV, g), make_float2(K.ax, K.ay)};
+        }
+        return PredRec{ldpv(PV, g), gat(pa.accel, g < soff ? g : 0u)};
+    };
+    auto predicted = [&](const PredRec& r, uint32_t g) {
+        return g < soff ? make_float4(r.pv.x, r.pv.y, r.pv.z + r.a.x * dt, r.pv.w + r.a.y * dt) : r.pv;
+    };
+    if (PREDICT) {
+        uint32_t vb = 0;
+        if (RIGID == 0 && pa.va.enabled && threadIdx.x < STRIPES) vb = scal->vstripe[threadIdx.x].vmax[pa.va.vslot & 3u];
+        auto load_pred2 = [&](uint32_t g) {
+            const Pair<float4> pv = ldpv2(PV, g);
+            if constexpr (RIGID != 0) {
+                if (k_a) return Pair<PredRec>{PredRec{pv.a, make_float2(K.ax, K.ay)}, PredRec{pv.b, make_float2(K.ax, K.ay)}};
+            }
+            const Pair<float2> a = gat2(pa.accel, g < soff ? g : 0u);
+            return Pair<PredRec>{PredRec{pv.a, a.a}, PredRec{pv.b, a.b}};
+        };
+        const NbStaged<PredRec> st = nb_stage_load(h, nb, blk, i, n, load_pred, load_pred2);
+        __shared__ float dt_s;
+        if (RIGID == 0 && pa.va.enabled && threadIdx.x < 64) {
+            const uint32_t b = wave_max_u32(vb);
+            const unsigned long long ns = timer_law_step_ns(pa.law, sqrtf(__uint_as_float(b)));
+            const float d = duration_as_secs_f32(ns);
+            if (threadIdx.x == 0) dt_s = d;
+            if (blockIdx.x == 0) vmax_publish(scal, pa.va, b, pa.law, ns, d);
+        }
+        if (RIGID == 0 && pa.va.enabled) {
+            __syncthreads();
+            dt = dt_s;
+        }
+        nb_stage_store(h, st, [&](uint32_t slot, const PredRec& r, uint32_t g) { put(slot, predicted(r, g)); });
+    } else {
+        nb_stage(h, nb, blk, i, n, [&](uint32_t g) { return ldpv(PV, g); }, [&](uint32_t g) { return ldpv2(PV, g); }, put);
+    }
+    __syncthreads();
+    float e = 0.0f, e_owned = 0.0f;
+    uint32_t k_bits = 0u;
+    [[maybe_unused]] float2 pnew = make_float2(0.0f, 0.0f);
+    [[maybe_unused]] DirAhead ahead{0xFFFFFFFFu, EMPTY};
+    if (i < n) {
+        const uint32_t ct = h.ct;
+        float4 pvi = h.wide ? ldpv(PV, i) : take((i - h.lw0) * 4u);
+        if (PREDICT && h.wide) pvi = predicted(load_pred(i), i);
+        if constexpr (SPEC) {
+            if (ta.hist) {
+                uint32_t cx0, cy0;
+                cell_of(K, make_float2(pvi.x, pvi.y), cx0, cy0);
+                ahead = dir_ahead(ta.g, cx0, cy0);
+            }
+        }
+        if (!(DIVERGENCE && ct < 9)) {
+            const float2 ri = make_float2(pvi.x, pvi.y);
+            float delta = 0.0f;
+            auto walk = [&](auto fast) {
+                auto consume = [&](const float4& r, uint32_t) {
+                    const float2 g = wendland_grad<decltype(fast)::value>(K, ri, make_float2(r.x, r.y));
+                    const float dvx = pvi.z - r.z, dvy = pvi.w - r.w;
+                    delta = delta + (dvx * g.x + dvy * g.y);
+                };
+                nb_traverse(h, ct, take, [&](uint32_t g) { return PREDICT ? predicted(load_pred(g), g) : ldpv(PV, g); }, consume);
+            };
+            if (K.q_noclamp)
+                walk(std::true_type{});
+            else
+                walk(std::false_type{});
+            if (DIVERGENCE) {
+                e = fmaxf(delta * K.mass, 0.0f);
+            } else {
+                e = rho_i + delta * K.mass * dt;
+                e = fmaxf(K.rho0, e) - K.rho0;
+            }
+        }
+        const float kv = e * alpha_i;
+        kbuf[i] = kv;
+        k_bits = __float_as_uint(kv);
+        if (PREDICT) pa.vel_out[i] = make_float2(pvi.z, pvi.w);
+        if constexpr (TAKE)
+            store_cold(&warm_zero[i], 0.0f + kv, K.nt_cold);
+        else if (warm_zero)
+            warm_zero[i] = 0.0f;
+        e_owned = tile_owns(K, pvi.x, pvi.y) ? e : 0.0f;
+        if constexpr (SPEC) pnew = make_float2(pvi.x + pvi.z * dt, pvi.y + pvi.w * dt);
+    }
+    if constexpr (SPEC)
+        if (ta.hist) count_cell(K, ta.g, i < n, i, pnew, ta.hist, ta.cidx, ta.slot, 1u, scal, ahead, &scal->spec.flags);
+    if constexpr (KNZ) knz_store(knz, i, k_bits, scal, knz_tag);
+    block_residual_add(e_owned, scal);
diff --git a/yasph2d_amd/csrc/sphx_handoff.hpp b/yasph2d_amd/csrc/sphx_handoff.hpp
--- a/yasph2d_amd/csrc/sphx_handoff.hpp
+++ b/yasph2d_amd/csrc/sphx_handoff.hpp
@@ -90,4 +90,28 @@
     }
 };
 
+struct AccelUniform {
+    bool owed = false, uniform = false;
+    uint32_t tag = 0;
+    struct Taken {
+        bool fill, k_a;
+        uint32_t tag;
+    };
+    void made(uint32_t gather_tag) { *this = AccelUniform{true, true, gather_tag}; }
+    void velocities_written() { uniform = false; }
+    void filled() { *this = AccelUniform{}; }
+    Taken read() {
+        const Taken t{owed, false, tag};
+        owed = false;
+        return t;
+    }
+    Taken take(bool substitute) {
+        const bool k_a = substitute && uniform;
+        const Taken t{owed && !k_a, k_a, tag};
+        if (t.fill) owed = false;
+        uniform = false;
+        return t;
+    }
+};
+
 }
diff --git a/yasph2d_amd/csrc/sphx_internal.hpp b/yasph2d_amd/csrc/sphx_internal.hpp
--- a/yasph2d_amd/csrc/sphx_internal.hpp
+++ b/yasph2d_amd/csrc/sphx_internal.hpp
@@ -124,7 +124,8 @@
     uint32_t pad0;
     unsigned long long zs_skipped, zs_window, zs_remote;
     unsigned long long zs_quiet;
-    uint32_t pad[12];
+    uint32_t rp_exit, rp_walk, rp_noverdict;
+    uint32_t pad[9];
 };
 static_assert(sizeof(Stripe) == 128, "one stripe, one cache line");
 struct alignas(128) VmaxStripe {
@@ -142,6 +143,10 @@
     uint32_t pad0;
     unsigned long long moved;
     uint32_t pad[28];
+};
+struct alignas(128) VerdictLine {
+    uint32_t accel_uniform;
+    uint32_t pad[31];
 };
 struct DevScalars {
     uint32_t flags;
@@ -157,6 +162,7 @@
     VmaxStripe vstripe[STRIPES];
     MarkStripe mstripe[STRIPES];
     SpecLine spec;
+    VerdictLine verdict;
 };
 
 struct Mailbox {
@@ -336,10 +342,14 @@
     uint32_t rigid_judged = 0;
     void rigid_forget() {
         velmarks.wrote();
+        accel_uniform.velocities_written();
         rigid_hint = false;
         rigid_judged = 0;
     }
     unsigned long long rigid_launches = 0;
+    int rigid_predict = 2;
+    sphx::AccelUniform accel_uniform;
+    unsigned long long rigid_predict_launches = 0;
     float2* accel = nullptr;
     float *density = nullptr, *alpha = nullptr, *alpha2 = nullptr, *kappa = nullptr, *stiff = nullptr;
     float *kappa2 = nullptr, *stiff2 = nullptr;
diff --git a/yasph2d_amd/csrc/sphx_kernels.hip b/yasph2d_amd/csrc/sphx_kernels.hip
--- a/yasph2d_amd/csrc/sphx_kernels.hip
+++ b/yasph2d_amd/csrc/sphx_kernels.hip
@@ -2095,6 +2095,7 @@
     uint32_t check_knz;
     uint32_t vgrid;
     Mailbox* mb;
+    uint32_t fill;
 };
 __device__ __forceinline__ bool rigid_marked(const DevScalars* __restrict__ scal, float rho0, float dt, const RigidArgs& ra) {
     uint32_t vm = ~ra.vmix_tag, km = ~ra.knz_tag;
@@ -2121,12 +2122,15 @@
     if (blockIdx.x == 0 && threadIdx.x == 0) {
         __hip_atomic_store(&ra.mb->rigid_tag, marked ? 0u : ra.vmix_tag, __ATOMIC_RELAXED, __HIP_MEMORY_SCOPE_SYSTEM);
         atomicAdd(marked ? &scal->rigid_marked : &scal->rigid_exits, 1u);
+        scal->verdict.accel_uniform = (!marked && ra.fill == 0u) ? ra.vmix_tag : ~ra.vmix_tag;
     }
     if (!marked) {
         const float2 a = make_float2(K.ax, K.ay);
-        for (uint32_t vblk = blockIdx.x; vblk < ra.vgrid; vblk += gridDim.x) {
-            const uint32_t i = xcd_map(vblk, ra.vgrid, K.rev, K.xcd_shift) * 256u + threadIdx.x;
-            if (i < n) accel[i] = a;
+        if (ra.fill != 0u) {
+            for (uint32_t vblk = blockIdx.x; vblk < ra.vgrid; vblk += gridDim.x) {
+                const uint32_t i = xcd_map(vblk, ra.vgrid, K.rev, K.xcd_shift) * 256u + threadIdx.x;
+                if (i < n) accel[i] = a;
+            }
         }
         if (blockIdx.x == 0 && threadIdx.x == 0) {
             const float2 v = PV.vel[0];
@@ -2294,109 +2298,34 @@
                                                         uint32_t* __restrict__ clear_hist, uint32_t clear_len, PredArgs pa,
                                                         uint32_t* __restrict__ knz, uint32_t knz_tag,
                                                         std::conditional_t<TAKE && !DIVERGENCE, CountArgs, NoTake> ta) {
-    static_assert(!TAKE || KNZ, "the take-over producers are the ones that leave flags");
-    constexpr bool SPEC = TAKE && !DIVERGENCE;
-    if (la.enabled && la.iter > 1u && scal->loop_done != 0u) return;
-    if (dt_dev) dt = *dt_dev;
-    if (clear_hist) {
-        const uint32_t per = (clear_len + gridDim.x - 1u) / gridDim.x;
-        const uint32_t c0 = blockIdx.x * per, c1 = min(c0 + per, clear_len);
-        for (uint32_t k = c0 + threadIdx.x; k < c1; k += 256u) clear_hist[k] = 0u;
-    }
-    __shared__ Stage<2, 0> rec;
-    auto put = [&](uint32_t slot, const float4& r) { rec.put_vec01(slot, r); };
-    auto take = [&](uint32_t o) { return rec.vec01(o); };
-    const uint32_t blk = xcd_bid(K.rev, K.xcd_shift);
-    const uint32_t i = blk * 256 + threadIdx.x;
-    NbHead h = nb_head(nb, blk, i, n);
-    const float rho_i = (!DIVERGENCE && i < n) ? density[i] : 0.0f;
-    const float alpha_i = i < n ? alpha[i] : 0.0f;
-    struct PredRec {
-        float4 pv;
-        float2 a;
-    };
-    auto load_pred = [&](uint32_t g) { return PredRec{ldpv(PV, g), gat(pa.accel, g < soff ? g : 0u)}; };
-    auto predicted = [&](const PredRec& r, uint32_t g) {
-        return g < soff ? make_float4(r.pv.x, r.pv.y, r.pv.z + r.a.x * dt, r.pv.w + r.a.y * dt) : r.pv;
-    };
-    if (PREDICT) {
-        uint32_t vb = 0;
-        if (pa.va.enabled && threadIdx.x < STRIPES) vb = scal->vstripe[threadIdx.x].vmax[pa.va.vslot & 3u];
-        auto load_pred2 = [&](uint32_t g) {
-            const Pair<float4> pv = ldpv2(PV, g);
-            const Pair<float2> a = gat2(pa.accel, g < soff ? g : 0u);
-            return Pair<PredRec>{PredRec{pv.a, a.a}, PredRec{pv.b, a.b}};
-        };
-        const NbStaged<PredRec> st = nb_stage_load(h, nb, blk, i, n, load_pred, load_pred2);
-        __shared__ float dt_s;
-        if (pa.va.enabled && threadIdx.x < 64) {
-            const uint32_t b = wave_max_u32(vb);
-            const unsigned long long ns = timer_law_step_ns(pa.law, sqrtf(__uint_as_float(b)));
-            const float d = duration_as_secs_f32(ns);
-            if (threadIdx.x == 0) dt_s = d;
-            if (blockIdx.x == 0) vmax_publish(scal, pa.va, b, pa.law, ns, d);
-        }
-        if (pa.va.enabled) {
-            __syncthreads();
-            dt = dt_s;
-        }
-        nb_stage_store(h, st, [&](uint32_t slot, const PredRec& r, uint32_t g) { put(slot, predicted(r, g)); });
-    } else {
-        nb_stage(h, nb, blk, i, n, [&](uint32_t g) { return ldpv(PV, g); }, [&](uint32_t g) { return ldpv2(PV, g); }, put);
-    }
-    __syncthreads();
-    float e = 0.0f, e_owned = 0.0f;
-    uint32_t k_bits = 0u;
-    [[maybe_unused]] float2 pnew = make_float2(0.0f, 0.0f);
-    [[maybe_unused]] DirAhead ahead{0xFFFFFFFFu, EMPTY};
-    if (i < n) {
-        const uint32_t ct = h.ct;
-        float4 pvi = h.wide ? ldpv(PV, i) : take((i - h.lw0) * 4u);
-        if (PREDICT && h.wide) pvi = predicted(load_pred(i), i);
-        if constexpr (SPEC) {
-            if (ta.hist) {
-                uint32_t cx0, cy0;
-                cell_of(K, make_float2(pvi.x, pvi.y), cx0, cy0);
-                ahead = dir_ahead(ta.g, cx0, cy0);
-            }
-        }
-        if (!(DIVERGENCE && ct < 9)) {
-            const float2 ri = make_float2(pvi.x, pvi.y);
-            float delta = 0.0f;
-            auto walk = [&](auto fast) {
-                auto consume = [&](const float4& r, uint32_t) {
-                    const float2 g = wendland_grad<decltype(fast)::value>(K, ri, make_float2(r.x, r.y));
-                    const float dvx = pvi.z - r.z, dvy = pvi.w - r.w;
-                    delta = delta + (dvx * g.x + dvy * g.y);
-                };
-                nb_traverse(h, ct, take, [&](uint32_t g) { return PREDICT ? predicted(load_pred(g), g) : ldpv(PV, g); }, consume);
-            };
-            if (K.q_noclamp)
-                walk(std::true_type{});
-            else
-                walk(std::false_type{});
-            if (DIVERGENCE) {
-                e = fmaxf(delta * K.mass, 0.0f);
-            } else {
-                e = rho_i + delta * K.mass * dt;
-                e = fmaxf(K.rho0, e) - K.rho0;
-            }
-        }
-        const float kv = e * alpha_i;
-        kbuf[i] = kv;
-        k_bits = __float_as_uint(kv);
-        if (PREDICT) pa.vel_out[i] = make_float2(pvi.z, pvi.w);
-        if constexpr (TAKE)
-            store_cold(&warm_zero[i], 0.0f + kv, K.nt_cold);
-        else if (warm_zero)
-            warm_zero[i] = 0.0f;
-        e_owned = tile_owns(K, pvi.x, pvi.y) ? e : 0.0f;
-        if constexpr (SPEC) pnew = make_float2(pvi.x + pvi.z * dt, pvi.y + pvi.w * dt);
-    }
-    if constexpr (SPEC)
-        if (ta.hist) count_cell(K, ta.g, i < n, i, pnew, ta.hist, ta.cidx, ta.slot, 1u, scal, ahead, &scal->spec.flags);
-    if constexpr (KNZ) knz_store(knz, i, k_bits, scal, knz_tag);
-    block_residual_add(e_owned, scal);
+    constexpr int RIGID = 0;
+#include "sphx_compute_error_body.inc"
+}
+
+struct RigidTake : CountArgs {
+    uint32_t accel_tag;
+    uint32_t count;
+};
+template <bool EXIT>
+__global__ TRAV_BOUNDS void k_compute_error_rigid(PVr PV, const float* __restrict__ density,
+                                                              const float* __restrict__ alpha, uint32_t n, uint32_t soff, Consts K, float dt,
+                                                              NbView nb, float* __restrict__ kbuf, float* __restrict__ warm_zero,
+                                                              DevScalars* __restrict__ scal, const float* __restrict__ dt_dev, LoopArgs la,
+                                                              uint32_t* __restrict__ clear_hist, uint32_t clear_len, PredArgs pa,
+                                                              uint32_t* __restrict__ knz, uint32_t knz_tag, RigidTake ta) {
+    constexpr bool DIVERGENCE = false, PREDICT = true, KNZ = true, TAKE = true;
+    constexpr int RIGID = EXIT ? 2 : 1;
+#include "sphx_compute_error_body.inc"
+}
+
+__global__ __launch_bounds__(256) void k_accel_materialize(float2* __restrict__ accel, uint32_t n, uint32_t vgrid, float ax, float ay,
+                                                           const DevScalars* __restrict__ scal, uint32_t tag) {
+    if (scal->verdict.accel_uniform != tag) return;
+    const float2 a = make_float2(ax, ay);
+    for (uint32_t vblk = blockIdx.x; vblk < vgrid; vblk += gridDim.x) {
+        const uint32_t i = vblk * 256u + threadIdx.x;
+        if (i < n) accel[i] = a;
+    }
 }
 
 struct ZeroSkipArgs {
diff --git a/yasph2d_amd/csrc/sphx_launch.inc b/yasph2d_amd/csrc/sphx_launch.inc
--- a/yasph2d_amd/csrc/sphx_launch.inc
+++ b/yasph2d_amd/csrc/sphx_launch.inc
@@ -529,6 +529,7 @@
     const bool partial = &g == &c->gdyn && tile_n && advect_dt == 0.0f && !counted && c->pending.is_for_first_of(n);
     const uint32_t first = partial ? c->pending.n() : 0u;
     if (&g == &c->gdyn) c->velmarks.wrote();
+    if (&g == &c->gdyn) c->accel_uniform.velocities_written();
     if (counted || partial)
         c->pending.forget();
     else
@@ -843,6 +844,7 @@
             launch(c, "neighbor_build+density_alpha+divergence_warmstart", (8.0 + list_bytes(c) + 8.0 + 8.0 + 8.0 + 4.0) * n, [&] { go(k_neighbor_build<3>, dv); });
             c->handoff = BuildHandoff::warm_applied();
             c->velmarks.wrote();
+            c->accel_uniform.velocities_written();
         } else if (fuse && fuse_div) {
             DivArgs dv{};
             dv.vel = (const float2*)c->vel;
@@ -885,6 +887,22 @@
     launch(c, "compute_alpha_factors", bytes, [&] { go(k_density_alpha<0, false, true>); });
 }
 
+void fill_accel(sphx_ctx* c, const AccelUniform::Taken& t) {
+    const uint32_t n = std::min(c->N, c->capN);
+    if (!t.fill || !n || !c->accel) return;
+    const uint32_t vgrid = nblocks(n);
+    launch(c, "accel_materialize", 8.0 * n, [&] {
+        hipLaunchKernelGGL(k_accel_materialize, dim3(std::min(vgrid, 2048u)), dim3(256), 0, c->stream, c->accel, n, vgrid, c->K.ax, c->K.ay,
+                           (const DevScalars*)c->d_scal, t.tag);
+    }, false);
+}
+void read_accel(sphx_ctx* c) { fill_accel(c, c->accel_uniform.read()); }
+AccelUniform::Taken take_accel(sphx_ctx* c, bool substitute) {
+    const AccelUniform::Taken t = c->accel_uniform.take(substitute);
+    fill_accel(c, t);
+    return t;
+}
+
 int alloc_particles(sphx_ctx* c, uint32_t n, uint32_t cap = 0, bool keep_set = false) {
     if (n <= c->capN) return SPHX_OK;
     cap = std::max(cap, n);
@@ -896,6 +914,7 @@
     if (keep_set) c->pid = nullptr;
     const uint32_t keep = std::min(c->cached_n, c->capN);
     const uint32_t keep_accel = std::min(c->wcsph_n, c->capN);
+    keep_accel ? read_accel(c) : c->accel_uniform.filled();
     c->kappa = c->stiff = c->alpha = nullptr;
     c->accel = nullptr;
     auto give_up = [&](int code) {
@@ -945,6 +964,7 @@
 void launch_predict(sphx_ctx* c, const char* label, float dt, const VmaxArgs& va = VmaxArgs{}, const TimerLaw& tl = TimerLaw{}) {
     const uint32_t n = c->N;
     c->velmarks.wrote();
+    take_accel(c, false);
     launch(c, label, 24.0 * n, [&] { hipLaunchKernelGGL(k_predict, dim3(nblocks(n)), dim3(256), 0, c->stream, c->vel, (const float2*)c->accel, n, dt, c->d_scal, va, tl); });
 }
 
@@ -968,6 +988,18 @@
         PredArgs pa = *pred;
         pa.accel = c->accel;
         pa.vel_out = c->vel2;
+        const AccelUniform::Taken au = take_accel(c, c->rigid_predict != 0 && knz && take_warm && c->K.q_noclamp && !c->tile_mode);
+        if (au.k_a) {
+            c->rigid_predict_launches += 1;
+            const RigidTake rt{take_count, au.tag, c->zero_skip_count ? 1u : 0u};
+            auto go_rigid = [&](auto kernel) {
+                hipLaunchKernelGGL(kernel, dim3(nblocks(n)), dim3(256), 0, c->stream, c->pv(), (const float*)c->density, (const float*)c->alpha, n, c->soff(), c->K, dt,
+                                   c->nbv(), c->kbuf, c->kappa, c->d_scal, dt_dev, la, clear_hist, clear_len, pa, knz, knz_tag, rt);
+            };
+            const double bytes = c->rigid_predict == 2 ? (8 + 4 + 4 + 2 + 4 + 8 + 4 + 4 + 8) * (double)n : (16 + 8 + 4 + 4 + 4 + lb) * n;
+            return launch(c, "velocity_prediction+compute_density_error", bytes,
+                          [&] { c->rigid_predict == 2 ? go_rigid(k_compute_error_rigid<true>) : go_rigid(k_compute_error_rigid<false>); });
+        }
         launch(c, "velocity_prediction+compute_density_error", (16 + 8 + 8 + 4 + 4 + 4 + lb) * n, [&] {
             if (knz && take_warm) return go(k_compute_error<false, true, true, true>, c->kappa, pa, take_count);
             if (knz) return go(k_compute_error<false, true, true>, nullptr, pa, NoTake{});
@@ -998,6 +1030,7 @@
     const bool thin = first && warm_taken && zs.knz && (divergence || ca.hist);
     if ((quiet_first || thin) && c->zero_skip_count) c->qf_launches += 1;
     thin ? c->velmarks.thin(ra.rseq) : c->velmarks.wrote();
+    c->accel_uniform.velocities_written();
     if (thin) {
         c->thin_launches += 1;
         const uint32_t vblocks = nblocks(n);
@@ -1026,6 +1059,7 @@
 void launch_warmstart(sphx_ctx* c, bool divergence, float dt, const float* dt_dev, bool labelled) {
     const uint32_t n = c->N;
     c->velmarks.wrote();
+    c->accel_uniform.velocities_written();
     const float inv_dt = 1.0f / dt, lim = -0.5f * c->K.rho0 * c->K.rho0;
     auto one = [&](auto kernel, float* warm) {
         hipLaunchKernelGGL(kernel, dim3(nblocks(n)), dim3(256), 0, c->stream, c->vel, (const float2*)c->posA, (const float*)c->kbuf, warm, n, c->soff(), c->K, inv_dt,
@@ -1182,11 +1216,12 @@
 void enqueue_nonpressure(sphx_ctx* c, float dt_prev, uint32_t vslot, const VelMarks::Taken& marks = VelMarks::Taken{}) {
     const uint32_t n = c->N;
     const bool judged = marks.usable && rigid_conditions(c, dt_prev);
-    const RigidArgs ra{marks.tag, marks.knz_tag, marks.check_knz ? 1u : 0u, nblocks(n), c->mbox_dev};
+    const RigidArgs ra{marks.tag, marks.knz_tag, marks.check_knz ? 1u : 0u, nblocks(n), c->mbox_dev, c->rigid_predict == 0 ? 1u : 0u};
     c->rigid_judged = judged ? marks.tag : 0u;
     if (!judged) c->rigid_hint = false;
     if (judged && (c->rigid_skip == 2 || c->rigid_hint)) {
         c->rigid_launches += 1;
+        ra.fill ? c->accel_uniform.filled() : c->accel_uniform.made(marks.tag);
         auto go_rigid = [&](auto kernel, auto visc) {
             hipLaunchKernelGGL(kernel, dim3(std::min(ra.vgrid, c->thin_grid ? c->thin_grid : 2048u)), dim3(256), 0, c->stream, c->pv(), (const float*)c->density, n,
                                c->soff(), c->K, dt_prev, c->nbv(), c->accel, c->d_scal, vslot, visc, ra);
@@ -1196,6 +1231,7 @@
             go_rigid(k_nonpressure_rigid<SPHX_VISCOSITY_XSPH>, ViscArg<SPHX_VISCOSITY_XSPH>{});
         }, false);
     }
+    c->accel_uniform.filled();
     auto go = [&](auto kernel, auto visc) {
         hipLaunchKernelGGL(kernel, dim3(nblocks(n)), dim3(256), 0, c->stream, c->pv(), (const float*)c->density, n, c->soff(), c->K, dt_prev, c->nbv(), c->accel,
                            c->d_scal, vslot, visc);
@@ -1354,9 +1390,26 @@
     return SPHX_OK;
 }
 
+int sphx_debug_rigid_predict_counts(sphx_ctx* c, uint64_t out[4]) {
+    if (!c || !out) return SPHX_ERR_INVALID_ARGUMENT;
+    SPHX_HIP(c, hipSetDevice(c->device));
+    SPHX_HIP(c, hipStreamSynchronize(c->stream));
+    std::vector<Stripe> st(STRIPES);
+    SPHX_HIP(c, hipMemcpy(st.data(), c->d_scal->stripe, sizeof(Stripe) * STRIPES, hipMemcpyDeviceToHost));
+    out[0] = c->rigid_predict_launches;
+    out[1] = out[2] = out[3] = 0;
+    for (const Stripe& s : st) {
+        out[1] += s.rp_exit;
+        out[2] += s.rp_walk;
+        out[3] += s.rp_noverdict;
+    }
+    return SPHX_OK;
+}
+
 int sphx_debug_download_accel(sphx_ctx* c, float* out_xy) {
     if (!c || (c->N && !out_xy)) return SPHX_ERR_INVALID_ARGUMENT;
     SPHX_HIP(c, hipSetDevice(c->device));
+    read_accel(c);
     SPHX_HIP(c, hipStreamSynchronize(c->stream));
     if (c->N) SPHX_HIP(c, hipMemcpy(out_xy, c->accel, (size_t)c->N * 8, hipMemcpyDeviceToHost));
     return SPHX_OK;
@@ -1413,6 +1466,7 @@
     if (const char* e = std::getenv("SPHX_QUIET_TAKEOVER")) c->quiet_takeover = std::strcmp(e, "force") == 0 ? 2 : (e[0] != '0' ? 1 : 0);
     if (const char* e = std::getenv("SPHX_QUIET_TAKEOVER_DENSITY")) c->quiet_takeover_density = e[0] != '0';
     if (const char* e = std::getenv("SPHX_RIGID_SKIP")) c->rigid_skip = std::strcmp(e, "force") == 0 ? 2 : (e[0] != '0' ? 1 : 0);
+    if (const char* e = std::getenv("SPHX_RIGID_PREDICT")) c->rigid_predict = std::strcmp(e, "accel") == 0 ? 1 : (e[0] != '0' ? 2 : 0);
     if (const char* e = std::getenv("SPHX_THIN_GRID")) c->thin_grid = (uint32_t)std::max(0, std::atoi(e));
     if (const char* e = std::getenv("SPHX_FUSE_WARM")) c->fuse_warm = e[0] != '0';
     c->P = *params;
@@ -1873,6 +1927,7 @@
     }
     hipStream_t st = c->stream;
     const dim3 g(nblocks(n)), b(256);
+    read_accel(c);
     if (c->wcsph_n < n)
         SPHX_HIP(c, hipMemsetAsync(c->accel + c->wcsph_n, 0, (size_t)(n - c->wcsph_n) * 8, st));
     c->wcsph_n = n;
diff --git a/yasph2d_amd/csrc/sphx_state.inc b/yasph2d_amd/csrc/sphx_state.inc
--- a/yasph2d_amd/csrc/sphx_state.inc
+++ b/yasph2d_amd/csrc/sphx_state.inc
@@ -82,6 +82,7 @@
 
 int state_digests(sphx_ctx* c, const Header& h, uint64_t* dig) {
     if (!c->state_dig) SPHX_HIP(c, hipMalloc((void**)&c->state_dig, STATE_NSEC * sizeof(unsigned long long)));
+    if (h.sec[SPHX_STATE_SEC_ACCEL].bytes) read_accel(c);
     hipStream_t st = c->stream;
     SPHX_HIP(c, hipMemsetAsync(c->state_dig, 0, STATE_NSEC * sizeof(unsigned long long), st));
     for (uint32_t k = 0; k < STATE_NSEC; ++k) {
@@ -223,6 +224,7 @@
     if ((rc = alloc_particles(c, std::max(n, h.s.wcsph_n)))) return broken(rc);
     c->N = n;
     lists_went_stale(c);
+    if (h.sec[SPHX_STATE_SEC_ACCEL].bytes) read_accel(c);
     if (c->capN) {
         SPHX_HIP(c, hipMemsetAsync(c->alpha, 0, (size_t)c->capN * 4, st));
         SPHX_HIP(c, hipMemsetAsync(c->kappa, 0, (size_t)c->capN * 4, st));
```

Measured after the change: 14.09 billion, median of 6. 5.4% higher.
